# imaginateit/csm-train-pytorch

Hardware: AMD Instinct MI355X
Metric: train tokens/sec (text+audio) CSM-1B bf16 seq2048 (higher is better)
Workload: dtype bf16

## Files before the change

csm-train-pytorch_amd/csm/engine.py:

```python
from __future__ import annotations

import math
import numbers
from contextlib import contextmanager
from typing import Dict, List, Optional

import torch

from .hip import ops

BF16 = torch.bfloat16
F32 = torch.float32
import os as _os
FUSE_SWIGLU = _os.environ.get("CSM_FUSE_SWIGLU", "1") == "1"
FUSE_ROPE_BWD = _os.environ.get("CSM_FUSE_ROPE_BWD", "1") == "1"
FUSE_ROPE_FWD = _os.environ.get("CSM_FUSE_ROPE_FWD", "1") == "1"
PAIR_DX_DW = int(_os.environ.get("CSM_PAIR_DX_DW", "0"))
GROUP_ATTN_DW = _os.environ.get("CSM_GROUP_ATTN_DW", "1") == "1"
DEFER_ATTN_DW = int(_os.environ.get("CSM_DEFER_ATTN_DW", "3"))
DEFER_NORM_DW = _os.environ.get("CSM_DEFER_NORM_DW", "1") == "1"
ROWS_ON_HOST = _os.environ.get("CSM_ROWS_ON_HOST", "1") == "1"
EMB_KEYSORT = _os.environ.get("CSM_EMB_KEYSORT", "1") == "1"
DECODE_POS_HOST = _os.environ.get("CSM_DECODE_POS_HOST", "1") == "1"
LORA_FUSE = _os.environ.get("CSM_LORA_FUSE", "1") != "0"
# ... 562 lines not shown

    def _decoder_forward(self, hidden, rows, tg, B, S, save, sel=None):
        m, a = self.m, self.m.args
        dev = m.device
        K, V, Vp = a.audio_num_codebooks, a.audio_vocab_size, m.vocab_pad
        N = rows.numel()
        d, dd = m.bb.embed_dim, m.dc.embed_dim
        codes = tg[:, :S, :].reshape(-1, K) if tg.shape[1] >= S else None
        if codes is None:
            b, p = rows.long() // S, rows.long() % S
            codes = tg[b, p]
        else:
            codes = codes[rows.long()]
        codes = codes.contiguous()
        seq = torch.empty(N * K, d, dtype=BF16, device=dev)
        ops.decoder_input_fwd(hidden, rows, codes, m.block("audio_embeddings.weight"), seq, V)
        x0 = torch.empty(N * K, dd, dtype=BF16, device=dev)
        ops.linear_fwd(seq, m.block("projection.weight"), x0)
        dsel = sel[rows.long()].repeat_interleave(K).contiguous() if sel is not None else None
        xf = self.decoder.forward(x0, N, K, save, on_layer_start=self.param_hook, sel=dsel)
        logits = torch.empty(K - 1, N, Vp, dtype=F32, device=dev)
        ah = m.block("audio_head.padded")
        xf2 = xf.view(N, K * dd)
        ops.gemm(xf2[:, dd:2 * dd], ah[0], logits[0], None, False, True, batch=K - 1, sA=dd, sB=dd * Vp, sC=N * Vp)
        tgt = codes[:, 1:].t().contiguous().reshape(-1)
        rows_loss = torch.empty((K - 1) * N, dtype=F32, device=dev)
        ops.ce_fwd_bwd(logits.view(-1, Vp), tgt, rows_loss, None, V, 0.0)
        out = dict(rows_loss=rows_loss, n_rows=(K - 1) * N)
        if save:
            out.update(rows=rows, codes=codes, seq=seq, xf=xf, logits=logits, tgt=tgt, N=N, sel=dsel)
        return out

    def backward(self, gscale: float = 1.0):
        if self.saved is None:
            raise RuntimeError("backward() without a saved forward (was the forward run under no_grad?)")
        s, m, a = self.saved, self.m, self.m.args
        self.saved = None
        dev = m.device
        B, S = s["B"], s["S"]
        K, V, Vp = a.audio_num_codebooks, a.audio_vocab_size, m.vocab_pad
        M, d, dd = B * S, m.bb.embed_dim, m.dc.embed_dim
        tr = m.trainable
        train_embeddings, train_other = tr["embeddings"], tr["other"]
        m.ensure_grads()
        gst = m.grad_state
        dec_runs = s["dec"] is not None and s["aw"] != 0.0
        writes = {"backbone": tr["backbone"], "decoder": dec_runs and tr["decoder"], "other": train_other,
                  "embeddings": train_embeddings}
        acc = {}
        for g_, w_ in writes.items():
            acc[g_] = gst[g_] == "live"
            if gst[g_] == "stale" and (not w_ or g_ == "embeddings"):
                o_, n_ = m.group_range(g_)
                m.grad_arena[o_:o_ + n_].zero_()
                gst[g_] = "zero"
            if w_:
                gst[g_] = "live"
        if train_other and not acc["other"] and not dec_runs:
            m.block("projection.weight", True).zero_()
            m.block("audio_head.padded", True).zero_()
        hidden = s["hidden"]
        dseq = None
        dec_pos0 = None
        dec = s["dec"]
        if dec is not None and s["aw"] != 0.0:
            N = dec["N"]
            dl = torch.empty(K - 1, N, Vp, dtype=BF16, device=dev)
            ops.ce_fwd_bwd(dec["logits"].view(-1, Vp), dec["tgt"], dec["rows_loss"], dl.view(-1, Vp), V,
                           gscale * s["aw"] / dec["n_rows"])
            ah = m.block("audio_head.padded")
            dxf = torch.zeros(N, K * dd, dtype=BF16, device=dev)
            ops.gemm(dl[0], ah[0], dxf[:, dd:2 * dd], None, False, False, batch=K - 1, sA=N * Vp, sB=dd * Vp, sC=dd)
            xf2 = dec["xf"].view(N, K * dd)
            if train_other:
                gah = m.block("audio_head.padded", True)
                ops.gemm(xf2[:, dd:2 * dd], dl[0], gah[0], gah[0] if acc["other"] else None, True, True, batch=K - 1, sA=dd,
                         sB=N * Vp, sC=dd * Vp, sR=dd * Vp)
            del dl
            dx0 = self.decoder.backward(dxf.view(N * K, dd), N, K, tr["decoder"], 1.0, on_layer_done=self.grad_hook,
                                        acc=acc["decoder"], sel=dec.get("sel"))
            dseq = torch.empty(N * K, d, dtype=BF16, device=dev)
            ops.linear_dx(dx0, m.block("projection.weight"), dseq)
            if train_other:
                ops.linear_dw(dx0, dec["seq"], m.block("projection.weight", True), accumulate=acc["other"])
            dec_pos0 = (dseq, dec["rows"], K)
            if self.grad_hook is not None:
                self.grad_hook("decoder", -1)

        dlog = torch.empty(M, Vp, dtype=BF16, device=dev)
        rows_loss = torch.empty(M, dtype=F32, device=dev)
        ops.ce_fwd_bwd(s["logits"], s["t0"], rows_loss, dlog, V, gscale * s["sw"] / s["n_sem"])
        dhid = torch.empty(M, d, dtype=BF16, device=dev)
        ops.linear_dx(dlog, m.block("codebook0_head.padded"), dhid)
        if train_other:
            ops.linear_dw(dlog, hidden, m.block("codebook0_head.padded", True), accumulate=acc["other"])
        del dlog
        if dec_pos0 is not None:
            ops.rows_add_bf16(dhid, dec_pos0[1], dec_pos0[0], dec_pos0[2])
        if self.grad_hook is not None:
            self.grad_hook("other", -1)

        dh0 = self.backbone.backward(dhid, B, S, tr["backbone"], 1.0, on_layer_done=self.grad_hook, acc=acc["backbone"], seg=s.get("seg"),
                                    sel=s.get("sel"))
        if train_embeddings:
            self._embedding_backward(s, dh0, dseq if (dec is not None and s["aw"] != 0.0) else None)
        if self.grad_hook is not None:
            self.grad_hook("embeddings", -1)

    def _embedding_backward(self, s, dh0, dseq):
        m, a = self.m, self.m.args
        dev = m.device
        K, V = a.audio_num_codebooks, a.audio_vocab_size
        TV = a.text_vocab_size
        n_rows = TV + K * V
        tk, mk = s["tk"], s["mk"]
        M = tk.shape[0]
        ck = ("embbwd", M, K, V, TV)
        c = self._consts.get(ck)
        if c is None:
            slot = torch.arange(K + 1, device=dev)
            c = self._consts[ck] = dict(off=torch.where(slot < K, TV + slot * V, torch.zeros_like(slot)),
                                        src=torch.arange(M, device=dev).unsqueeze(1).expand(M, K + 1).reshape(-1).contiguous())
        rows = torch.where(mk.bool(), tk + c["off"], torch.full_like(tk, n_rows)).reshape(-1)
        src = c["src"]
        n_src = M
        if dseq is not None:
            codes, N = s["dec"]["codes"], s["dec"]["N"]
            dk = ("embbwd_dec", M, N, K, V, TV)
            d = self._consts.get(dk)
            if d is None:
                d = self._consts[dk] = dict(off=TV + torch.arange(K - 1, device=dev) * V,
                                            src=(M + torch.arange(N, device=dev).unsqueeze(1) * K + torch.arange(1, K, device=dev)).reshape(-1))
            rows = torch.cat([rows, (codes[:, :K - 1] + d["off"]).reshape(-1)])
            src = torch.cat([src, d["src"]])
            n_src = M + N * K
        if n_src <= (1 << 20) and EMB_KEYSORT:
            key = torch.sort((rows << 20) | src).values
            rows_s, src_s = key >> 20, key & ((1 << 20) - 1)
        else:
            order = torch.argsort(rows, stable=True)
            rows_s, src_s = rows[order].contiguous(), src[order].contiguous()
        ops.embed_bwd_sorted(rows_s, src_s, dh0, dseq,
                             m.block("text_embeddings.weight", True), m.block("audio_embeddings.weight", True))

    @torch.no_grad()
    def hidden_states(self, tokens: torch.Tensor, masks: torch.Tensor) -> torch.Tensor:
        m, a = self.m, self.m.args
        B, S, K1 = tokens.shape
        M = B * S
        tk = tokens.reshape(M, K1).to(device=m.device, dtype=torch.int64).contiguous()
        mk = masks.reshape(M, K1).to(device=m.device, dtype=torch.uint8).contiguous()
        h0 = torch.empty(M, m.bb.embed_dim, dtype=BF16, device=m.device)
        self._need()
        ops.embed_fwd(tk, mk, m.block("text_embeddings.weight"), m.block("audio_embeddings.weight"), h0, a.audio_vocab_size)
        return self.backbone.forward(h0, B, S, False).view(B, S, -1)

    @torch.no_grad()
    def generate_frame(self, tokens, tokens_mask, input_pos, temperature, topk, noise=None, adapters=None, top_p=None,
                       min_p=None):
        m, a = self.m, self.m.args
        self._need()
        if int(input_pos[0, 0]) == 0:
            m._gen_adapters = list(adapters) if adapters is not None and any(x is not None for x in adapters) else None
        if not getattr(m, "use_kv_cache", True):
            if top_p is not None or min_p is not None:
                raise ValueError("the recompute path (use_kv_cache = False) has no top_p / min_p: the filters need the KV-cache path")
            return self._generate_frame_recompute(tokens, tokens_mask, input_pos, temperature, topk, noise)
        dev = m.device
        K, V, Vp = a.audio_num_codebooks, a.audio_vocab_size, m.vocab_pad
        d, dd = m.bb.embed_dim, m.dc.embed_dim
        tokens, tokens_mask = tokens.to(dev), tokens_mask.to(dev)
        Bn, Sn, K1 = tokens.shape
        first = int(input_pos[0, 0]) == 0
        st = getattr(m, "_decode_state", None)
        if not first and (st is None or st.B != Bn or st.cur < 0):
            raise RuntimeError("generate_frame: a non-first call (input_pos > 0) needs the state of a prompt prefilled with the "
                               "same batch size (call it with input_pos starting at 0 first)")
        if first:
            st = m._decode_state = DecodeState(self, Bn, adapters)
        temperature, topk = st.sampling_args(temperature, topk, top_p, min_p)
        if first:
            last_h = st.prefill(tokens, tokens_mask)
            return self._frame_tail(st, last_h, temperature, topk, noise)
        if Sn != 1:
            raise ValueError("generate_frame with caches: after the prompt, feed one position per call")
        if getattr(m, "use_hip_graph", True):
            return st.graph_frame(tokens, tokens_mask, temperature, topk, noise)
        st._advance()
        return self._decode_frame(st, tokens, tokens_mask, temperature, topk, noise)

    @torch.no_grad()
    def generate_first_frames(self, tokens_list, masks_list, temperature, topk, noise=None, adapters=None, top_p=None,
                              min_p=None):
        m = self.m
        self._need()
        st = m._decode_state = DecodeState(self, len(tokens_list), adapters)
# ... 753 lines not shown
```

csm-train-pytorch_amd/csm/hip/__init__.py:

```python
import ctypes as C
import os

_HERE = os.path.dirname(os.path.abspath(__file__))
LIB_PATH = os.environ.get("CSM_HIP_LIB") or os.path.join(_HERE, "libcsm_hip.so")


class CsmHipError(RuntimeError):
    pass


if not os.path.exists(LIB_PATH):
    raise ImportError(
        f"{LIB_PATH} is missing: build it with `python __graft_entry__.py build` (or `make -C csm-train-pytorch_amd/csrc`). "
        "The CSM MI355X path has no fallback implementation."
    )

lib = C.CDLL(LIB_PATH)

_p, _i, _f, _ll = C.c_void_p, C.c_int, C.c_float, C.c_longlong

_SIGS = {
    "csm_abi_version": ([], _i),
    "csm_last_error": ([], C.c_char_p),
    "csm_device_check": ([_i], _i),
    "csm_gemm_bf16": ([_p, _p, _p, _p, _i, _i, _i, _i, _i, _i, _i, _i, _i, _i, _f, _i, _ll, _ll, _ll, _ll, _p], _i),
    "csm_gemm_bf16_ex": ([_p, _p, _p, _p, _i, _i, _i, _i, _i, _i, _i, _i, _i, _i, _f, _i, _ll, _ll, _ll, _ll, _i, _p, _p, _i, _p], _i),
    "csm_gemm_bf16_rope": ([_p, _p, _p, _i, _i, _i, _i, _i, _i, _p, _i, _i, _i, _p], _i),
    "csm_gemm_bf16_kext": ([_p, _p, _p, _p, _i, _i, _i, _i, _i, _i, _i, _i, _i, _p, _p, _i, _i, _p, _p, _i, _i, _i, _p], _i),
    "csm_gemm_bf16_pinned": ([_p, _p, _p, _p, _i, _i, _i, _i, _i, _i, _i, _i, _i, _f, _p, _p, _i, _i, _p, _p, _i, _i, _i, _p], _i),
    "csm_skinny_nt_bf16": ([_p, _p, _p, _i, _i, _i, _i, _i, _i, _f, _p], _i),
    "csm_skinny_nt_sel_bf16": ([_p, _p, _p, _p, _i, _i, _i, _i, _i, _i, _i, _f, _p], _i),
    "csm_gemm_bf16_dgrad_wgrad": ([_p, _p, _p, _p, _p, _i, _i, _i, _i, _i, _i, _i, _i, _i, _p, _i, _i, _f, _p], _i),
    "csm_gemm_bf16_two_wgrad": ([_p, _p, _p, _i, _i, _i, _i, _i, _p, _p, _p, _i, _i, _i, _i, _i, _i, _i, _f, _p], _i),
    "csm_gemm_bf16_multi_wgrad": ([_i, _p, _p, _p, _p, _p, _p, _p, _p, _i, _i, _f, _p], _i),
    "csm_set_gemm_variant": ([_i], _i),
    "csm_set_gemm256_persistent": ([_i], _i),
    "csm_get_gemm256_persistent": ([], _i),
    "csm_set_gemm_tuning": ([_i, _i], _i),
    "csm_gemm_last_kernel": ([], C.c_char_p),
    "csm_attn_bwd_workspace_bytes": ([_i, _i, _i], _ll),
    "csm_rmsnorm_fwd": ([_p, _p, _p, _p, _i, _i, _f, _p], _i),
    "csm_rmsnorm_bwd_blocks": ([], _i),
    "csm_rmsnorm_bwd": ([_p, _p, _p, _p, _p, _p, _p, _i, _i, _p], _i),
    "csm_colsum_bf16": ([_p, _i, _i, _p, _i, _p], _i),
    "csm_colsum_bf16_multi": ([_i, _p, _p, _i, _i, _i, _p], _i),
    "csm_dropout_bf16": ([_p, _i, _p, _i, _ll, _i, _f, C.c_ulonglong, _i, _p], _i),
    "csm_bias_add_bf16": ([_p, _i, _p, _ll, _i, _p], _i),
    "csm_colsum_rows_bf16": ([_p, _i, _ll, _i, _p, _i, _p], _i),
    "csm_rope": ([_p, _p, _p, _ll, _i, _i, _i, _i, _i, _p], _i),
    "csm_set_attn_variant": ([_i], _i),
    "csm_attn_last_dkv_kernel": ([], _i),
    "csm_attn64_set_debug": ([_p], _i),
    "csm_set_decode_tuning": ([_i, _i], _i),
    "csm_attn_fwd": ([_p, _p, _p, _i, _i, _i, _i, _i, _p], _i),
    "csm_attn_bwd": ([_p, _p, _p, _p, _p, _p, _i, _i, _i, _i, _i, _p], _i),
    "csm_attn_bwd_rope": ([_p, _p, _p, _p, _p, _p, _p, _i, _i, _i, _i, _i, _p], _i),
    "csm_attn_fwd_seg": ([_p, _p, _p, _p, _i, _i, _i, _i, _i, _p], _i),
    "csm_attn_bwd_seg": ([_p, _p, _p, _p, _p, _p, _p, _p, _i, _i, _i, _i, _i, _p], _i),
    "csm_swiglu_fwd": ([_p, _p, _ll, _i, _p], _i),
    "csm_swiglu_bwd": ([_p, _p, _p, _ll, _i, _p], _i),
    "csm_embed_fwd": ([_p, _p, _p, _p, _p, _ll, _i, _i, _i, _p], _i),
    "csm_embed_bwd_sorted": ([_p, _p, _ll, _p, _p, _ll, _p, _p, _ll, _ll, _i, _p], _i),
    "csm_rows_add_bf16": ([_p, _p, _p, _ll, _i, _i, _p], _i),
    "csm_rows_take_bf16": ([_p, _p, _p, _ll, _i, _p], _i),
    "csm_decoder_input_fwd": ([_p, _p, _p, _p, _p, _ll, _i, _i, _i, _p], _i),
    "csm_ce_fwd_bwd": ([_p, _p, _p, _p, _ll, _i, _i, _i, _f, _p], _i),
    "csm_reduce_sum_f32": ([_p, _ll, _f, _p, _p], _i),
    "csm_sumsq_blocks": ([], _i),
    "csm_sumsq_bf16": ([_p, _ll, _p, _p], _i),
    "csm_clip_coef": ([_p, _i, _f, _p, _p], _i),
    "csm_adamw_step": ([_p, _p, _p, _p, _p, _ll, _f, _f, _f, _f, _f, _i, _p, _f, _i, _p], _i),
    "csm_adamw_step_split": ([_p, _p, _p, _p, _p, _ll, _f, _f, _f, _f, _f, _i, _p, _f, _i, _p], _i),
    "csm_adamw_step_live": ([_p, _p, _p, _p, _p, _ll, _f, _f, _f, _f, _f, _i, _p, _f, _i, _p, _p], _i),
    "csm_adamw_step_split_live": ([_p, _p, _p, _p, _p, _ll, _f, _f, _f, _f, _f, _i, _p, _f, _i, _p, _p], _i),
    "csm_set_adamw_blocks": ([_i], _i),
    "csm_gemv_bf16": ([_p, _p, _p, _p, _i, _i, _i, _i, _i, _i, _i, _p], _i),
    "csm_gemv_bf16_kext": ([_p, _p, _p, _p, _i, _i, _i, _i, _i, _i, _i, _p, _f, _i, _p, _i, _p, _p, _i, _i, _i, _p, _p], _i),
    "csm_lora_project_bf16": ([_p, _p, _p, _i, _i, _i, _i, _i, _i, _f, _p, _f, _p], _i),
    "csm_lora_project_rows_bf16": ([_p, _p, _p, _p, _p, _i, _i, _i, _i, _i, _i, _i, _p, _f, _p], _i),
    "csm_gemv_bf16_kext_rows": ([_p, _p, _p, _p, _i, _i, _i, _i, _i, _i, _i, _p, _f, _i, _p, _i, _p, _p, _p, _p, _i, _i, _i, _i, _p], _i),
    "csm_gemv_t_bf16": ([_p, _p, _p, _i, _i, _i, _i, _i, _i, _i, _p], _i),
    "csm_gemv_bf16_ex": ([_p, _p, _p, _p, _i, _i, _i, _i, _i, _i, _i, _p, _f, _i, _p, _i, _p], _i),
    "csm_quantize_rows_fp8": ([_p, _p, _p, _i, _i, _i, _i, _p], _i),
    "csm_gemv_fp8w": ([_p, _p, _p, _p, _p, _i, _i, _i, _i, _i, _i, _i, _p, _f, _i, _p, _i, _p], _i),
    "csm_attn_decode_rope": ([_p, _p, _p, _p, _p, _p, _i, _i, _i, _i, _i, _i, _p], _i),
    "csm_gemv_attn_bf16": ([_p, _p, _p, _p, _p, _p, _p, _p, _i, _i, _i, _i, _i, _i, _i, _i, _i, _p], _i),
    "csm_gemv_attn_at_bf16": ([_p, _p, _p, _i, _p, _p, _p, _p, _i, _i, _i, _i, _i, _i, _p], _i),
    "csm_attn_decode_rope_at": ([_p, _p, _p, _p, _i, _p, _i, _i, _i, _i, _i, _i, _p], _i),
    "csm_attn_append": ([_p, _p, _p, _p, _i, _i, _i, _i, _i, _i, _i, _f, _p], _i),
    "csm_attn_append_rows": ([_p, _p, _p, _p, _p, _p, _p, _i, _i, _i, _i, _i, _f, _p], _i),
    "csm_kv_append": ([_p, _p, _p, _p, _i, _i, _i, _i, _i, _i, _p], _i),
    "csm_kv_shift": ([_p, _p, _p, _i, _i, _i, _i, _i, _i, _i, _p], _i),
    "csm_attn_decode": ([_p, _p, _p, _p, _p, _i, _i, _i, _i, _i, _i, _p], _i),
    "csm_sample_topk": ([_p, _p, _p, _i, _i, _i, _i, _f, _p], _i),
    "csm_sample_topk_rows": ([_p, _p, _p, _i, _i, _i, _p, _p, _p], _i),
    "csm_sample_filtered_rows": ([_p, _p, _p, _i, _i, _i, _p, _p, _p, _p, _p], _i),
    "csm_rvq_encode": ([_p, _p, _p, _i, _i, _i, _i, _i, _p], _i),
    "csm_conv1d_f32": ([_p, _p, _p, _p, _p, _i, _i, _i, _i, _i, _i, _i, _i, _i, _i, _i, _p], _i),
    "csm_conv_transpose1d_f32": ([_p, _p, _p, _p, _i, _i, _i, _i, _i, _i, _i, _i, _i, _p], _i),
    "csm_layernorm_f32": ([_p, _p, _p, _p, _i, _i, _f, _p], _i),
    "csm_linear_f32": ([_p, _p, _p, _p, _p, _i, _i, _i, _i, _i, _p], _i),
    "csm_rope_half_f32": ([_p, _i, _i, _i, _f, _i, _p], _i),
    "csm_attn_window_f32": ([_p, _p, _i, _i, _i, _i, _p], _i),
    "csm_transpose_f32": ([_p, _p, _i, _i, _p], _i),
    "csm_conv1d_stream_f32": ([_p, _p, _p, _p, _p, _p, _p, _i, _i, _i, _i, _i, _i, _i, _p], _i),
    "csm_conv1d_stream_strided_f32": ([_p, _p, _p, _p, _p, _p, _p, _i, _i, _i, _i, _i, _i, _i, _i, _i, _p], _i),
    "csm_conv_transpose1d_stream_f32": ([_p, _p, _p, _p, _p, _p, _i, _i, _i, _i, _i, _i, _i, _i, _p], _i),
    "csm_attn_window_stream_f32": ([_p, _p, _p, _p, _i, _i, _i, _i, _i, _i, _p], _i),
    "csm_rvq_decode": ([_p, _p, _p, _i, _i, _i, _i, _p], _i),
    "csm_conv1d_stream_rows_f32": ([_p, _p, _p, _p, _p, _p, _i, _p, _p, _i, _i, _i, _i, _i, _i, _i, _i, _p], _i),
    "csm_conv1d_stream_strided_rows_f32": ([_p, _p, _p, _p, _p, _p, _i, _p, _p, C.c_uint, _i, _i, _i, _i, _i, _i, _i, _i, _i, _p], _i),
    "csm_conv_transpose1d_stream_rows_f32": ([_p, _p, _p, _p, _p, _i, _p, _p, _p, _i, _i, _i, _i, _i, _i, _i, _i, _p], _i),
    "csm_rope_half_rows_f32": ([_p, _i, _p, _i, _i, _i, _f, _p], _i),
    "csm_attn_window_stream_rows_f32": ([_p, _p, _p, _p, _i, _p, _p, _i, _i, _i, _i, _i, _i, _p], _i),
    "csm_transpose_rows_f32": ([_p, _p, _i, _i, _i, _p], _i),
    "csm_resample_f32": ([_p, _p, _p, _i, _ll, _i, _i, _i, _p], _i),
    "csm_resample_stream_rows_f32": ([_p, _p, _p, _p, _ll, _i, _p, _p, _p, _p, C.c_uint, _i, _i, _i, _i, _i, _p], _i),
    "csm_resample_stream_f32": ([_p, _i, _p, _i, _ll, _i, _p, _p, _ll, _i, _i, _i, _i, _p], _i),
}

for _name, (_args, _res) in _SIGS.items():
    _fn = getattr(lib, _name)
    _fn.argtypes = _args
# ... 34 lines not shown
```

csm-train-pytorch_amd/csm/hip/ops.py:

```python
import ctypes
import math
from typing import Optional

import torch

from . import CsmHipError, check, lib

BF16 = torch.bfloat16


def _stream() -> int:
    return torch.cuda.current_stream().cuda_stream


def _ptr(t: Optional[torch.Tensor]) -> Optional[int]:
    return None if t is None else t.data_ptr()


def _mat(t: torch.Tensor, dtype=BF16):
    assert t.is_cuda and t.dtype == dtype and t.dim() == 2 and t.stride(1) == 1, (t.dtype, t.shape, t.stride())
    return t.data_ptr(), t.shape[0], t.shape[1], t.stride(0)


def _pin(pin):
# ... 256 lines not shown
    need = lib.csm_attn_bwd_workspace_bytes(B, S, H)
    assert delta_ws.dtype == torch.float32 and delta_ws.is_contiguous() and delta_ws.numel() * 4 >= need, f"delta_ws: {need} bytes of scratch"
    if rope_table is None:
        check(lib.csm_attn_bwd(qkv.data_ptr(), out.data_ptr(), dout.data_ptr(), lse.data_ptr(), dqkv.data_ptr(),
                               delta_ws.data_ptr(), B, S, H, KV, HD, _stream()), "csm_attn_bwd")
    else:
        assert rope_table.dtype == torch.float32 and rope_table.is_contiguous() and rope_table.shape[0] >= S
        check(lib.csm_attn_bwd_rope(qkv.data_ptr(), out.data_ptr(), dout.data_ptr(), lse.data_ptr(), dqkv.data_ptr(),
                                    delta_ws.data_ptr(), rope_table.data_ptr(), B, S, H, KV, HD, _stream()), "csm_attn_bwd_rope")
    return dqkv


def _seg_array(t, B, S):
    assert t.dtype == torch.int32 and t.is_cuda and t.is_contiguous() and t.numel() == B * S, "segment array: int32 [B*S] on the device"
    return t.data_ptr()


def attn_fwd_seg(qkv, out, lse, seg_start, B, S, H, KV, HD):
    assert qkv.is_contiguous() and out.is_contiguous() and qkv.shape == (B * S, (H + 2 * KV) * HD)
    check(lib.csm_attn_fwd_seg(qkv.data_ptr(), out.data_ptr(), lse.data_ptr(), _seg_array(seg_start, B, S), B, S, H, KV, HD, _stream()),
          "csm_attn_fwd_seg")
    return out


def attn_bwd_seg(qkv, out, dout, lse, dqkv, delta_ws, seg_start, seg_end, B, S, H, KV, HD):
    assert qkv.is_contiguous() and out.is_contiguous() and dout.is_contiguous() and dqkv.is_contiguous()
    need = lib.csm_attn_bwd_workspace_bytes(B, S, H)
    assert delta_ws.dtype == torch.float32 and delta_ws.is_contiguous() and delta_ws.numel() * 4 >= need, f"delta_ws: {need} bytes of scratch"
    check(lib.csm_attn_bwd_seg(qkv.data_ptr(), out.data_ptr(), dout.data_ptr(), lse.data_ptr(), dqkv.data_ptr(), delta_ws.data_ptr(),
                               _seg_array(seg_start, B, S), _seg_array(seg_end, B, S), B, S, H, KV, HD, _stream()), "csm_attn_bwd_seg")
    return dqkv


def swiglu_fwd(gu, out):
    M, F2 = gu.shape
    check(lib.csm_swiglu_fwd(gu.data_ptr(), out.data_ptr(), M, F2 // 2, _stream()), "csm_swiglu_fwd")
    return out


def swiglu_bwd(gu, dout, dgu):
    M, F2 = gu.shape
    check(lib.csm_swiglu_bwd(gu.data_ptr(), dout.data_ptr(), dgu.data_ptr(), M, F2 // 2, _stream()), "csm_swiglu_bwd")
    return dgu


def embed_fwd(tokens, mask_u8, text_emb, audio_emb, out, audio_vocab):
    M, K1 = tokens.shape
    assert tokens.dtype == torch.int64 and mask_u8.dtype == torch.uint8 and tokens.is_contiguous() and mask_u8.is_contiguous()
    check(lib.csm_embed_fwd(tokens.data_ptr(), mask_u8.data_ptr(), text_emb.data_ptr(), audio_emb.data_ptr(), out.data_ptr(),
                            M, K1 - 1, out.shape[1], audio_vocab, _stream()), "csm_embed_fwd")
    return out


def embed_bwd_sorted(sorted_rows, src_index, dh, dseq, g_text, g_audio):
    assert sorted_rows.dtype == torch.int64 and src_index.dtype == torch.int64 and sorted_rows.is_contiguous() and src_index.is_contiguous()
    check(lib.csm_embed_bwd_sorted(sorted_rows.data_ptr(), src_index.data_ptr(), sorted_rows.numel(), dh.data_ptr(), _ptr(dseq),
                                   dh.shape[0], g_text.data_ptr(), g_audio.data_ptr(), g_text.shape[0],
                                   g_text.shape[0] + g_audio.shape[0], dh.shape[1], _stream()), "csm_embed_bwd_sorted")


def rows_add_bf16(dst, rows_i32, src, src_stride_rows):
    check(lib.csm_rows_add_bf16(dst.data_ptr(), rows_i32.data_ptr(), src.data_ptr(), rows_i32.numel(), int(src_stride_rows),
                                dst.shape[1], _stream()), "csm_rows_add_bf16")


def rows_take_bf16(table, rows_i32, out):
    assert rows_i32.dtype == torch.int32 and rows_i32.is_contiguous() and out.is_contiguous() and out.shape == (rows_i32.numel(), table.shape[1])
    check(lib.csm_rows_take_bf16(table.data_ptr(), rows_i32.data_ptr(), out.data_ptr(), rows_i32.numel(), table.shape[1], _stream()),
          "csm_rows_take_bf16")
    return out


def decoder_input_fwd(hidden, rows_i32, codes, audio_emb, out, audio_vocab):
    N, K = codes.shape
    assert rows_i32.dtype == torch.int32 and codes.dtype == torch.int64 and codes.is_contiguous()
    check(lib.csm_decoder_input_fwd(hidden.data_ptr(), rows_i32.data_ptr(), codes.data_ptr(), audio_emb.data_ptr(),
                                    out.data_ptr(), N, K, hidden.shape[1], audio_vocab, _stream()), "csm_decoder_input_fwd")
    return out


def ce_fwd_bwd(logits_f32, targets, loss_rows, dlogits, V, grad_scale):
    R, ldl = logits_f32.shape[0], logits_f32.stride(0)
    assert logits_f32.dtype == torch.float32 and targets.dtype == torch.int64 and targets.is_contiguous()
    ldd = dlogits.stride(0) if dlogits is not None else 0
    check(lib.csm_ce_fwd_bwd(logits_f32.data_ptr(), targets.data_ptr(), loss_rows.data_ptr(), _ptr(dlogits), R, V, ldl, ldd,
                             float(grad_scale), _stream()), "csm_ce_fwd_bwd")


def reduce_sum(x_f32, out_f32, scale=1.0):
    check(lib.csm_reduce_sum_f32(x_f32.data_ptr(), x_f32.numel(), float(scale), out_f32.data_ptr(), _stream()), "csm_reduce_sum_f32")


def sumsq_blocks() -> int:
    return lib.csm_sumsq_blocks()


def sumsq_bf16(g, partials):
    check(lib.csm_sumsq_bf16(g.data_ptr(), g.numel(), partials.data_ptr(), _stream()), "csm_sumsq_bf16")


def clip_coef(partials, max_norm, norm_and_coef):
    check(lib.csm_clip_coef(partials.data_ptr(), partials.numel(), float(max_norm), norm_and_coef.data_ptr(), _stream()), "csm_clip_coef")


ADAMW_BLOCK = 2048


def _live_ptr(block_live, n):
    assert block_live.dtype == torch.uint8 and block_live.is_contiguous() and block_live.numel() == -(-n // ADAMW_BLOCK)
    return block_live.data_ptr()


def adamw_step(master, m, v, param, grad, lr, beta1, beta2, eps, wd, step, norm_and_coef=None, grad_mul=1.0, zero_grad=False, *,
               block_live=None):
    n = master.numel()
    assert master.dtype == torch.float32 and param.dtype == BF16 and grad.dtype == BF16 and param.numel() == n == grad.numel()
    args = (master.data_ptr(), m.data_ptr(), v.data_ptr(), param.data_ptr(), grad.data_ptr(), n, lr, beta1, beta2, eps, wd, int(step),
            _ptr(norm_and_coef), float(grad_mul), int(zero_grad))
    if block_live is None:
        check(lib.csm_adamw_step(*args, _stream()), "csm_adamw_step")
    else:
        check(lib.csm_adamw_step_live(*args, _live_ptr(block_live, n), _stream()), "csm_adamw_step_live")


def adamw_step_split(master_lo, m, v, param, grad, lr, beta1, beta2, eps, wd, step, norm_and_coef=None, grad_mul=1.0, zero_grad=False, *,
                     block_live=None):
    n = master_lo.numel()
    assert master_lo.dtype == torch.int16 and param.dtype == BF16 and grad.dtype == BF16 and param.numel() == n == grad.numel()
    args = (master_lo.data_ptr(), m.data_ptr(), v.data_ptr(), param.data_ptr(), grad.data_ptr(), n, lr, beta1, beta2, eps, wd, int(step),
            _ptr(norm_and_coef), float(grad_mul), int(zero_grad))
    if block_live is None:
        check(lib.csm_adamw_step_split(*args, _stream()), "csm_adamw_step_split")
    else:
        check(lib.csm_adamw_step_split_live(*args, _live_ptr(block_live, n), _stream()), "csm_adamw_step_split_live")


def gemv(x, W, y, residual=None):
    B, K = x.shape
    N = W.shape[0]
    assert W.shape[1] == K and y.shape == (B, N) and x.stride(1) == 1 and W.stride(1) == 1 and y.stride(1) == 1
    check(lib.csm_gemv_bf16(x.data_ptr(), W.data_ptr(), y.data_ptr(), _ptr(residual), B, N, K, W.stride(0), x.stride(0),
                            y.stride(0), int(y.dtype == torch.float32), _stream()), "csm_gemv_bf16")
    return y


def gemv_ex(x, W, y, residual=None, norm_scale=None, eps=1e-5, swiglu=False, row_index=None, row_offset=0):
    B = y.shape[0]
    K = x.shape[1]
    N = W.shape[0]
    assert W.shape[1] == K and y.shape == (B, N // 2 if swiglu else N) and x.stride(1) == 1 and W.stride(1) == 1 and y.stride(1) == 1
    assert row_index is not None or x.shape[0] == B
    assert row_index is None or (row_index.dtype == torch.int32 and row_index.numel() == B and row_index.is_contiguous())
    check(lib.csm_gemv_bf16_ex(x.data_ptr(), W.data_ptr(), y.data_ptr(), _ptr(residual), B, N, K, W.stride(0), x.stride(0),
                               y.stride(0), int(y.dtype == torch.float32), _ptr(norm_scale), float(eps), int(swiglu),
                               _ptr(row_index), int(row_offset), _stream()), "csm_gemv_bf16_ex")
# ... 411 lines not shown
```

csm-train-pytorch_amd/csm/training/optim.py:

```python
import os
from typing import Dict, List, Optional

import torch

from ..hip import ops

F32 = torch.float32
SPLIT_MASTER = os.environ.get("CSM_ADAMW_SPLIT", "1") == "1"
FLAGGED_GROUPS = ("embeddings",)


def split_master(master: torch.Tensor, param_out: torch.Tensor) -> torch.Tensor:
    bits = master.contiguous().view(torch.int32)
    param_out.view(torch.int16).copy_(((bits + 0x8000) >> 16).to(torch.int16))
    return (bits & 0xFFFF).to(torch.int16)


def join_master(param: torch.Tensor, lo: torch.Tensor) -> torch.Tensor:
    hi = param.view(torch.int16).to(torch.int32) & 0xFFFF
    l = lo.to(torch.int32) & 0xFFFF
    return (((hi - (l >> 15)) << 16) | l).view(torch.float32)


def seed_master(model, offset: int, numel: int, param: torch.Tensor, from_fp32_source: bool = False) -> torch.Tensor:
    master = param.float()
    src = getattr(model, "_fp32_source", None) if from_fp32_source else None
    if src:
        views, base = model._views(model.arena), model.arena.storage_offset()
        for k, t in src.items():
            v = views.get(k)
            if v is None:
                continue
            so = v.storage_offset() - base
            end = _span_end(v, so)
            if so >= offset and end <= offset + numel:
                torch.as_strided(master, v.size(), v.stride(), so - offset).copy_(t.to(master.device))
            elif so < offset + numel and end > offset:
                a_, b_ = max(so, offset), min(end, offset + numel)
                scratch = torch.zeros(end - so, dtype=master.dtype, device=master.device)
                scratch[a_ - so:b_ - so] = master[a_ - offset:b_ - offset]
                torch.as_strided(scratch, v.size(), v.stride(), 0).copy_(t.to(master.device))
                master[a_ - offset:b_ - offset] = scratch[a_ - so:b_ - so]
    return master


def _span_end(v: torch.Tensor, so: int) -> int:
    return so + sum((sz - 1) * st for sz, st in zip(v.size(), v.stride())) + 1


def live_blocks(m: torch.Tensor, v: torch.Tensor) -> torch.Tensor:
    bits, B = m.view(torch.int32) | v.view(torch.int32), ops.ADAMW_BLOCK
    full = bits.numel() // B * B
    live = [bits[:full].view(-1, B).any(dim=1)]
    if full < bits.numel():
        live.append(bits[full:].any().reshape(1))
    return torch.cat(live).to(torch.uint8)


class FusedAdamW:
    sharded = False
    dead_blocks = True

    def __init__(self, model, group_lrs: Dict[str, float], weight_decay: float = 0.01, betas=(0.9, 0.999),
                 eps: float = 1e-8, lora_lr: Optional[float] = None, lora_weight_decay: float = 0.0):
        self.model = model
        self.betas, self.eps = betas, eps
        self.param_groups: List[dict] = []
        self.state: Dict[str, Dict[str, torch.Tensor]] = {}
        self.step_count = 0
        self._coef: Optional[torch.Tensor] = None
        self.dead_blocks = os.environ.get("CSM_ADAMW_DEAD_BLOCKS", "1") == "1"
        model.ensure_grads()
        for name, lr in group_lrs.items():
            if lr is None or not model.trainable.get(name, False):
                continue
            off, n = model.group_range(name)
            self.param_groups.append(dict(name=name, lr=float(lr), weight_decay=weight_decay, offset=off, numel=n,
                                          param=model.arena[off:off + n], grad=model.grad_arena[off:off + n]))
        if model.lora is not None and lora_lr is not None:
            lo = model.lora
            self.param_groups.append(dict(name="lora", lr=float(lora_lr), weight_decay=lora_weight_decay, offset=0,
                                          numel=lo.arena.numel(), param=lo.arena, grad=lo.grad_arena))
        for g in self.param_groups:
            master = self._seed_master(g, from_fp32_source=True)
            if SPLIT_MASTER:
                lo = split_master(master, g["param"])
                self.state[g["name"]] = dict(lo=lo, m=torch.zeros_like(master), v=torch.zeros_like(master))
                del master
            else:
                self.state[g["name"]] = dict(master=master, m=torch.zeros_like(master), v=torch.zeros_like(master))
            if self.dead_blocks and g["name"] in FLAGGED_GROUPS:
                self.state[g["name"]]["live"] = torch.zeros(-(-g["numel"] // ops.ADAMW_BLOCK), dtype=torch.uint8, device=g["param"].device)
        self._partials = torch.empty(max(1, len(self.param_groups)) * ops.sumsq_blocks(), dtype=F32, device=model.device)
        self._norm_coef = torch.ones(2, dtype=F32, device=model.device)
        import weakref
        if not hasattr(model, "_optimizers"):
            model._optimizers = []
        model._optimizers.append(weakref.ref(self))

    def _seed_master(self, g, from_fp32_source: bool = False) -> torch.Tensor:
        return seed_master(self.model, g["offset"], g["numel"], g["param"], from_fp32_source and g["name"] != "lora")

    def moments_rewritten(self):
        for name in FLAGGED_GROUPS:
            if self.dead_blocks and name in self.state:
                st = self.state[name]
                st["live"] = live_blocks(st["m"], st["v"])

    def named_master(self):
        m = self.model
        views, base = m._views(m.arena), m.arena.storage_offset()
        for g in self.param_groups:
            if g["name"] == "lora":
                continue
            master = self.master(g["name"])
            for k, v in views.items():
                so = v.storage_offset() - base
                if g["offset"] <= so < g["offset"] + g["numel"]:
                    yield k, torch.as_strided(master, v.size(), v.stride(), so - g["offset"])

    def _group(self, name):
        return next(g for g in self.param_groups if g["name"] == name)

    def master(self, name: str) -> torch.Tensor:
        st = self.state[name]
        return st["master"] if "master" in st else join_master(self._group(name)["param"], st["lo"])

    def set_master(self, name: str, master: torch.Tensor):
        st, g = self.state[name], self._group(name)
        if "master" in st:
            st["master"].copy_(master)
            g["param"].copy_(st["master"])
        else:
            st["lo"].copy_(split_master(master.to(device=g["param"].device, dtype=F32), g["param"]))

    def num_trainable(self) -> int:
        return sum(g["numel"] for g in self.param_groups)

    def zero_grad(self, set_to_none: bool = False):
        for g in self.param_groups:
            g["grad"].zero_()
            if g["name"] in self.model.grad_state:
                self.model.grad_state[g["name"]] = "zero"
        self._coef = None

    def _settle(self):
        gs = self.model.grad_state
        for g in self.param_groups:
            if gs.get(g["name"]) == "stale":
                g["grad"].zero_()
                gs[g["name"]] = "zero"

    def clip_grad_norm(self, max_norm: float) -> torch.Tensor:
        self._settle()
        nb = ops.sumsq_blocks()
        for i, g in enumerate(self.param_groups):
            ops.sumsq_bf16(g["grad"], self._partials[i * nb:(i + 1) * nb])
        ops.clip_coef(self._partials[:len(self.param_groups) * nb], max_norm, self._norm_coef)
        self._coef = self._norm_coef
        return self._norm_coef[0]

    def step(self, zero_grad=False, skip: Optional[torch.Tensor] = None):
        self._settle()
        self.step_count += 1
        self.model._fp32_source = None
        if skip is not None:
            coef = self._coef[1] if self._coef is not None else torch.ones((), dtype=F32, device=skip.device)
            self._norm_coef[1] = torch.where(skip.reshape(()) != 0, torch.full_like(coef, -1.0), coef)
            self._coef = self._norm_coef
        b1, b2 = self.betas
        gs = self.model.grad_state
        for g in self.param_groups:
            st = self.state[g["name"]]
            name = g["name"]
            zero = bool(zero_grad) if zero_grad != "lazy" else (name == "embeddings" or name not in gs)
            if "lo" in st:
                ops.adamw_step_split(st["lo"], st["m"], st["v"], g["param"], g["grad"], g["lr"], b1, b2, self.eps,
                                     g["weight_decay"], self.step_count, self._coef, zero_grad=zero, block_live=st.get("live"))
            else:
                ops.adamw_step(st["master"], st["m"], st["v"], g["param"], g["grad"], g["lr"], b1, b2, self.eps,
                               g["weight_decay"], self.step_count, self._coef, zero_grad=zero, block_live=st.get("live"))
            if name in gs:
                if zero:
                    gs[name] = "zero"
                elif zero_grad == "lazy" and gs[name] == "live":
                    gs[name] = "stale"
        self._coef = None

    def uncount_step(self):
        self.step_count = max(0, self.step_count - 1)

    def params_rewritten(self, base: bool = True, lora: bool = True, from_fp32_source: bool = False):
        for g in self.param_groups:
            if lora if g["name"] == "lora" else base:
                self.set_master(g["name"], self._seed_master(g, from_fp32_source))

    def state_dict(self):
        return {"step": self.step_count,
                "groups": [{k: g[k] for k in ("name", "lr", "weight_decay", "offset", "numel")} for g in self.param_groups],
                "state": {n: {"master": self.master(n).cpu(), "m": st["m"].cpu(), "v": st["v"].cpu()} for n, st in self.state.items()}}

    def load_state_dict(self, sd):
        saved_by_name = {g["name"]: g for g in sd["groups"]}
        mine = [g["name"] for g in self.param_groups]
        if sorted(saved_by_name) != sorted(mine) or sorted(sd["state"]) != sorted(mine):
            raise ValueError(f"optimizer state was saved for parameter groups {sorted(saved_by_name)} but this optimizer has "
                             f"{sorted(mine)} (different freeze flags / LoRA setting?)")
        for g in self.param_groups:
            saved = saved_by_name[g["name"]]
            if (saved["offset"], saved["numel"]) != (g["offset"], g["numel"]):
                raise ValueError(f"optimizer group {g['name']!r}: saved range {saved['offset']}+{saved['numel']} != {g['offset']}+{g['numel']}")
        self.step_count = sd["step"]
        for n, st in sd["state"].items():
            for k, v in st.items():
                if k == "master":
                    self.set_master(n, v)
# ... 7 lines not shown
```

csm-train-pytorch_amd/csrc/common.h:

```cpp
#pragma once
#include <hip/hip_runtime.h>
#include <stdint.h>

typedef uint16_t bf16_t;
typedef __attribute__((ext_vector_type(8))) short bf16x8;
typedef __attribute__((ext_vector_type(4))) short bf16x4;
typedef __attribute__((ext_vector_type(4))) float f32x4;

#define CSM_WAVE 64

__device__ __forceinline__ float bf2f(bf16_t v) { return __uint_as_float(((uint32_t)v) << 16); }

__device__ __forceinline__ bf16_t f2bf(float f) {
    __bf16 b = (__bf16)f;
    return *reinterpret_cast<bf16_t*>(&b);
}

__device__ __forceinline__ uint32_t pack2bf(float lo, float hi) {
    return (uint32_t)f2bf(lo) | ((uint32_t)f2bf(hi) << 16);
}

typedef __attribute__((ext_vector_type(2))) float csm_f32x2;
typedef __attribute__((ext_vector_type(2))) __bf16 csm_bf16x2;
__device__ __forceinline__ uint32_t pack2bf_pk(float lo, float hi) {
// ... 33 lines not shown
    v += lane_xor<32>(v); v += lane_xor<16>(v); v += lane_xor<8>(v); v += lane_xor<4>(v); v += lane_xor<2>(v); v += lane_xor<1>(v);
    return v;
}

__device__ __forceinline__ float wave_max(float v) {
    v = fmaxf(v, lane_xor<32>(v)); v = fmaxf(v, lane_xor<16>(v)); v = fmaxf(v, lane_xor<8>(v));
    v = fmaxf(v, lane_xor<4>(v)); v = fmaxf(v, lane_xor<2>(v)); v = fmaxf(v, lane_xor<1>(v));
    return v;
}

__device__ __forceinline__ void lds_barrier() { asm volatile("s_waitcnt lgkmcnt(0)\n\ts_barrier" ::: "memory"); }

__device__ __forceinline__ float block_sum(float v, float* red) {
    const int lane = threadIdx.x & 63, w = threadIdx.x >> 6, nw = (blockDim.x + 63) >> 6;
    v = wave_sum(v);
    __syncthreads();
    if (lane == 0) red[w] = v;
    __syncthreads();
    float t = 0.f;
    for (int i = 0; i < nw; ++i) t += red[i];
    return t;
}

__device__ __forceinline__ float block_max(float v, float* red) {
    const int lane = threadIdx.x & 63, w = threadIdx.x >> 6, nw = (blockDim.x + 63) >> 6;
    v = wave_max(v);
    __syncthreads();
    if (lane == 0) red[w] = v;
    __syncthreads();
    float t = red[0];
    for (int i = 1; i < nw; ++i) t = fmaxf(t, red[i]);
    return t;
}

typedef __attribute__((ext_vector_type(4))) uint32_t U4;

__device__ __forceinline__ void unpack8(const U4& u, float* f) {
    f[0] = __uint_as_float(u.x << 16); f[1] = __uint_as_float(u.x & 0xffff0000u);
    f[2] = __uint_as_float(u.y << 16); f[3] = __uint_as_float(u.y & 0xffff0000u);
    f[4] = __uint_as_float(u.z << 16); f[5] = __uint_as_float(u.z & 0xffff0000u);
    f[6] = __uint_as_float(u.w << 16); f[7] = __uint_as_float(u.w & 0xffff0000u);
}

__device__ __forceinline__ U4 pack8(const float* f) {
    U4 u = {pack2bf(f[0], f[1]), pack2bf(f[2], f[3]), pack2bf(f[4], f[5]), pack2bf(f[6], f[7])};
    return u;
}

__device__ __forceinline__ U4 pack8_pk(const float* f) {
    U4 u = {pack2bf_pk(f[0], f[1]), pack2bf_pk(f[2], f[3]), pack2bf_pk(f[4], f[5]), pack2bf_pk(f[6], f[7])};
    return u;
}

__device__ __forceinline__ bf16x4 lds_read_tr16(const void* lds_addr) {
    return __builtin_amdgcn_ds_read_tr16_b64_v4i16((__attribute__((address_space(3))) bf16x4*)(lds_addr));
}

__device__ __forceinline__ bf16x8 cat4(bf16x4 a, bf16x4 b) {
    bf16x8 r;
    r[0] = a[0]; r[1] = a[1]; r[2] = a[2]; r[3] = a[3];
    r[4] = b[0]; r[5] = b[1]; r[6] = b[2]; r[7] = b[3];
    return r;
}

extern "C" void csm_set_error(const char* fmt, ...);
#define CSM_CHECK_LAUNCH(name)                                                        \
    do {                                                                              \
        hipError_t e__ = hipGetLastError();                                           \
        if (e__ != hipSuccess) {                                                      \
            csm_set_error("%s: launch failed: %s", name, hipGetErrorString(e__));     \
            return 2;                                                                 \
        }                                                                             \
    } while (0)
#define CSM_REQUIRE(cond, ...)                                                        \
    do {                                                                              \
        if (!(cond)) {                                                                \
            csm_set_error(__VA_ARGS__);                                               \
            return 1;                                                                 \
        }                                                                             \
    } while (0)
```

csm-train-pytorch_amd/csrc/gemm.hip:

```cpp
#include "gemm_common.h"

const char* g_last_gemm_kernel = "";

namespace {

template <int TA, int TB, typename OutT, bool GLDS>
__global__ __launch_bounds__(256, 2) void gemm_kernel(GemmArgs g) {
    extern __shared__ __attribute__((aligned(16))) char smem[];
    const int nwg = g.tiles_m * g.tiles_n;
    int id = blockIdx.x;
    {
        const int q = nwg >> 3, r = nwg & 7, xcd = id & 7, within = id >> 3;
        id = (xcd < r ? xcd * (q + 1) : r * (q + 1) + (xcd - r) * q) + within;
    }
    constexpr int GROUP_M = 8;
    const int per_group = GROUP_M * g.tiles_n;
    const int grp = id / per_group;
    const int first_m = grp * GROUP_M;
    const int gsz = min(g.tiles_m - first_m, GROUP_M);
    const int tm = first_m + (id % per_group) % gsz;
    const int tn = (id % per_group) / gsz;
    const int m0 = tm * BM, n0 = tn * BN;

    const int bz = blockIdx.z;
// ... 254 lines not shown
}

}

int csm_gemm256_launch(const void* A, const void* B, void* C, const void* R, int M, int N, int K, int lda, int ldb, int ldc,
                       int ldr, int transA, int transB, int out_f32, float alpha, int batch, long long sA, long long sB,
                       long long sC, long long sR, int epi_mode, const void* aux_in, void* aux_out, int ld_aux,
                       hipStream_t stream, int epi_p0 = 0, int epi_p1 = 0, const void* xA = nullptr, const void* xB = nullptr, int kx = 0);

int csm_gemm256w4_launch(const void* A, const void* B, void* C, const void* R, int M, int N, int K, int lda, int ldb, int ldc, int ldr,
                         int transA, int transB, int out_f32, float alpha, int batch, long long sA, long long sB, long long sC,
                         long long sR, int epi_mode, const void* aux_in, void* aux_out, int ld_aux,
                         hipStream_t stream, int epi_p0, int epi_p1, const void* xA = nullptr, const void* xB = nullptr, int kx = 0);

int g_gemm_w4 = 1;
int g_w4_kext = 1;
static bool prefer_256(int M, int N, int K, int batch, double need = 0.80) {
    if (K % 64 != 0 || M < 8 || N < 8) return false;
    const long long tiles = (long long)((M + 255) / 256) * ((N + 255) / 256) * batch;
    const long long rounds = (tiles + 255) / 256;
    const double fill = (double)tiles / (double)(rounds * 256);
    const double area = ((double)M * N * batch) / ((double)tiles * 65536.0);
    return fill * area >= need;
}

extern int g_persistent;
extern "C" int csm_set_gemm256_persistent(int v) { g_persistent = v ? 1 : 0; return 0; }
extern "C" int csm_get_gemm256_persistent(void) { return g_persistent; }
extern "C" const char* csm_gemm_last_kernel(void) { return g_last_gemm_kernel; }

extern int g_gemm_touch;
extern int g_w4_stagger[4];
extern int g_w4_fast_epi, g_w4_n6;
extern "C" int csm_set_gemm_tuning(int key, int value) {
    CSM_REQUIRE(key >= 0 && key <= 8, "csm_set_gemm_tuning: unknown key %d", key);
    if (key == 0) g_gemm_touch = value ? 1 : 0;
    else if (key == 1) g_gemm_w4 = value ? 1 : 0;
    else if (key == 6) g_w4_fast_epi = value ? 1 : 0;
    else if (key == 7) g_w4_kext = value ? 1 : 0;
    else if (key == 8) g_w4_n6 = value ? 1 : 0;
    else {
        CSM_REQUIRE(value >= 0 && value <= (key == 2 ? 32 : 20000), "csm_set_gemm_tuning: key %d value %d out of range", key, value);
        g_w4_stagger[key - 2] = key == 2 ? (value < 1 ? 1 : value) : value;
    }
    return 0;
}

extern "C" int csm_set_gemm_variant(int v) {
    CSM_REQUIRE(v >= 0 && v <= 4, "csm_set_gemm_variant: %d is not one of 0..4", v);
    g_gemm_variant = v;
    return 0;
}

static int gemm_dispatch(const void* A, const void* B, void* C, const void* R, int M, int N, int K, int lda,
                         int ldb, int ldc, int ldr, int transA, int transB, int out_f32, float alpha, int batch,
                         long long strideA, long long strideB, long long strideC, long long strideR, int epilogue,
                         const void* aux_in, void* aux_out, int ld_aux, hipStream_t stream, int epi_p0, int epi_p1,
                         const void* xA = nullptr, const void* xB = nullptr, int kx = 0, int pin = 0) {
    const int variant = pin ? 1 : g_gemm_variant;
    CSM_REQUIRE(A && B && C, "csm_gemm_bf16: null operand");
    CSM_REQUIRE(M > 0 && N > 0 && K > 0 && batch > 0, "csm_gemm_bf16: bad shape M=%d N=%d K=%d batch=%d", M, N, K, batch);
    CSM_REQUIRE((lda & 7) == 0 && (ldb & 7) == 0, "csm_gemm_bf16: lda/ldb must be multiples of 8 (lda=%d ldb=%d)", lda, ldb);
    CSM_REQUIRE(((uintptr_t)A & 15) == 0 && ((uintptr_t)B & 15) == 0, "csm_gemm_bf16: A/B must be 16-byte aligned");
    CSM_REQUIRE((strideA & 7) == 0 && (strideB & 7) == 0, "csm_gemm_bf16: batch strides of A/B must be multiples of 8");
    if (!transA) CSM_REQUIRE((K & 7) == 0, "csm_gemm_bf16: K must be a multiple of 8 when A is [M][K] (K=%d)", K);
    else CSM_REQUIRE((M & 7) == 0, "csm_gemm_bf16: M must be a multiple of 8 when A is [K][M] (M=%d)", M);
    if (!transB) CSM_REQUIRE((K & 7) == 0, "csm_gemm_bf16: K must be a multiple of 8 when B is [N][K] (K=%d)", K);
    else CSM_REQUIRE((N & 7) == 0, "csm_gemm_bf16: N must be a multiple of 8 when B is [K][N] (N=%d)", N);
    CSM_REQUIRE(lda >= (transA ? M : K) && ldb >= (transB ? N : K) && ldc >= (epilogue == 2 ? 2 * N : N), "csm_gemm_bf16: leading dimension too small");
    if (epilogue == 1) CSM_REQUIRE(!out_f32 && aux_out && (N & 3) == 0 && (ldc & 3) == 0 && ld_aux >= N / 2 && (ld_aux & 1) == 0, "csm_gemm_bf16_ex: bad SwiGLU-forward epilogue arguments");
    if (epilogue == 2) CSM_REQUIRE(!out_f32 && aux_in && (N & 3) == 0 && (ldc & 7) == 0 && (ld_aux & 7) == 0 && ld_aux >= 2 * N && !R && ((uintptr_t)aux_in & 15) == 0 && ((uintptr_t)C & 15) == 0, "csm_gemm_bf16_ex: bad SwiGLU-backward epilogue arguments");
    CSM_REQUIRE(epilogue >= 0 && epilogue <= 3, "csm_gemm_bf16_ex: unknown epilogue %d", epilogue);
    if (epilogue == 1 || epilogue == 3) CSM_REQUIRE(!R || (ldr & 3) == 0, "csm_gemm_bf16: a residual under the SwiGLU-forward / RoPE epilogue needs ldr %% 4 == 0 (ldr=%d)", ldr);
    if (((variant == 2 && g_gemm_w4 && prefer_256(M, N, K, batch, 0.70)) || (variant == 4 && K % 64 == 0 && M >= 8 && N >= 8)) && (kx == 0 || g_w4_kext))
        return csm_gemm256w4_launch(A, B, C, R, M, N, K, lda, ldb, ldc, ldr, transA, transB, out_f32, alpha, batch, strideA, strideB,
                                    strideC, strideR, epilogue, aux_in, aux_out, ld_aux, stream, epi_p0, epi_p1, xA, xB, kx);
    if ((variant == 2 && prefer_256(M, N, K, batch)) || (variant >= 3 && K % 64 == 0 && M >= 8 && N >= 8))
        return csm_gemm256_launch(A, B, C, R, M, N, K, lda, ldb, ldc, ldr, transA, transB, out_f32, alpha, batch, strideA,
                                  strideB, strideC, strideR, epilogue, aux_in, aux_out, ld_aux, stream, epi_p0, epi_p1, xA, xB, kx);
    GemmArgs g;
    g.epi_p0 = epi_p0; g.epi_p1 = epi_p1;
    g.xA = (const bf16_t*)xA; g.xB = (const bf16_t*)xB; g.kx = kx;
    g.A = (const bf16_t*)A; g.B = (const bf16_t*)B; g.C = C; g.R = (const bf16_t*)R;
    g.M = M; g.N = N; g.K = K; g.lda = lda; g.ldb = ldb; g.ldc = ldc; g.ldr = ldr;
    g.sA = strideA; g.sB = strideB; g.sC = strideC; g.sR = strideR;
    g.alpha = alpha;
    g.epi_mode = epilogue; g.aux_in = (const bf16_t*)aux_in; g.aux_out = (bf16_t*)aux_out; g.ld_aux = ld_aux;
    g.tiles_m = (M + BM - 1) / BM; g.tiles_n = (N + BN - 1) / BN;
    if (!transA && !transB) return launch<0, 0>(g, out_f32, batch, stream, pin);
    if (!transA && transB) return launch<0, 1>(g, out_f32, batch, stream, pin);
    if (transA && transB) return launch<1, 1>(g, out_f32, batch, stream, pin);
    return launch<1, 0>(g, out_f32, batch, stream, pin);
}

extern "C" int csm_gemm_bf16_ex(const void* A, const void* B, void* C, const void* R, int M, int N, int K, int lda,
                                int ldb, int ldc, int ldr, int transA, int transB, int out_f32, float alpha, int batch,
                                long long strideA, long long strideB, long long strideC, long long strideR, int epilogue,
                                const void* aux_in, void* aux_out, int ld_aux, hipStream_t stream) {
    CSM_REQUIRE(epilogue >= 0 && epilogue <= 2, "csm_gemm_bf16_ex: unknown epilogue %d", epilogue);
    return gemm_dispatch(A, B, C, R, M, N, K, lda, ldb, ldc, ldr, transA, transB, out_f32, alpha, batch, strideA, strideB, strideC,
                         strideR, epilogue, aux_in, aux_out, ld_aux, stream, 0, 0);
}

extern "C" int csm_gemm_bf16_rope(const void* A, const void* W, void* C, int M, int N, int K, int lda, int ldw, int ldc,
                                  const float* rope_table, int rows_per_seq, int n_rope_cols, int head_dim, hipStream_t stream) {
    CSM_REQUIRE(rope_table && rows_per_seq > 0 && head_dim >= 8 && (head_dim & 7) == 0 && n_rope_cols >= 0 && n_rope_cols <= N &&
                n_rope_cols % head_dim == 0 && (N & 7) == 0 && (ldc & 7) == 0 && ((uintptr_t)C & 15) == 0,
                "csm_gemm_bf16_rope: bad arguments");
    return gemm_dispatch(A, W, C, nullptr, M, N, K, lda, ldw, ldc, 0, 0, 0, 0, 1.f, 1, 0, 0, 0, 0, EPI_ROPE, rope_table, nullptr,
                         rows_per_seq, stream, n_rope_cols, head_dim);
}

extern "C" int csm_gemm_bf16_kext(const void* A, const void* B, void* C, const void* R, int M, int N, int K, int lda, int ldb, int ldc,
// ... 34 lines not shown
    CSM_CHECK_LAUNCH("csm_skinny_nt_bf16");
    return 0;
}

extern "C" int csm_skinny_nt_sel_bf16(const void* X, const void* Wt, void* out, const int* sel, int M, int N, int K, int blk, int ldx,
                                      int ldw, int ldo, float alpha, hipStream_t stream) {
    CSM_REQUIRE(X && Wt && out && sel && M > 0, "csm_skinny_nt_sel_bf16: null operand");
    CSM_REQUIRE(N >= 32 && N <= 256 && N % 32 == 0 && K >= 128 && K % 128 == 0,
                "csm_skinny_nt_sel_bf16: N must be a multiple of 32 in [32, 256] and K a multiple of 128 (N=%d K=%d)", N, K);
    CSM_REQUIRE(blk >= 8 && blk % 8 == 0, "csm_skinny_nt_sel_bf16: blk must be a positive multiple of 8 (blk=%d)", blk);
    CSM_REQUIRE((ldx & 7) == 0 && (ldw & 7) == 0 && (ldo & 3) == 0 && ldx >= K && ldw >= K && ldo >= N, "csm_skinny_nt_sel_bf16: bad leading dimensions");
    CSM_REQUIRE(((uintptr_t)X & 15) == 0 && ((uintptr_t)Wt & 15) == 0 && ((uintptr_t)out & 7) == 0 && ((uintptr_t)sel & 3) == 0,
                "csm_skinny_nt_sel_bf16: operands must be 16-byte aligned (sel: 4-byte)");
    const dim3 grid((M + 15) / 16), block(256);
#define CSM_SEL_CASE(NT) \
    case NT: hipLaunchKernelGGL((skinny_nt_sel_kernel<NT>), grid, block, 0, stream, (const bf16_t*)X, (const bf16_t*)Wt, (bf16_t*)out, sel, M, K, blk, \
                                ldx, ldw, ldo, alpha); break;
    switch (N / 16) {
        CSM_SEL_CASE(2) CSM_SEL_CASE(4) CSM_SEL_CASE(6) CSM_SEL_CASE(8) CSM_SEL_CASE(10) CSM_SEL_CASE(12) CSM_SEL_CASE(14) CSM_SEL_CASE(16)
    }
#undef CSM_SEL_CASE
    CSM_CHECK_LAUNCH("csm_skinny_nt_sel_bf16");
    return 0;
}

extern "C" int csm_gemm_bf16(const void* A, const void* B, void* C, const void* R, int M, int N, int K, int lda,
                             int ldb, int ldc, int ldr, int transA, int transB, int out_f32, float alpha, int batch,
                             long long strideA, long long strideB, long long strideC, long long strideR,
                             hipStream_t stream) {
    return csm_gemm_bf16_ex(A, B, C, R, M, N, K, lda, ldb, ldc, ldr, transA, transB, out_f32, alpha, batch, strideA, strideB,
                            strideC, strideR, 0, nullptr, nullptr, 0, stream);
}

int csm_gemm256_pair_launch(const void* dY, const void* W, void* dX, int M, int Nout, int Kin, int ld_dy, int ldw, int ld_dx,
                            int dx_epi, const void* aux_in, int ld_aux,
                            const void* X, int ldx, void* dW, int ld_dw, int accumulate, float alpha_w, hipStream_t stream);

extern "C" int csm_gemm_bf16_dgrad_wgrad(const void* dY, const void* W, void* dX, const void* X, void* dW, int M, int Nout, int Kin,
                                         int ld_dy, int ldw, int ld_dx, int ldx, int ld_dw, int dx_epilogue, const void* aux_in,
                                         int ld_aux, int accumulate, float alpha_w, hipStream_t stream) {
    CSM_REQUIRE(dY && W && dX && X && dW, "csm_gemm_bf16_dgrad_wgrad: null operand");
    CSM_REQUIRE(M > 0 && Nout > 0 && Kin > 0 && M % 64 == 0 && Nout % 64 == 0 && (Kin & 7) == 0,
                "csm_gemm_bf16_dgrad_wgrad: M and Nout must be multiples of 64, Kin of 8 (M=%d Nout=%d Kin=%d)", M, Nout, Kin);
    CSM_REQUIRE((ld_dy & 7) == 0 && (ldw & 7) == 0 && (ldx & 7) == 0 && (ld_dw & 7) == 0 && (ld_dx & 7) == 0 && ld_dy >= Nout && ldw >= Kin &&
                ldx >= Kin && ld_dw >= Kin, "csm_gemm_bf16_dgrad_wgrad: bad leading dimensions");
    CSM_REQUIRE(((uintptr_t)dY & 15) == 0 && ((uintptr_t)W & 15) == 0 && ((uintptr_t)X & 15) == 0 && ((uintptr_t)dX & 15) == 0 &&
                ((uintptr_t)dW & 15) == 0, "csm_gemm_bf16_dgrad_wgrad: operands must be 16-byte aligned");
    CSM_REQUIRE(dx_epilogue == 0 || dx_epilogue == 2, "csm_gemm_bf16_dgrad_wgrad: dx_epilogue must be 0 or 2");
    if (dx_epilogue == 2)
        CSM_REQUIRE(aux_in && (Kin & 3) == 0 && ld_dx >= 2 * Kin && (ld_aux & 7) == 0 && ld_aux >= 2 * Kin && ((uintptr_t)aux_in & 15) == 0,
                    "csm_gemm_bf16_dgrad_wgrad: bad SwiGLU-backward epilogue arguments");
    else
        CSM_REQUIRE(ld_dx >= Kin, "csm_gemm_bf16_dgrad_wgrad: ld_dx too small");
    return csm_gemm256_pair_launch(dY, W, dX, M, Nout, Kin, ld_dy, ldw, ld_dx, dx_epilogue, aux_in, ld_aux, X, ldx, dW, ld_dw, accumulate,
                                   alpha_w, stream);
}

int csm_gemm256_two_wgrad_launch(const void* dY1, const void* X1, void* dW1, int N1, int K1, int ld_dy1, int ldx1, int ld_dw1,
                                 const void* dY2, const void* X2, void* dW2, int N2, int K2, int ld_dy2, int ldx2, int ld_dw2,
                                 int M, int accumulate, float alpha, hipStream_t stream);

int csm_gemm256w4_two_wgrad_launch(const void* dY1, const void* X1, void* dW1, int N1, int K1, int ld_dy1, int ldx1, int ld_dw1,
                                   const void* dY2, const void* X2, void* dW2, int N2, int K2, int ld_dy2, int ldx2, int ld_dw2,
                                   int M, int accumulate, float alpha, hipStream_t stream);
extern "C" int csm_gemm_bf16_two_wgrad(const void* dY1, const void* X1, void* dW1, int N1, int K1, int ld_dy1, int ldx1, int ld_dw1,
                                       const void* dY2, const void* X2, void* dW2, int N2, int K2, int ld_dy2, int ldx2, int ld_dw2,
                                       int M, int accumulate, float alpha, hipStream_t stream) {
    CSM_REQUIRE(dY1 && X1 && dW1 && dY2 && X2 && dW2, "csm_gemm_bf16_two_wgrad: null operand");
    CSM_REQUIRE(M > 0 && M % 64 == 0 && N1 > 0 && N2 > 0 && K1 > 0 && K2 > 0 && ((N1 | N2 | K1 | K2) & 7) == 0,
                "csm_gemm_bf16_two_wgrad: M must be a multiple of 64, the other dimensions of 8");
    CSM_REQUIRE(((ld_dy1 | ldx1 | ld_dw1 | ld_dy2 | ldx2 | ld_dw2) & 7) == 0 && ld_dy1 >= N1 && ldx1 >= K1 && ld_dw1 >= K1 && ld_dy2 >= N2 &&
                ldx2 >= K2 && ld_dw2 >= K2, "csm_gemm_bf16_two_wgrad: bad leading dimensions");
    CSM_REQUIRE((((uintptr_t)dY1 | (uintptr_t)X1 | (uintptr_t)dW1 | (uintptr_t)dY2 | (uintptr_t)X2 | (uintptr_t)dW2) & 15) == 0,
                "csm_gemm_bf16_two_wgrad: operands must be 16-byte aligned");
    if (g_gemm_w4 && g_gemm_variant != 3)
        return csm_gemm256w4_two_wgrad_launch(dY1, X1, dW1, N1, K1, ld_dy1, ldx1, ld_dw1, dY2, X2, dW2, N2, K2, ld_dy2, ldx2, ld_dw2, M,
                                              accumulate, alpha, stream);
    return csm_gemm256_two_wgrad_launch(dY1, X1, dW1, N1, K1, ld_dy1, ldx1, ld_dw1, dY2, X2, dW2, N2, K2, ld_dy2, ldx2, ld_dw2, M,
                                        accumulate, alpha, stream);
}

int csm_gemm256w4_multi_wgrad_launch(int n, const void* const* dY, const void* const* X, void* const* dW, const int* N, const int* K,
                                     const int* ld_dy, const int* ldx, const int* ld_dw, int M, int accumulate, float alpha,
                                     hipStream_t stream);
extern "C" int csm_gemm_bf16_multi_wgrad(int n, const void* const* dY, const void* const* X, void* const* dW, const int* N, const int* K,
                                         const int* ld_dy, const int* ldx, const int* ld_dw, int M, int accumulate, float alpha,
                                         hipStream_t stream) {
    CSM_REQUIRE(n >= 1 && n <= 12 && dY && X && dW && N && K && ld_dy && ldx && ld_dw, "csm_gemm_bf16_multi_wgrad: 1..12 products, no null array");
    CSM_REQUIRE(M > 0 && M % 64 == 0, "csm_gemm_bf16_multi_wgrad: M must be a positive multiple of 64");
    for (int i = 0; i < n; ++i) {
        CSM_REQUIRE(dY[i] && X[i] && dW[i], "csm_gemm_bf16_multi_wgrad: null operand in product %d", i);
        CSM_REQUIRE(N[i] > 0 && K[i] > 0 && ((N[i] | K[i] | ld_dy[i] | ldx[i] | ld_dw[i]) & 7) == 0 && ld_dy[i] >= N[i] && ldx[i] >= K[i] &&
                    ld_dw[i] >= K[i], "csm_gemm_bf16_multi_wgrad: product %d: dimensions must be multiples of 8, leading dimensions >= the row length", i);
        CSM_REQUIRE((((uintptr_t)dY[i] | (uintptr_t)X[i] | (uintptr_t)dW[i]) & 15) == 0, "csm_gemm_bf16_multi_wgrad: product %d: operands must be 16-byte aligned", i);
    }
    if (!(g_gemm_w4 && g_gemm_variant != 3)) {
        for (int i = 0; i < n; ++i) {
            const int rc = csm_gemm_bf16(dY[i], X[i], dW[i], accumulate ? dW[i] : nullptr, N[i], K[i], M, ld_dy[i], ldx[i], ld_dw[i], ld_dw[i], 1, 1,
                                         0, alpha, 1, 0, 0, 0, 0, stream);
            if (rc) return rc;
        }
        return 0;
    }
    return csm_gemm256w4_multi_wgrad_launch(n, dY, X, dW, N, K, ld_dy, ldx, ld_dw, M, accumulate, alpha, stream);
}
```

csm-train-pytorch_amd/csrc/gemm256w4.hip:

```cpp
#include "gemm_common.h"
#include "gemm256w4_loop.inc"

extern const char* g_last_gemm_kernel;
extern int g_persistent;
extern int g_gemm_touch;
int g_w4_fast_epi = 1;
int g_w4_n6 = 1;
int g_w4_stagger[4] = {1, 0, 0, 0};
#ifndef CSM_W4_TOUCH
#define CSM_W4_TOUCH 0
#endif
namespace { constexpr int g_w4_touch_dev = CSM_W4_TOUCH; }

namespace {

struct W4Args {
    const bf16_t* A; const bf16_t* B; void* C; const bf16_t* R;
    int M, N, K, lda, ldb, ldc, ldr;
    long long sA, sB, sC, sR;
    float alpha;
    int tiles_m, tiles_n;
    int epi_mode; const bf16_t* aux_in; bf16_t* aux_out; int ld_aux;
    int epi_p0, epi_p1;
    int touch;
    int fast_epi;
    const bf16_t* xA; const bf16_t* xB; int kx;
    int stagger_groups, stagger_ticks;
    int n6;
};

template <int N>
__device__ __forceinline__ f32x4 acc_read() {
    f32x4 v;
    asm volatile("v_accvgpr_read_b32 %0, a[%4]\n\tv_accvgpr_read_b32 %1, a[%5]\n\tv_accvgpr_read_b32 %2, a[%6]\n\tv_accvgpr_read_b32 %3, a[%7]"
                 : "=v"(v[0]), "=v"(v[1]), "=v"(v[2]), "=v"(v[3]) : "i"(N), "i"(N + 1), "i"(N + 2), "i"(N + 3));
    return v;
}
template <int I, int N, class F>
__device__ __forceinline__ void static_for(F&& f) {
    if constexpr (I < N) { f(std::integral_constant<int, I>{}); static_for<I + 1, N>(f); }
}

#ifndef CSM_ABLATE_W4EPI
#define CSM_ABLATE_W4EPI 0
#endif
#ifndef CSM_W4_STORE_POLICY
#define CSM_W4_STORE_POLICY ""
#endif
template <int IMM>
__device__ __forceinline__ void st16_s(const void* sbase, unsigned voff, const U4& v) {
    if (CSM_ABLATE_W4EPI & 2) { asm volatile("" ::"v"(v)); return; }
    asm volatile("global_store_dwordx4 %0, %1, %2 offset:%3" CSM_W4_STORE_POLICY "\n\ts_nop 1" ::"v"(voff), "v"(v), "s"(sbase), "n"(IMM) : "memory");
}
template <int IMM>
__device__ __forceinline__ void st8_s(const void* sbase, unsigned voff, const uint2& v) {
    if (CSM_ABLATE_W4EPI & 2) { asm volatile("" ::"v"(v)); return; }
    asm volatile("global_store_dwordx2 %0, %1, %2 offset:%3" CSM_W4_STORE_POLICY ::"v"(voff), "v"(v), "s"(sbase), "n"(IMM) : "memory");
}
template <int IMM>
__device__ __forceinline__ void ld16_s(U4& d, const void* sbase, unsigned voff) {
    if (CSM_ABLATE_W4EPI & 1) { d = (U4){0x3f803f80u + voff, 0x3f803f80u, 0x3f803f80u, 0x3f803f80u}; return; }
    asm volatile("global_load_dwordx4 %0, %1, %2 offset:%3" : "=v"(d) : "v"(voff), "s"(sbase), "n"(IMM) : "memory");
}
template <int N>
__device__ __forceinline__ void wait_loaded(U4 (&d)[2][4]) {
    asm volatile("s_waitcnt vmcnt(%8)"
                 : "+v"(d[0][0]), "+v"(d[0][1]), "+v"(d[0][2]), "+v"(d[0][3]), "+v"(d[1][0]), "+v"(d[1][1]), "+v"(d[1][2]), "+v"(d[1][3])
                 : "n"(N) : "memory");
}
template <int NA, int NB>
__device__ __forceinline__ void w4_gather(float (&v)[8]) {
    asm volatile("v_accvgpr_read_b32 %0, a[%8]\n\tv_accvgpr_read_b32 %1, a[%9]\n\tv_accvgpr_read_b32 %2, a[%10]\n\tv_accvgpr_read_b32 %3, a[%11]\n\t"
                 "v_accvgpr_read_b32 %4, a[%12]\n\tv_accvgpr_read_b32 %5, a[%13]\n\tv_accvgpr_read_b32 %6, a[%14]\n\tv_accvgpr_read_b32 %7, a[%15]\n\t"
                 "s_nop 1\n\t"
                 "v_permlane16_swap_b32 %0, %4\n\tv_permlane16_swap_b32 %1, %5\n\tv_permlane16_swap_b32 %2, %6\n\tv_permlane16_swap_b32 %3, %7\n\t"
                 "s_nop 1"
                 : "=v"(v[0]), "=v"(v[1]), "=v"(v[2]), "=v"(v[3]), "=v"(v[4]), "=v"(v[5]), "=v"(v[6]), "=v"(v[7])
                 : "n"(NA), "n"(NA + 1), "n"(NA + 2), "n"(NA + 3), "n"(NB), "n"(NB + 1), "n"(NB + 2), "n"(NB + 3));
}

template <int JH, bool SWIGLU>
__device__ __forceinline__ void w4_epi_plain(const Epi& e, int mb, int nb, int lane) {
    asm volatile("" : "+v"(lane));
    const int g = lane >> 4, r = lane & 15;
    const int nl = (g & 1) ? 16 + 4 * (g - 1) : 4 * g;
    const char* baseC = reinterpret_cast<const char*>(e.C) + ((size_t)mb * e.ldc + nb) * 2;
    const char* baseX = reinterpret_cast<const char*>(e.aux_out) + ((size_t)mb * e.ld_aux + (nb >> 1)) * 2;
    const unsigned voffC = (unsigned)(r * e.ldc + nl) * 2u, stepC = (unsigned)e.ldc * 32u;
    const unsigned voffX = (unsigned)(r * e.ld_aux + (nl >> 1)) * 2u, stepX = (unsigned)e.ld_aux * 32u;
    static_for<0, 8>([&](auto i_) {
        constexpr int i = decltype(i_)::value;
        static_for<0, 2>([&](auto jp_) {
            constexpr int jp = decltype(jp_)::value;
            float v[8];
            w4_gather<(8 * i + 4 * JH + 2 * jp) * 4, (8 * i + 4 * JH + 2 * jp + 1) * 4>(v);
#pragma unroll
            for (int k = 0; k < 8; ++k) v[k] *= e.alpha;
            st16_s<64 * jp>(baseC, voffC + i * stepC, pack8_pk(v));
            if constexpr (SWIGLU) {
                float a[4];
#pragma unroll
                for (int k = 0; k < 4; ++k) a[k] = silu(v[2 * k]) * v[2 * k + 1];
                uint2 w; w.x = pack2bf_pk(a[0], a[1]); w.y = pack2bf_pk(a[2], a[3]);
                st8_s<32 * jp>(baseX, voffX + i * stepX, w);
            }
        });
    });
}

__device__ __forceinline__ void w4_epi_swiglu_bwd(const Epi& e, int mb, int nb, int lane) {
    asm volatile("" : "+v"(lane));
    const int g = lane >> 4, r = lane & 15;
    const char* baseG = reinterpret_cast<const char*>(e.aux_in) + ((size_t)mb * e.ld_aux + 2 * nb) * 2;
    const char* baseC = reinterpret_cast<const char*>(e.C) + ((size_t)mb * e.ldc + 2 * nb) * 2;
    const unsigned voffG = (unsigned)(r * e.ld_aux + 8 * g) * 2u, stepG = (unsigned)e.ld_aux * 32u;
    const unsigned voffC = (unsigned)(r * e.ldc + 8 * g) * 2u, stepC = (unsigned)e.ldc * 32u;
    U4 gu[2][2][4];
    auto fetch = [&](auto p_, U4 (&dst)[2][4]) {
        constexpr int P = decltype(p_)::value, JH = P / 4, I0 = 2 * (P % 4);
#pragma unroll
        for (int ii = 0; ii < 2; ++ii) {
            const unsigned vo = voffG + (unsigned)(I0 + ii) * stepG;
            ld16_s<256 * JH>(dst[ii][0], baseG, vo); ld16_s<256 * JH + 64>(dst[ii][1], baseG, vo);
            ld16_s<256 * JH + 128>(dst[ii][2], baseG, vo); ld16_s<256 * JH + 192>(dst[ii][3], baseG, vo);
        }
    };
    fetch(std::integral_constant<int, 0>{}, gu[0]);
    static_for<0, 8>([&](auto p_) {
        constexpr int P = decltype(p_)::value, JH = P / 4, I0 = 2 * (P % 4);
        if constexpr (P < 7) fetch(std::integral_constant<int, P + 1>{}, gu[(P + 1) & 1]);
        U4 (&cur)[2][4] = gu[P & 1];
        wait_loaded<(P == 0 || P == 7) ? 8 : 16>(cur);
        static_for<0, 2>([&](auto ii_) {
            constexpr int ii = decltype(ii_)::value;
            constexpr int i = I0 + ii;
            const unsigned vo = voffC + (unsigned)i * stepC;
            static_for<0, 4>([&](auto j_) {
                constexpr int j = decltype(j_)::value;
                const f32x4 a = acc_read<(8 * i + 4 * JH + j) * 4>();
                float gv[8], o[8];
                unpack8(cur[ii][j], gv);
#pragma unroll
                for (int k = 0; k < 4; ++k) {
                    const float v = a[k] * e.alpha, gt = gv[2 * k], up = gv[2 * k + 1];
                    const float sg = (CSM_ABLATE_W4EPI & 4) ? gt : fast_sigmoid(gt);
                    o[2 * k] = v * up * sg * (1.f + gt * (1.f - sg));
                    o[2 * k + 1] = v * gt * sg;
                }
                st16_s<256 * JH + 64 * j>(baseC, vo, pack8_pk(o));
            });
        });
    });
}

template <int T, int PPW = 4>
__device__ __forceinline__ const char* w4_dma_offsets(const bf16_t* __restrict__ P, int ld, int rows, int row0, int wave, int lane,
                                                      unsigned (&off)[8], long long& step) {
    static_assert(PPW == 4 || T == 0, "the 96-row half-tile exists for K-contiguous operands only");
    step = T == 0 ? 128 : (long long)ld * 128;
    const int ub = T == 0 ? min(row0, rows - 1) : min(row0, rows - 8);
#pragma unroll
    for (int h = 0; h < 2; ++h)
#pragma unroll
        for (int i = 0; i < 4; ++i) {
            const int j = wave * PPW + (i < PPW ? i : PPW - 1);
            if (T == 0) {
                const int r = 8 * j + (lane >> 3);
                const int c = (lane & 7) ^ (r & 7);
                const int row = min(row0 + 32 * PPW * h + r, rows - 1);
                off[4 * h + i] = (unsigned)((row - ub) * ld + c * 8) * 2u;
            } else {
                const int kr = 4 * j + (lane >> 4);
                const int u = lane & 15;
                const int sl = (u >> 1) ^ ks_swz(kr);
                const int gc = min(row0 + 128 * h + sl * 16 + (u & 1) * 8, rows - 8);
                off[4 * h + i] = (unsigned)(kr * ld + (gc - ub)) * 2u;
            }
        }
    return reinterpret_cast<const char*>(T == 0 ? P + (size_t)ub * ld : P + ub);
}

#define WAIT_VM(n) asm volatile("s_waitcnt vmcnt(" #n ")" ::: "memory")
#define WAIT_VM_DYN(n) do { switch ((n) >> 2) { case 15: WAIT_VM(60); break; case 14: WAIT_VM(56); break; case 13: WAIT_VM(52); break; \
    case 12: WAIT_VM(48); break; case 11: WAIT_VM(44); break; case 10: WAIT_VM(40); break; case 9: WAIT_VM(36); break;                  \
    case 8: WAIT_VM(32); break; case 7: WAIT_VM(28); break; case 6: WAIT_VM(24); break; case 5: WAIT_VM(20); break;                     \
    case 4: WAIT_VM(16); break; case 3: WAIT_VM(12); break; case 2: WAIT_VM(8); break; case 1: WAIT_VM(4); break;                       \
    default: WAIT_VM(0); break; } } while (0)

template <int TA, int TB, typename OutT, int NJ = 8>
__device__ __forceinline__ void w4_tiles(const W4Args& g, int tile, const int stride, const int bz, char* smem) {
    constexpr int TN = 32 * NJ;
    const int nwg = g.tiles_m * g.tiles_n;
    const bf16_t* Ap = g.A + (size_t)bz * g.sA;
    const bf16_t* Bp = g.B + (size_t)bz * g.sB;
    const int lane = threadIdx.x & 63;
    const int wave = __builtin_amdgcn_readfirstlane(threadIdx.x >> 6);
    const int wr = wave >> 1, wc = wave & 1;
    const unsigned sbase = (unsigned)(uintptr_t)smem;
    unsigned la, lb;
    {
        const int r = lane & 15;
        const unsigned row_img = (unsigned)(r * 128 + (((lane >> 4) ^ (r & 7)) << 4));
        la = sbase + wr * 16384 + (TA == 0 ? row_img : (unsigned)tr_lane_off(lane));
        lb = sbase + wc * 16384 + (TB == 0 ? row_img : (unsigned)tr_lane_off(lane));
    }
    const unsigned key = (unsigned)tr_lane_key(lane);
    const int nt = __builtin_amdgcn_readfirstlane(g.K / 64);
    const unsigned woff = __builtin_amdgcn_readfirstlane(sbase + wave * 4096);
    auto coords = [&](int t_id, int& m0_, int& n0_) {
        const int q = nwg >> 3, r = nwg & 7, xcd = t_id & 7, within = t_id >> 3;
        t_id = (xcd < r ? xcd * (q + 1) : r * (q + 1) + (xcd - r) * q) + within;
        constexpr int GROUP_M = 4;
        const int per_group = GROUP_M * g.tiles_n;
        const int grp = t_id / per_group;
        const int first_m = grp * GROUP_M;
        const int gsz = min(g.tiles_m - first_m, GROUP_M);
        m0_ = (first_m + (t_id % per_group) % gsz) * 256;
        n0_ = ((t_id % per_group) / gsz) * TN;
    };
    unsigned offA[8], offB[8];
    long long stepA, stepB;
    const char *baseA, *baseB;
    int m0, n0;
    auto prep = [&]() {
        baseA = w4_dma_offsets<TA>(Ap, g.lda, g.M, m0, wave, lane, offA, stepA);
        baseB = w4_dma_offsets<TB, NJ / 2>(Bp, g.ldb, g.N, n0, wave, lane, offB, stepB);
    };
#define CSM_W4_OFFS "v"(offA[0]), "v"(offA[1]), "v"(offA[2]), "v"(offA[3]), "v"(offA[4]), "v"(offA[5]), "v"(offA[6]), "v"(offA[7]),      \
        "v"(offB[0]), "v"(offB[1]), "v"(offB[2]), "v"(offB[3]), "v"(offB[4]), "v"(offB[5]), "v"(offB[6]), "v"(offB[7])
    auto prologue = [&]() {
        prep();
        if constexpr (NJ == 8) asm volatile(CSM_W4_PRO ::CSM_W4_OFFS, "s"(baseA), "s"(baseB), "s"(stepA), "s"(stepB), "s"(nt), "s"(woff) : CSM_W4_PRO_CLOBBERS);
        else asm volatile(CSM_W4N6_PRO ::CSM_W4_OFFS, "s"(baseA), "s"(baseB), "s"(stepA), "s"(stepB), "s"(nt), "s"(woff) : CSM_W4_PRO_CLOBBERS);
    };
    coords(tile, m0, n0);
    prologue();
    int pend = 0;
    for (;;) {
        prep();
        const char* tptr = baseA;
        long long tstride = 0;
        int tcount = 0, tper = 0;
        if constexpr (sizeof(OutT) == 2) {
            if (NJ == 8 && g.epi_mode == EPI_SWIGLU_BWD && nt >= 16 && m0 + 256 <= g.M && n0 + 256 <= g.N) {
                tptr = reinterpret_cast<const char*>(g.aux_in) + (long long)(m0 + (int)(threadIdx.x >> 4)) * g.ld_aux * 2 +
                       (long long)n0 * 4 + (threadIdx.x & 15) * 64;
                tstride = (long long)16 * g.ld_aux * 2;
                tcount = (g_w4_touch_dev && g.touch) ? 16 : 0;
                tper = (nt - 4) / 16 - 1;
            }
        }
        tcount = __builtin_amdgcn_readfirstlane(tcount); tper = __builtin_amdgcn_readfirstlane(tper);
        { const int w = min(63, 8 + NJ + pend); WAIT_VM_DYN(w); }
#define CSM_W4_OPERANDS                                                                                                  \
    ::"v"(la), "v"(lb), "v"(key), CSM_W4_OFFS, "s"(baseA), "s"(baseB), "s"(stepA), "s"(stepB), "s"(nt), "s"(woff), "v"(tptr),            \
        "s"(tstride), "s"(tcount), "s"(tper)                                                                             \
        : CSM_W4_CLOBBERS
        if constexpr (NJ == 6) {
            static_assert(NJ == 8 || TB == 0, "256 x 192 tiles: K-contiguous B only");
            if constexpr (TA == 0) { asm volatile(CSM_W4N6_LOOP_00 CSM_W4_OPERANDS); } else { asm volatile(CSM_W4N6_LOOP_10 CSM_W4_OPERANDS); }
        }
        else if constexpr (TA == 0 && TB == 0) { asm volatile(CSM_W4_LOOP_00 CSM_W4_OPERANDS); }
        else if constexpr (TA == 0 && TB == 1) { asm volatile(CSM_W4_LOOP_01 CSM_W4_OPERANDS); }
        else if constexpr (TA == 1 && TB == 1) { asm volatile(CSM_W4_LOOP_11 CSM_W4_OPERANDS); }
        else { asm volatile(CSM_W4_LOOP_10 CSM_W4_OPERANDS); }
#undef CSM_W4_OPERANDS
        if (NJ == 8 && g.kx) {
            const int c8 = (lane >> 4) * 8, r16 = lane & 15;
            const int mb_ = m0 + wr * 128, nb_ = n0 + wc * 128;
            for (int k0 = 0; k0 < g.kx; k0 += 32) {
                bf16x8 fa[8], fb[8];
#pragma unroll
                for (int j = 0; j < 8; ++j)
                    fb[j] = *reinterpret_cast<const bf16x8*>(g.xB + (size_t)min(nb_ + 16 * j + r16, g.N - 1) * g.kx + k0 + c8);
#pragma unroll
                for (int i = 0; i < 8; ++i)
                    fa[i] = *reinterpret_cast<const bf16x8*>(g.xA + (size_t)min(mb_ + 16 * i + r16, g.M - 1) * g.kx + k0 + c8);
                asm volatile(CSM_W4_KEXT ::"v"(fa[0]), "v"(fa[1]), "v"(fa[2]), "v"(fa[3]), "v"(fa[4]), "v"(fa[5]), "v"(fa[6]), "v"(fa[7]),
                             "v"(fb[0]), "v"(fb[1]), "v"(fb[2]), "v"(fb[3]), "v"(fb[4]), "v"(fb[5]), "v"(fb[6]), "v"(fb[7])
                             : CSM_W4_KEXT_CLOBBERS);
            }
        }
        const int em0 = m0, en0 = n0;
        tile += stride;
        const bool more = tile < nwg;
        if (more) {
            coords(tile, m0, n0);
            prologue();
            asm volatile("" ::: "memory");
            __builtin_amdgcn_sched_barrier(0);
        }
        Epi e;
        e.C = reinterpret_cast<OutT*>(g.C) + (size_t)bz * g.sC;
        e.R = g.R ? g.R + (size_t)bz * g.sR : nullptr;
        e.ldc = g.ldc; e.ldr = g.ldr; e.alpha = g.alpha; e.mode = g.epi_mode; e.aux_in = g.aux_in; e.aux_out = g.aux_out;
        e.ld_aux = g.ld_aux; e.M = g.M; e.N = g.N; e.p0 = g.epi_p0; e.p1 = g.epi_p1;
        const bool vec_ok = ((g.ldc & 3) == 0) && (!e.R || (g.ldr & 3) == 0);
        const bool full = em0 + 256 <= g.M && en0 + TN <= g.N;
        pend = 0;
        int fastm = 0;
        if constexpr (sizeof(OutT) == 2) {
            const bool al = NJ == 8 && full && !e.R && (g.ldc & 7) == 0 && (reinterpret_cast<uintptr_t>(e.C) & 15) == 0 && g.fast_epi;
            if (al && e.mode == EPI_NONE) fastm = 1;
            else if (al && e.mode == EPI_SWIGLU_FWD && (e.ld_aux & 3) == 0 && (reinterpret_cast<uintptr_t>(e.aux_out) & 7) == 0) fastm = 2;
            else if (al && e.mode == EPI_SWIGLU_BWD && (e.ld_aux & 7) == 0 && (reinterpret_cast<uintptr_t>(e.aux_in) & 15) == 0) fastm = 3;
        }
        fastm = __builtin_amdgcn_readfirstlane(fastm);
        static_for<0, 2>([&](auto jh_) {
            constexpr int jh = decltype(jh_)::value;
            if constexpr (sizeof(OutT) == 2) {
                if (fastm) {
                    if (CSM_ABLATE_W4EPI & 8) return;
                    const int mb = __builtin_amdgcn_readfirstlane(em0 + wr * 128), nb = __builtin_amdgcn_readfirstlane(en0 + wc * (16 * NJ) + jh * 64);
                    if (fastm == 1) { w4_epi_plain<jh, false>(e, mb, nb, lane); pend += 16; }
                    else if (fastm == 2) { w4_epi_plain<jh, true>(e, mb, nb, lane); pend += 32; }
                    else if (jh == 0) { w4_epi_swiglu_bwd(e, mb, nb, lane); pend += 128; }
                    return;
                }
            }
            f32x4 acc[8][4];
            static_for<0, 8>([&](auto i_) {
                constexpr int i = decltype(i_)::value;
                static_for<0, 4>([&](auto j_) {
                    constexpr int j = decltype(j_)::value;
                    if constexpr (4 * jh + j < NJ) acc[i][j] = acc_read<(8 * i + 4 * jh + j) * 4>();
                });
            });
            const int mb = em0 + wr * 128, nb = en0 + wc * (16 * NJ) + jh * 64;
            bool swb = false;
            if constexpr (sizeof(OutT) == 2) swb = e.mode == EPI_SWIGLU_BWD;
            if constexpr (NJ == 6 && jh == 1) {
                pend += epi_block<OutT, 8, 1>(e, vec_ok, mb, nb, lane, acc);
            } else if (swb) {
                if constexpr (sizeof(OutT) == 2) epi_swiglu_bwd_block<8, 4>(e, mb, nb, lane, acc);
                pend += 32;
            } else {
                pend += epi_block<OutT, 8>(e, vec_ok, mb, nb, lane, acc);
            }
        });
        if (!full) pend = 0;
        if (!more) break;
    }
#undef CSM_W4_OFFS
}

template <int TA, int TB, typename OutT>
__global__ __launch_bounds__(256, 1) void gemm256w4_kernel(W4Args g) {
    extern __shared__ __attribute__((aligned(16))) char smem[];
    if (g.stagger_ticks > 0) {
        const unsigned grp = (blockIdx.x >> 3) % (unsigned)g.stagger_groups;
        if (grp) {
            const unsigned long long t0 = wall_clock64(), d = (unsigned long long)grp * (unsigned)g.stagger_ticks;
            while (wall_clock64() - t0 < d) __builtin_amdgcn_s_sleep(8);
        }
    }
    w4_tiles<TA, TB, OutT>(g, blockIdx.x, gridDim.x, blockIdx.z, smem);
}

template <int TA>
__global__ __launch_bounds__(256, 1) void gemm256w4n6_kernel(W4Args g) {
    extern __shared__ __attribute__((aligned(16))) char smem[];
    w4_tiles<TA, 0, bf16_t, 6>(g, blockIdx.x, gridDim.x, blockIdx.z, smem);
}

struct W4Two { W4Args a, b; int na; };
__global__ __launch_bounds__(256, 1) void gemm256w4_two_tn_kernel(W4Two p) {
    extern __shared__ __attribute__((aligned(16))) char smem[];
    if ((int)blockIdx.x < p.na) w4_tiles<1, 1, bf16_t>(p.a, blockIdx.x, 1 << 30, 0, smem);
    else w4_tiles<1, 1, bf16_t>(p.b, blockIdx.x - p.na, 1 << 30, 0, smem);
}

constexpr int W4_MULTI_MAX = 12;
struct W4Multi { W4Args p[W4_MULTI_MAX]; int start[W4_MULTI_MAX + 1]; int n; };
__global__ __launch_bounds__(256, 1) void gemm256w4_multi_tn_kernel(W4Multi m) {
    extern __shared__ __attribute__((aligned(16))) char smem[];
    int i = 0;
    while (i + 1 < m.n && (int)blockIdx.x >= m.start[i + 1]) ++i;
    i = __builtin_amdgcn_readfirstlane(i);
    w4_tiles<1, 1, bf16_t>(m.p[i], blockIdx.x - m.start[i], 1 << 30, 0, smem);
}

#define CSM_KNAMEW4(TA, TB, f32) \
    ((f32) ? (TA ? (TB ? "gemm256w4_kernel<1, 1, float>" : "gemm256w4_kernel<1, 0, float>") : (TB ? "gemm256w4_kernel<0, 1, float>" : "gemm256w4_kernel<0, 0, float>")) \
           : (TA ? (TB ? "gemm256w4_kernel<1, 1, unsigned short>" : "gemm256w4_kernel<1, 0, unsigned short>") : (TB ? "gemm256w4_kernel<0, 1, unsigned short>" : "gemm256w4_kernel<0, 0, unsigned short>")))

template <int TA, int TB>
int launch_w4(const W4Args& g, int out_f32, int batch, hipStream_t stream) {
    const int tiles = g.tiles_m * g.tiles_n;
    dim3 grid(g_persistent && tiles > 256 ? 256 : tiles, 1, batch), block(256);
    const size_t lds = 160 * 1024;
    if constexpr (TB == 0) {
        if (g.n6) {
            static bool done6 = false;
            auto k = gemm256w4n6_kernel<TA>;
            if (!done6) { (void)hipFuncSetAttribute((const void*)k, hipFuncAttributeMaxDynamicSharedMemorySize, (int)lds); done6 = true; }
            hipLaunchKernelGGL(k, grid, block, lds, stream, g);
            g_last_gemm_kernel = TA ? "gemm256w4n6_kernel<1>" : "gemm256w4n6_kernel<0>";
            CSM_CHECK_LAUNCH("csm_gemm_bf16(256 x 192 w4)");
            return 0;
        }
    }
    static bool done[2] = {false, false};
    if (out_f32) {
        auto k = gemm256w4_kernel<TA, TB, float>;
        if (!done[1]) { (void)hipFuncSetAttribute((const void*)k, hipFuncAttributeMaxDynamicSharedMemorySize, (int)lds); done[1] = true; }
        hipLaunchKernelGGL(k, grid, block, lds, stream, g);
    } else {
        auto k = gemm256w4_kernel<TA, TB, bf16_t>;
        if (!done[0]) { (void)hipFuncSetAttribute((const void*)k, hipFuncAttributeMaxDynamicSharedMemorySize, (int)lds); done[0] = true; }
        hipLaunchKernelGGL(k, grid, block, lds, stream, g);
    }
    g_last_gemm_kernel = CSM_KNAMEW4(TA, TB, out_f32);
    CSM_CHECK_LAUNCH("csm_gemm_bf16(256 w4)");
    return 0;
}

}

int csm_gemm256w4_launch(const void* A, const void* B, void* C, const void* R, int M, int N, int K, int lda, int ldb, int ldc, int ldr,
                         int transA, int transB, int out_f32, float alpha, int batch, long long sA, long long sB, long long sC,
                         long long sR, int epi_mode, const void* aux_in, void* aux_out, int ld_aux,
                         hipStream_t stream, int epi_p0, int epi_p1, const void* xA, const void* xB, int kx) {
    W4Args g;
    g.xA = (const bf16_t*)xA; g.xB = (const bf16_t*)xB; g.kx = kx;
    g.sA = sA; g.sB = sB; g.sC = sC; g.sR = sR;
    g.A = (const bf16_t*)A; g.B = (const bf16_t*)B; g.C = C; g.R = (const bf16_t*)R;
    g.M = M; g.N = N; g.K = K; g.lda = lda; g.ldb = ldb; g.ldc = ldc; g.ldr = ldr; g.alpha = alpha;
    g.tiles_m = (M + 255) / 256; g.tiles_n = (N + 255) / 256;
    g.n6 = 0;
    {
        const long long t8 = (long long)g.tiles_m * g.tiles_n, t6 = (long long)g.tiles_m * (N / 192);
        const bool ok = g_w4_n6 && !transB && !out_f32 && kx == 0 && N % 192 == 0 && (epi_mode == EPI_NONE || epi_mode == EPI_ROPE) && M % 256 == 0 && g_persistent;
        if (ok && 3 * ((t6 + 255) / 256) < 4 * ((t8 + 255) / 256)) { g.n6 = 1; g.tiles_n = N / 192; }
    }
    g.epi_mode = epi_mode; g.aux_in = (const bf16_t*)aux_in; g.aux_out = (bf16_t*)aux_out; g.ld_aux = ld_aux;
    g.epi_p0 = epi_p0; g.epi_p1 = epi_p1; g.touch = g_gemm_touch; g.fast_epi = g_w4_fast_epi;
    {
        const long long tiles = (long long)g.tiles_m * g.tiles_n;
        const int ticks = g_w4_stagger[epi_mode == EPI_SWIGLU_FWD ? 1 : epi_mode == EPI_SWIGLU_BWD ? 2 : 3];
        const bool on = g_persistent && g_w4_stagger[0] > 1 && ticks > 0 && tiles >= 768;
        g.stagger_groups = on ? g_w4_stagger[0] : 1; g.stagger_ticks = on ? ticks : 0;
    }
    if (!transA && !transB) return launch_w4<0, 0>(g, out_f32, batch, stream);
    if (!transA && transB) return launch_w4<0, 1>(g, out_f32, batch, stream);
    if (transA && transB) return launch_w4<1, 1>(g, out_f32, batch, stream);
    return launch_w4<1, 0>(g, out_f32, batch, stream);
}

static void fill_w4(W4Args& g, const void* A, const void* B, void* C, const void* R, int M, int N, int K, int lda, int ldb, int ldc, int ldr,
                    float alpha) {
    g.A = (const bf16_t*)A; g.B = (const bf16_t*)B; g.C = C; g.R = (const bf16_t*)R;
    g.M = M; g.N = N; g.K = K; g.lda = lda; g.ldb = ldb; g.ldc = ldc; g.ldr = ldr; g.alpha = alpha;
    g.sA = g.sB = g.sC = g.sR = 0;
    g.tiles_m = (M + 255) / 256; g.tiles_n = (N + 255) / 256;
    g.epi_mode = EPI_NONE; g.aux_in = nullptr; g.aux_out = nullptr; g.ld_aux = 0; g.epi_p0 = g.epi_p1 = 0; g.touch = 0;
    g.stagger_groups = 1; g.stagger_ticks = 0; g.fast_epi = g_w4_fast_epi;
    g.xA = g.xB = nullptr; g.kx = 0; g.n6 = 0;
}

int csm_gemm256w4_two_wgrad_launch(const void* dY1, const void* X1, void* dW1, int N1, int K1, int ld_dy1, int ldx1, int ld_dw1,
                                   const void* dY2, const void* X2, void* dW2, int N2, int K2, int ld_dy2, int ldx2, int ld_dw2,
                                   int M, int accumulate, float alpha, hipStream_t stream) {
    W4Two p;
    fill_w4(p.a, dY1, X1, dW1, accumulate ? dW1 : nullptr, N1, K1, M, ld_dy1, ldx1, ld_dw1, ld_dw1, alpha);
    fill_w4(p.b, dY2, X2, dW2, accumulate ? dW2 : nullptr, N2, K2, M, ld_dy2, ldx2, ld_dw2, ld_dw2, alpha);
    p.na = p.a.tiles_m * p.a.tiles_n;
    const int nb = p.b.tiles_m * p.b.tiles_n;
    static bool done = false;
    const size_t lds = 160 * 1024;
    if (!done) { (void)hipFuncSetAttribute((const void*)gemm256w4_two_tn_kernel, hipFuncAttributeMaxDynamicSharedMemorySize, (int)lds); done = true; }
    g_last_gemm_kernel = "gemm256w4_two_tn_kernel";
    hipLaunchKernelGGL(gemm256w4_two_tn_kernel, dim3(p.na + nb), dim3(256), lds, stream, p);
    CSM_CHECK_LAUNCH("csm_gemm_bf16_two_wgrad(w4)");
    return 0;
}

int csm_gemm256w4_multi_wgrad_launch(int n, const void* const* dY, const void* const* X, void* const* dW, const int* N, const int* K,
                                     const int* ld_dy, const int* ldx, const int* ld_dw, int M, int accumulate, float alpha,
                                     hipStream_t stream) {
    if (n < 1 || n > W4_MULTI_MAX) return -1;
    W4Multi p;
    p.n = n; p.start[0] = 0;
    for (int i = 0; i < n; ++i) {
        fill_w4(p.p[i], dY[i], X[i], dW[i], accumulate ? dW[i] : nullptr, N[i], K[i], M, ld_dy[i], ldx[i], ld_dw[i], ld_dw[i], alpha);
        p.start[i + 1] = p.start[i] + p.p[i].tiles_m * p.p[i].tiles_n;
    }
    for (int i = n; i < W4_MULTI_MAX; ++i) { p.p[i] = p.p[0]; p.start[i + 1] = p.start[n]; }
    static bool done = false;
    const size_t lds = 160 * 1024;
    if (!done) { (void)hipFuncSetAttribute((const void*)gemm256w4_multi_tn_kernel, hipFuncAttributeMaxDynamicSharedMemorySize, (int)lds); done = true; }
    g_last_gemm_kernel = "gemm256w4_multi_tn_kernel";
    hipLaunchKernelGGL(gemm256w4_multi_tn_kernel, dim3(p.start[n]), dim3(256), lds, stream, p);
    CSM_CHECK_LAUNCH("csm_gemm_bf16_multi_wgrad");
    return 0;
}
```

csm-train-pytorch_amd/csrc/gemm_common.h:

```cpp
#pragma once
#include "common.h"

namespace {

__device__ __forceinline__ int ks_swz(int kr) { return (kr & 3) | (((kr >> 3) & 1) << 2); }

constexpr int BM = 128, BN = 128, BK = 64;
constexpr int TILE_BYTES = 128 * 64 * 2;

struct GemmArgs {
    const bf16_t* A; const bf16_t* B; void* C; const bf16_t* R;
    int M, N, K, lda, ldb, ldc, ldr;
    long long sA, sB, sC, sR;
    float alpha;
    int tiles_m, tiles_n;
    int epi_mode; const bf16_t* aux_in; bf16_t* aux_out; int ld_aux;
    int epi_p0, epi_p1;
    const bf16_t* xA; const bf16_t* xB; int kx;
};

template <int T>
__device__ __forceinline__ void stage_load(const bf16_t* __restrict__ P, int ld, int rows , int K,
                                           int row0, int k0, U4 (&reg)[4]) {
    const int t = threadIdx.x;
// ... 143 lines not shown
                for (int ks = 0; ks < 2; ++ks) row[i][ks] = load_frag_row(img, r0 + 16 * i, ks, lane);
        } else {
            const unsigned base = (unsigned)(uintptr_t)img + tr_lane_off(lane);
            const int key = tr_lane_key(lane);
#pragma unroll
            for (int i = 0; i < NT; ++i) {
                const unsigned a = base + ((((r0 >> 4) + i) ^ key) << 5);
                tr[i][0] = load_frag_tr<0>(a);
                tr[i][1] = load_frag_tr<1>(a);
            }
        }
    }
    __device__ __forceinline__ bf16x8 get(int i, int ks) const {
        if constexpr (T == 0) return row[i][ks];
        else return cat4(tr[i][ks].lo, tr[i][ks].hi);
    }
};

__device__ __forceinline__ void store16_asm(void* p, const U4& v) {
    asm volatile("global_store_dwordx4 %0, %1, off\n\ts_nop 1" ::"v"(p), "v"(v) : "memory");
}
__device__ __forceinline__ void store8_asm(void* p, const uint2& v) {
    asm volatile("global_store_dwordx2 %0, %1, off" ::"v"(p), "v"(v) : "memory");
}
__device__ __forceinline__ void store4_asm(void* p, uint32_t v) {
    asm volatile("global_store_dword %0, %1, off" ::"v"(p), "v"(v) : "memory");
}
__device__ __forceinline__ void store2_asm(void* p, uint32_t v ) {
    asm volatile("global_store_short %0, %1, off" ::"v"(p), "v"(v) : "memory");
}

struct Epi {
    void* C; const bf16_t* R; int ldc, ldr; float alpha;
    int mode; const bf16_t* aux_in; bf16_t* aux_out; int ld_aux;
    int M, N;
    int p0, p1;
};
enum { EPI_NONE = 0, EPI_SWIGLU_FWD = 1, EPI_SWIGLU_BWD = 2, EPI_ROPE = 3 };

template <int NP>
__device__ __forceinline__ void epi_rope(const Epi& e, int m, int n, float* v) {
    if (n >= e.p0) return;
    const float* table = reinterpret_cast<const float*>(e.aux_in);
    const int pos = m % e.ld_aux, hd = e.p1;
    const float* t = table + ((size_t)pos * (hd >> 1) + ((n % hd) >> 1)) * 2;
#pragma unroll
    for (int i = 0; i < NP; i += 2) {
        const float4 cs = *reinterpret_cast<const float4*>(t + 2 * i);
        rope_rot(v[2 * i], v[2 * i + 1], cs.x, cs.y);
        rope_rot(v[2 * i + 2], v[2 * i + 3], cs.z, cs.w);
    }
}

template <typename OutT>
__device__ __forceinline__ void epi_store(const Epi& e, bool vec_ok, int m, int n, const f32x4& a) {
    float v[4] = {a[0] * e.alpha, a[1] * e.alpha, a[2] * e.alpha, a[3] * e.alpha};
    if (e.mode == EPI_SWIGLU_BWD) {
        if constexpr (sizeof(OutT) == 2) {
            float g[8], o[8];
            unpack8(*reinterpret_cast<const U4*>(e.aux_in + (size_t)m * e.ld_aux + 2 * n), g);
#pragma unroll
            for (int i = 0; i < 4; ++i) {
                const float gt = g[2 * i], up = g[2 * i + 1];
                const float sg = fast_sigmoid(gt);
                o[2 * i] = v[i] * up * sg * (1.f + gt * (1.f - sg));
                o[2 * i + 1] = v[i] * gt * sg;
            }
            store16_asm(reinterpret_cast<bf16_t*>(e.C) + (size_t)m * e.ldc + 2 * n, pack8(o));
        }
        return;
    }
    if (vec_ok && n + 3 < e.N) {
        if (e.R) {
            const uint2 r2 = *reinterpret_cast<const uint2*>(e.R + (size_t)m * e.ldr + n);
            v[0] += __uint_as_float(r2.x << 16); v[1] += __uint_as_float(r2.x & 0xffff0000u);
            v[2] += __uint_as_float(r2.y << 16); v[3] += __uint_as_float(r2.y & 0xffff0000u);
        }
        if (e.mode == EPI_ROPE) epi_rope<2>(e, m, n, v);
        if constexpr (sizeof(OutT) == 2) {
            uint2 o; o.x = pack2bf(v[0], v[1]); o.y = pack2bf(v[2], v[3]);
            store8_asm(reinterpret_cast<bf16_t*>(e.C) + (size_t)m * e.ldc + n, o);
            if (e.mode == EPI_SWIGLU_FWD) {
                const float a0 = silu(v[0]) * v[1];
                const float a1 = silu(v[2]) * v[3];
                store4_asm(e.aux_out + (size_t)m * e.ld_aux + (n >> 1), pack2bf(a0, a1));
            }
        } else {
            store16_asm(reinterpret_cast<float*>(e.C) + (size_t)m * e.ldc + n,
                        (U4){__float_as_uint(v[0]), __float_as_uint(v[1]), __float_as_uint(v[2]), __float_as_uint(v[3])});
        }
    } else {
        for (int k = 0; k < 4 && n + k < e.N; ++k) {
            float x = v[k];
            if (e.R) x += bf2f(e.R[(size_t)m * e.ldr + n + k]);
            if constexpr (sizeof(OutT) == 2) store2_asm(reinterpret_cast<bf16_t*>(e.C) + (size_t)m * e.ldc + n + k, f2bf(x));
            else store4_asm(reinterpret_cast<float*>(e.C) + (size_t)m * e.ldc + n + k, __float_as_uint(x));
        }
    }
}

#ifndef CSM_ABLATE_EPI
#define CSM_ABLATE_EPI 0
#endif
template <int NI, int NJ>
__device__ __forceinline__ void epi_swiglu_bwd_block(const Epi& e, int mb, int nb, int lane, const f32x4 (&acc)[NI][NJ]) {
    const int g = lane >> 4;
    bf16_t* C = reinterpret_cast<bf16_t*>(e.C);
    U4 gu[2][2][NJ];
    auto fetch = [&](int i, U4 (&dst)[2][NJ]) {
#pragma unroll
        for (int ii = 0; ii < 2; ++ii)
#pragma unroll
            for (int j = 0; j < NJ; ++j) {
                const int m = min(mb + 16 * (i + ii) + (lane & 15), e.M - 1), n = min(nb + 16 * j + 4 * g, e.N - 4);
                if (CSM_ABLATE_EPI & 1) dst[ii][j] = (U4){0x3f803f80u + (unsigned)m, 0x3f803f80u, 0x3f803f80u, 0x3f803f80u + (unsigned)n};
                else dst[ii][j] = *reinterpret_cast<const U4*>(e.aux_in + (size_t)m * e.ld_aux + 2 * n);
            }
    };
    fetch(0, gu[0]);
#pragma unroll
    for (int i = 0; i < NI; i += 2) {
        if (i + 2 < NI) fetch(i + 2, gu[((i >> 1) + 1) & 1]);
        const U4 (&cur)[2][NJ] = gu[(i >> 1) & 1];
#pragma unroll
        for (int ii = 0; ii < 2; ++ii)
#pragma unroll
            for (int j = 0; j < NJ; ++j) {
                const int m = mb + 16 * (i + ii) + (lane & 15), n = nb + 16 * j + 4 * g;
                float gv[8], o[8];
                unpack8(cur[ii][j], gv);
#pragma unroll
                for (int k = 0; k < 4; ++k) {
                    const float v = acc[i + ii][j][k] * e.alpha, gt = gv[2 * k], up = gv[2 * k + 1];
                    const float sg = (CSM_ABLATE_EPI & 4) ? gt : fast_sigmoid(gt);
                    o[2 * k] = v * up * sg * (1.f + gt * (1.f - sg));
                    o[2 * k + 1] = v * gt * sg;
                }
                if ((CSM_ABLATE_EPI & 2) ? (m < 0 && o[0] == 12345.f) : (m < e.M && n < e.N)) store16_asm(C + (size_t)m * e.ldc + 2 * n, pack8(o));
            }
    }
}

template <typename OutT>
__device__ __forceinline__ void epi_store_pair(const Epi& e, bool vec_ok, int m, int nb, int lane, const f32x4& a, const f32x4& b) {
    const int g = lane >> 4;
    bool wide = false;
    if constexpr (sizeof(OutT) == 2)
        wide = vec_ok && (e.mode == EPI_NONE || e.mode == EPI_ROPE || (e.mode == EPI_SWIGLU_FWD && (e.ld_aux & 3) == 0)) && (e.ldc & 7) == 0 &&
               (!e.R || (e.ldr & 7) == 0) && nb + 31 < e.N && ((reinterpret_cast<uintptr_t>(e.C) & 15) == 0) &&
               (!e.R || (reinterpret_cast<uintptr_t>(e.R) & 15) == 0);
    if (!wide) {
        const int n = nb + 4 * g;
        if (m < e.M && n < e.N) epi_store<OutT>(e, vec_ok, m, n, a);
        if (m < e.M && n + 16 < e.N) epi_store<OutT>(e, vec_ok, m, n + 16, b);
        return;
    }
    float v[8];
#pragma unroll
    for (int k = 0; k < 4; ++k) {
        auto r = __builtin_amdgcn_permlane16_swap(__float_as_uint(a[k]), __float_as_uint(b[k]), false, false);
        v[k] = __uint_as_float(r[0]) * e.alpha;
        v[4 + k] = __uint_as_float(r[1]) * e.alpha;
    }
    if (m >= e.M) return;
    const int n = nb + ((g & 1) ? 16 + 4 * (g - 1) : 4 * g);
    if (e.R) {
        float rr[8];
        unpack8(*reinterpret_cast<const U4*>(e.R + (size_t)m * e.ldr + n), rr);
#pragma unroll
        for (int k = 0; k < 8; ++k) v[k] += rr[k];
    }
    if (e.mode == EPI_ROPE) epi_rope<4>(e, m, n, v);
    store16_asm(reinterpret_cast<bf16_t*>(e.C) + (size_t)m * e.ldc + n, pack8(v));
    if (e.mode == EPI_SWIGLU_FWD) {
        float a[4];
#pragma unroll
        for (int k = 0; k < 4; ++k) a[k] = silu(v[2 * k]) * v[2 * k + 1];
        uint2 w; w.x = pack2bf(a[0], a[1]); w.y = pack2bf(a[2], a[3]);
        store8_asm(e.aux_out + (size_t)m * e.ld_aux + (n >> 1), w);
    }
}

template <typename OutT, int NI, int NJP = 2>
__device__ __forceinline__ int epi_block(const Epi& e, bool vec_ok, int mb, int nb, int lane, const f32x4 (&acc)[NI][4]) {
    bool fast = false;
    if constexpr (sizeof(OutT) == 2)
        fast = vec_ok && (e.mode == EPI_NONE || (e.mode == EPI_ROPE && (e.p0 & 63) == 0 && (e.p1 & 7) == 0) ||
                          (e.mode == EPI_SWIGLU_FWD && (e.ld_aux & 3) == 0)) &&
               (e.ldc & 7) == 0 && (!e.R || (e.ldr & 7) == 0) && nb + 32 * NJP - 1 < e.N && ((reinterpret_cast<uintptr_t>(e.C) & 15) == 0) &&
               (!e.R || (reinterpret_cast<uintptr_t>(e.R) & 15) == 0);
    if (!fast) {
#pragma unroll
        for (int i = 0; i < NI; ++i) {
            const int m = mb + 16 * i + (lane & 15);
#pragma unroll
            for (int jp = 0; jp < NJP; ++jp) epi_store_pair<OutT>(e, vec_ok, m, nb + 32 * jp, lane, acc[i][2 * jp], acc[i][2 * jp + 1]);
        }
        return 0;
    }
    if constexpr (sizeof(OutT) == 2) {
        const int g = lane >> 4;
        const int nl = nb + ((g & 1) ? 16 + 4 * (g - 1) : 4 * g);
        const int ml = mb + (lane & 15);
        bf16_t* C = reinterpret_cast<bf16_t*>(e.C);
        auto gather = [&](int i, int jp, float (&v)[8]) {
#pragma unroll
            for (int k = 0; k < 4; ++k) {
                auto r = __builtin_amdgcn_permlane16_swap(__float_as_uint(acc[i][2 * jp][k]), __float_as_uint(acc[i][2 * jp + 1][k]), false, false);
                v[k] = __uint_as_float(r[0]) * e.alpha;
                v[4 + k] = __uint_as_float(r[1]) * e.alpha;
            }
        };
        if (e.mode == EPI_ROPE && nb < e.p0) {
            float4 cs[2][2][2][2];
            auto rope_fetch = [&](int i, float4 (&dst)[2][2][2]) {
                const float* table = reinterpret_cast<const float*>(e.aux_in);
#pragma unroll
                for (int ii = 0; ii < 2; ++ii)
#pragma unroll
                    for (int jp = 0; jp < NJP; ++jp) {
                        const int pos = (ml + 16 * (i + ii)) % e.ld_aux, n = nl + 32 * jp;
                        const float* t = table + ((size_t)pos * (e.p1 >> 1) + ((n % e.p1) >> 1)) * 2;
                        dst[ii][jp][0] = *reinterpret_cast<const float4*>(t);
                        dst[ii][jp][1] = *reinterpret_cast<const float4*>(t + 4);
                    }
            };
            rope_fetch(0, cs[0]);
#pragma unroll
            for (int i = 0; i < NI; ++i) {
                if ((i & 1) == 0 && i + 2 < NI) rope_fetch(i + 2, cs[((i >> 1) + 1) & 1]);
                const int m = ml + 16 * i;
#pragma unroll
                for (int jp = 0; jp < NJP; ++jp) {
                    float v[8];
                    gather(i, jp, v);
                    const int n = nl + 32 * jp;
                    if (e.R && m < e.M) {
                        float f[8];
                        unpack8(*reinterpret_cast<const U4*>(e.R + (size_t)m * e.ldr + n), f);
#pragma unroll
                        for (int k = 0; k < 8; ++k) v[k] += f[k];
                    }
                    const float4 (&q)[2] = cs[(i >> 1) & 1][i & 1][jp];
                    if (nb + 32 * jp < e.p0)
#pragma unroll
                    for (int h = 0; h < 2; ++h) {
                        rope_rot(v[4 * h], v[4 * h + 1], q[h].x, q[h].y);
                        rope_rot(v[4 * h + 2], v[4 * h + 3], q[h].z, q[h].w);
                    }
                    if (m < e.M) store16_asm(C + (size_t)m * e.ldc + n, pack8(v));
                }
            }
            return NJP * NI;
        }
        U4 rr[NI][2];
        if (e.R) {
#pragma unroll
            for (int i = 0; i < NI; ++i)
#pragma unroll
                for (int jp = 0; jp < NJP; ++jp)
                    rr[i][jp] = *reinterpret_cast<const U4*>(e.R + (size_t)min(ml + 16 * i, e.M - 1) * e.ldr + nl + 32 * jp);
        }
#pragma unroll
        for (int i = 0; i < NI; ++i) {
            const int m = ml + 16 * i;
#pragma unroll
            for (int jp = 0; jp < NJP; ++jp) {
                float v[8];
                gather(i, jp, v);
                if (e.R) {
                    float f[8];
                    unpack8(rr[i][jp], f);
#pragma unroll
                    for (int k = 0; k < 8; ++k) v[k] += f[k];
                }
                const int n = nl + 32 * jp;
                if (m < e.M) {
                    store16_asm(C + (size_t)m * e.ldc + n, pack8(v));
                    if (e.mode == EPI_SWIGLU_FWD) {
                        float a[4];
#pragma unroll
                        for (int k = 0; k < 4; ++k) a[k] = silu(v[2 * k]) * v[2 * k + 1];
                        uint2 w; w.x = pack2bf(a[0], a[1]); w.y = pack2bf(a[2], a[3]);
                        store8_asm(e.aux_out + (size_t)m * e.ld_aux + (n >> 1), w);
                    }
                }
            }
        }
        return NJP * NI * (1 + (e.mode == EPI_SWIGLU_FWD ? 1 : 0));
    }
    return 0;
}

template <int NI>
__device__ __forceinline__ void k_extend(const bf16_t* __restrict__ xA, const bf16_t* __restrict__ xB, int kx, int M, int N, int mb,
                                         int nb, int lane, f32x4 (&acc)[NI][4]) {
    const int c = (lane >> 4) * 8;
    for (int k0 = 0; k0 < kx; k0 += 32) {
        bf16x8 fa[NI], fb[4];
#pragma unroll
        for (int j = 0; j < 4; ++j)
            fb[j] = *reinterpret_cast<const bf16x8*>(xB + (size_t)min(nb + 16 * j + (lane & 15), N - 1) * kx + k0 + c);
#pragma unroll
        for (int i = 0; i < NI; ++i)
            fa[i] = *reinterpret_cast<const bf16x8*>(xA + (size_t)min(mb + 16 * i + (lane & 15), M - 1) * kx + k0 + c);
#pragma unroll
        for (int i = 0; i < NI; ++i)
#pragma unroll
            for (int j = 0; j < 4; ++j) acc[i][j] = __builtin_amdgcn_mfma_f32_16x16x32_bf16(fb[j], fa[i], acc[i][j], 0, 0, 0);
    }
}

}
```

csm-train-pytorch_amd/csrc/ops.hip:

```cpp
#include "common.h"
#include <math.h>

namespace {

template <int NC>
__global__ __launch_bounds__(256) void rmsnorm_fwd_kernel(const bf16_t* __restrict__ x, const bf16_t* __restrict__ w,
                                                          bf16_t* __restrict__ y, float* __restrict__ rstd, int M, int D,
                                                          float eps) {
    const int lane = threadIdx.x & 63;
    const int wpb = blockDim.x >> 6;
    const int nchunk = D >> 3;
    for (long long row = (long long)blockIdx.x * wpb + (threadIdx.x >> 6); row < M; row += (long long)gridDim.x * wpb) {
        U4 v[NC];
        float ss = 0.f;
#pragma unroll
        for (int i = 0; i < NC; ++i) {
            const int c = lane + 64 * i;
            v[i] = (U4){0u, 0u, 0u, 0u};
            if (c < nchunk) v[i] = *reinterpret_cast<const U4*>(x + (size_t)row * D + c * 8);
            float f[8];
            unpack8(v[i], f);
#pragma unroll
            for (int j = 0; j < 8; ++j) ss += f[j] * f[j];
        }
        ss = wave_sum(ss);
        const float r = rsqrtf(ss / (float)D + eps);
        if (lane == 0 && rstd) rstd[row] = r;
#pragma unroll
        for (int i = 0; i < NC; ++i) {
            const int c = lane + 64 * i;
            if (c < nchunk) {
                float f[8], s[8];
                unpack8(v[i], f);
                unpack8(*reinterpret_cast<const U4*>(w + c * 8), s);
#pragma unroll
                for (int j = 0; j < 8; ++j) f[j] = f[j] * r * s[j];
                *reinterpret_cast<U4*>(y + (size_t)row * D + c * 8) = pack8(f);
            }
        }
    }
}

template <int NC>
__global__ __launch_bounds__(512) void rmsnorm_bwd_kernel(const bf16_t* __restrict__ x, const bf16_t* __restrict__ w,
                                                          const float* __restrict__ rstd, const bf16_t* __restrict__ dy,
                                                          const bf16_t* __restrict__ dres, bf16_t* __restrict__ dx,
                                                          float* __restrict__ dw_acc, int M, int D) {
    extern __shared__ __attribute__((aligned(16))) char smem_dw[];
    const int lane = threadIdx.x & 63;
    const int wpb = blockDim.x >> 6;
    const int nchunk = D >> 3;
    float dwl[NC][8];
#pragma unroll
    for (int i = 0; i < NC; ++i)
// ... 217 lines not shown
        float g[8];
        unpack8(*reinterpret_cast<const U4*>(gu + (size_t)row * 2 * F + c * 8), g);
        uint2 o;
        o.x = pack2bf(silu(g[0]) * g[1], silu(g[2]) * g[3]);
        o.y = pack2bf(silu(g[4]) * g[5], silu(g[6]) * g[7]);
        *reinterpret_cast<uint2*>(out + (size_t)row * F + c * 4) = o;
    }
}

__global__ __launch_bounds__(256) void swiglu_bwd_kernel(const bf16_t* __restrict__ gu, const bf16_t* __restrict__ dout,
                                                         bf16_t* __restrict__ dgu, long long M, int F) {
    const int cpr = F >> 2;
    const long long total = M * cpr;
    for (long long idx = (long long)blockIdx.x * blockDim.x + threadIdx.x; idx < total;
         idx += (long long)gridDim.x * blockDim.x) {
        const long long row = idx / cpr;
        const int c = (int)(idx % cpr);
        float g[8], o[8];
        unpack8(*reinterpret_cast<const U4*>(gu + (size_t)row * 2 * F + c * 8), g);
        const uint2 d2 = *reinterpret_cast<const uint2*>(dout + (size_t)row * F + c * 4);
        const float d[4] = {__uint_as_float(d2.x << 16), __uint_as_float(d2.x & 0xffff0000u), __uint_as_float(d2.y << 16),
                            __uint_as_float(d2.y & 0xffff0000u)};
#pragma unroll
        for (int i = 0; i < 4; ++i) {
            const float gt = g[2 * i], up = g[2 * i + 1];
            const float sg = fast_sigmoid(gt);
            o[2 * i] = d[i] * up * sg * (1.f + gt * (1.f - sg));
            o[2 * i + 1] = d[i] * gt * sg;
        }
        *reinterpret_cast<U4*>(dgu + (size_t)row * 2 * F + c * 8) = pack8(o);
    }
}

__global__ __launch_bounds__(256) void embed_fwd_kernel(const long long* __restrict__ tokens, const uint8_t* __restrict__ mask,
                                                        const bf16_t* __restrict__ text_emb, const bf16_t* __restrict__ audio_emb,
                                                        bf16_t* __restrict__ out, int K, int D, int audio_vocab) {
    const long long row = blockIdx.x;
    const long long* tok = tokens + row * (K + 1);
    const uint8_t* mk = mask + row * (K + 1);
    for (int c0 = threadIdx.x * 8; c0 < D; c0 += blockDim.x * 8) {
        float acc[8] = {0.f, 0.f, 0.f, 0.f, 0.f, 0.f, 0.f, 0.f};
        for (int s = 0; s <= K; ++s) {
            if (!mk[s]) continue;
            const bf16_t* src = (s < K) ? audio_emb + ((size_t)tok[s] + (size_t)s * audio_vocab) * D : text_emb + (size_t)tok[s] * D;
            float f[8];
            unpack8(*reinterpret_cast<const U4*>(src + c0), f);
#pragma unroll
            for (int j = 0; j < 8; ++j) acc[j] += f[j];
        }
        *reinterpret_cast<U4*>(out + (size_t)row * D + c0) = pack8(acc);
    }
}

template <int NC>
__global__ __launch_bounds__(256) void embed_bwd_sorted_kernel(const long long* __restrict__ rows, const long long* __restrict__ src,
                                                               long long n_occ, const bf16_t* __restrict__ dh,
                                                               const bf16_t* __restrict__ dseq, long long M,
                                                               bf16_t* __restrict__ g_text, bf16_t* __restrict__ g_audio,
                                                               long long text_rows, long long n_rows, int D) {
    const int lane = threadIdx.x & 63;
    const long long i = (long long)blockIdx.x * (blockDim.x >> 6) + (threadIdx.x >> 6);
    if (i >= n_occ) return;
    const long long r = rows[i];
    if (r >= n_rows || (i > 0 && rows[i - 1] == r)) return;
    float acc[NC][8];
#pragma unroll
    for (int c = 0; c < NC; ++c)
#pragma unroll
        for (int j = 0; j < 8; ++j) acc[c][j] = 0.f;
    const int nchunk = D >> 3;
    for (long long k = i; k < n_occ && rows[k] == r; ++k) {
        const long long sidx = src[k];
        const bf16_t* p = sidx < M ? dh + (size_t)sidx * D : dseq + (size_t)(sidx - M) * D;
#pragma unroll
        for (int c = 0; c < NC; ++c) {
            const int ch = lane + 64 * c;
            if (ch < nchunk) {
                float f[8];
                unpack8(*reinterpret_cast<const U4*>(p + ch * 8), f);
#pragma unroll
                for (int j = 0; j < 8; ++j) acc[c][j] += f[j];
            }
        }
    }
    bf16_t* dst = r < text_rows ? g_text + (size_t)r * D : g_audio + (size_t)(r - text_rows) * D;
#pragma unroll
    for (int c = 0; c < NC; ++c) {
        const int ch = lane + 64 * c;
        if (ch < nchunk) {
            float f[8];
            unpack8(*reinterpret_cast<const U4*>(dst + ch * 8), f);
#pragma unroll
            for (int j = 0; j < 8; ++j) f[j] += acc[c][j];
            *reinterpret_cast<U4*>(dst + ch * 8) = pack8(f);
        }
    }
}

__global__ __launch_bounds__(256) void rows_add_kernel(bf16_t* __restrict__ dst, const int* __restrict__ rows,
                                                       const bf16_t* __restrict__ src, long long N, int src_stride_rows, int D) {
    const int lane = threadIdx.x & 63;
    const long long n = (long long)blockIdx.x * (blockDim.x >> 6) + (threadIdx.x >> 6);
    if (n >= N) return;
    if (rows[n] < 0) return;
    bf16_t* d = dst + (size_t)rows[n] * D;
    const bf16_t* s = src + (size_t)n * src_stride_rows * D;
    for (int c0 = lane * 8; c0 < D; c0 += 512) {
        float a[8], b[8];
        unpack8(*reinterpret_cast<const U4*>(d + c0), a);
        unpack8(*reinterpret_cast<const U4*>(s + c0), b);
#pragma unroll
        for (int j = 0; j < 8; ++j) a[j] += b[j];
        *reinterpret_cast<U4*>(d + c0) = pack8(a);
    }
}

__global__ __launch_bounds__(256) void rows_take_kernel(bf16_t* __restrict__ table, const int* __restrict__ rows,
                                                        bf16_t* __restrict__ out, long long N, int D) {
    const int lane = threadIdx.x & 63;
    const long long n = (long long)blockIdx.x * (blockDim.x >> 6) + (threadIdx.x >> 6);
    if (n >= N) return;
    const int r = rows[n];
    bf16_t* o = out + (size_t)n * D;
    const U4 z = {0u, 0u, 0u, 0u};
    for (int c0 = lane * 8; c0 < D; c0 += 512) {
        if (r < 0) { *reinterpret_cast<U4*>(o + c0) = z; continue; }
        bf16_t* t = table + (size_t)r * D + c0;
        *reinterpret_cast<U4*>(o + c0) = *reinterpret_cast<const U4*>(t);
        *reinterpret_cast<U4*>(t) = z;
    }
}

__global__ __launch_bounds__(256) void decoder_input_kernel(const bf16_t* __restrict__ hidden, const int* __restrict__ rows,
                                                            const long long* __restrict__ codes ,
                                                            const bf16_t* __restrict__ audio_emb, bf16_t* __restrict__ out,
                                                            int K, int D, int audio_vocab) {
    const long long n = blockIdx.x / K;
    const int i = blockIdx.x % K;
    const bf16_t* src = (i == 0) ? hidden + (size_t)rows[n] * D
                                 : audio_emb + ((size_t)codes[n * K + i - 1] + (size_t)(i - 1) * audio_vocab) * D;
    for (int c0 = threadIdx.x * 8; c0 < D; c0 += blockDim.x * 8)
        *reinterpret_cast<U4*>(out + ((size_t)n * K + i) * D + c0) = *reinterpret_cast<const U4*>(src + c0);
}

__global__ __launch_bounds__(256) void ce_kernel(const float* __restrict__ logits, const long long* __restrict__ targets,
                                                 float* __restrict__ loss_rows, bf16_t* __restrict__ dlogits, int V, int ldl,
                                                 int ldd, float gscale) {
    __shared__ float red[16];
// ... 62 lines not shown
#pragma unroll
        for (int i = 0; i < NC; ++i) {
            const int c = (lane + 64 * i) * 4;
            if (c < ldd) {
                float g[4];
#pragma unroll
                for (int j = 0; j < 4; ++j) g[j] = c + j < V ? (__expf(v[i][j] - lse) - (c + j == t ? 1.f : 0.f)) * gscale : 0.f;
                uint2 o; o.x = pack2bf(g[0], g[1]); o.y = pack2bf(g[2], g[3]);
                *reinterpret_cast<uint2*>(dlogits + (size_t)row * ldd + c) = o;
            }
        }
    }
}

__global__ __launch_bounds__(1024) void reduce_sum_kernel(const float* __restrict__ x, long long n, float scale,
                                                          float* __restrict__ out) {
    __shared__ float red[16];
    float acc = 0.f;
    for (long long i = threadIdx.x; i < n; i += blockDim.x) acc += x[i];
    acc = block_sum(acc, red);
    if (threadIdx.x == 0) out[0] = acc * scale;
}

__global__ __launch_bounds__(256) void sumsq_kernel(const bf16_t* __restrict__ g, long long n, float* __restrict__ partials) {
    __shared__ float red[16];
    float acc = 0.f;
    const long long nvec = n >> 3;
    const long long stride = (long long)gridDim.x * blockDim.x;
    long long i = (long long)blockIdx.x * blockDim.x + threadIdx.x;
    for (; i + 3 * stride < nvec; i += 4 * stride) {
        const U4 q0 = *reinterpret_cast<const U4*>(g + i * 8), q1 = *reinterpret_cast<const U4*>(g + (i + stride) * 8);
        const U4 q2 = *reinterpret_cast<const U4*>(g + (i + 2 * stride) * 8), q3 = *reinterpret_cast<const U4*>(g + (i + 3 * stride) * 8);
        float f0[8], f1[8], f2[8], f3[8];
        unpack8(q0, f0); unpack8(q1, f1); unpack8(q2, f2); unpack8(q3, f3);
#pragma unroll
        for (int j = 0; j < 8; ++j) acc += f0[j] * f0[j];
#pragma unroll
        for (int j = 0; j < 8; ++j) acc += f1[j] * f1[j];
#pragma unroll
        for (int j = 0; j < 8; ++j) acc += f2[j] * f2[j];
#pragma unroll
        for (int j = 0; j < 8; ++j) acc += f3[j] * f3[j];
    }
    for (; i < nvec; i += stride) {
        float f[8];
        unpack8(*reinterpret_cast<const U4*>(g + i * 8), f);
#pragma unroll
        for (int j = 0; j < 8; ++j) acc += f[j] * f[j];
    }
    if (blockIdx.x == 0)
        for (long long i = (nvec << 3) + threadIdx.x; i < n; i += blockDim.x) { const float f = bf2f(g[i]); acc += f * f; }
    acc = block_sum(acc, red);
    if (threadIdx.x == 0) partials[blockIdx.x] = acc;
}

__global__ __launch_bounds__(1024) void clip_coef_kernel(const float* __restrict__ partials, int n, float max_norm,
                                                         float* __restrict__ out) {
    __shared__ float red[16];
    float acc = 0.f;
    for (int i = threadIdx.x; i < n; i += blockDim.x) acc += partials[i];
    acc = block_sum(acc, red);
    if (threadIdx.x == 0) {
        const float norm = sqrtf(acc);
        out[0] = norm;
        out[1] = (max_norm > 0.f) ? fminf(1.f, max_norm / (norm + 1e-6f)) : 1.f;
    }
}

__device__ __forceinline__ float adam_decay(float p, float lr, float wd) {
#pragma clang fp contract(off)
    return p * (1.f - lr * wd);
}

__device__ __forceinline__ float adam_moments(float& m, float& v, float g, float lr, float beta1, float beta2, float eps, float bc1,
                                              float bc2_sqrt) {
#pragma clang fp contract(off)
    m = beta1 * m + (1.f - beta1) * g;
    v = beta2 * v + ((1.f - beta2) * g) * g;
    const float denom = sqrtf(v) / bc2_sqrt + eps;
    return (lr / bc1) * (m / denom);
}

__device__ __forceinline__ void adam_update(float& p, float& m, float& v, float g, float lr, float beta1, float beta2, float eps,
                                            float wd, float bc1, float bc2_sqrt) {
#pragma clang fp contract(off)
    p = adam_decay(p, lr, wd);
    p = p - adam_moments(m, v, g, lr, beta1, beta2, eps, bc1, bc2_sqrt);
}

__device__ __forceinline__ void adamw_skipped(bf16_t* __restrict__ grad, long long nvec, int zero_grad) {
    if (!zero_grad) return;
    for (long long i = (long long)blockIdx.x * blockDim.x + threadIdx.x; i < nvec; i += (long long)gridDim.x * blockDim.x)
        *reinterpret_cast<U4*>(grad + i * 8) = (U4){0u, 0u, 0u, 0u};
}

struct AdamArgs {
    float lr, beta1, beta2, eps, wd, bc1, bc2_sqrt, coef;
    int zero_grad;
};

__device__ __forceinline__ void adamw_vec(float* __restrict__ master, float* __restrict__ m, float* __restrict__ v,
                                          bf16_t* __restrict__ param, bf16_t* __restrict__ grad, long long i, const AdamArgs& a) {
    float g[8];
    unpack8(*reinterpret_cast<const U4*>(grad + i * 8), g);
    float4 p0 = *reinterpret_cast<const float4*>(master + i * 8), p1 = *reinterpret_cast<const float4*>(master + i * 8 + 4);
    float4 m0 = *reinterpret_cast<const float4*>(m + i * 8), m1 = *reinterpret_cast<const float4*>(m + i * 8 + 4);
// ... 157 lines not shown
                continue;
            }
            if (threadIdx.x == 0) block_live[b] = 1;
        }
        if (in) adamw_split_vec(lo, m, v, param, grad, i, a);
    }
}

inline int grid_for(long long work_items, int block, int cap = 256 * 8) {
    long long b = (work_items + block - 1) / block;
    if (b < 1) b = 1;
    return (int)(b > cap ? cap : b);
}

}

extern "C" int csm_rmsnorm_fwd(const void* x, const void* scale, void* y, float* rstd, int M, int D, float eps,
                               hipStream_t stream) {
    CSM_REQUIRE(x && scale && y, "csm_rmsnorm_fwd: null pointer");
    CSM_REQUIRE(M > 0 && D > 0 && (D & 7) == 0 && D <= 4096, "csm_rmsnorm_fwd: D=%d must be a multiple of 8 and <= 4096", D);
    const int grid = grid_for(M, 4, 4096);
    const int nc = (D + 511) / 512;
#define L(NC) hipLaunchKernelGGL((rmsnorm_fwd_kernel<NC>), dim3(grid), dim3(256), 0, stream, (const bf16_t*)x, (const bf16_t*)scale, (bf16_t*)y, rstd, M, D, eps)
    if (nc <= 1) L(1); else if (nc <= 2) L(2); else if (nc <= 4) L(4); else L(8);
#undef L
    CSM_CHECK_LAUNCH("csm_rmsnorm_fwd");
    return 0;
}

#define CSM_RMSNORM_BWD_BLOCKS 256
extern "C" int csm_rmsnorm_bwd_blocks(void) { return CSM_RMSNORM_BWD_BLOCKS; }

extern "C" int csm_rmsnorm_bwd(const void* x, const void* scale, const float* rstd, const void* dy, const void* dres,
                               void* dx, float* dscale_partials, int M, int D, hipStream_t stream) {
    CSM_REQUIRE(x && scale && rstd && dy && dx, "csm_rmsnorm_bwd: null pointer");
    CSM_REQUIRE(M > 0 && D > 0 && (D & 7) == 0 && D <= 4096, "csm_rmsnorm_bwd: D=%d must be a multiple of 8 and <= 4096", D);
    const int grid = CSM_RMSNORM_BWD_BLOCKS;
    const int nc = (D + 511) / 512;
    const size_t lds = dscale_partials ? (size_t)8 * D * sizeof(float) : 0;
    if (lds > 65536) {
        static bool done = false;
        if (!done) (void)hipFuncSetAttribute((const void*)rmsnorm_bwd_kernel<8>, hipFuncAttributeMaxDynamicSharedMemorySize, (int)(8 * 4096 * sizeof(float)));
        done = true;
    }
#define L(NC) hipLaunchKernelGGL((rmsnorm_bwd_kernel<NC>), dim3(grid), dim3(512), lds, stream, (const bf16_t*)x, (const bf16_t*)scale, rstd, (const bf16_t*)dy, (const bf16_t*)dres, (bf16_t*)dx, dscale_partials, M, D)
    if (nc <= 1) L(1); else if (nc <= 2) L(2); else if (nc <= 4) L(4); else L(8);
#undef L
    CSM_CHECK_LAUNCH("csm_rmsnorm_bwd");
    return 0;
}

extern "C" int csm_colsum_bf16(const float* partials, int rows, int D, void* dst, int accumulate, hipStream_t stream) {
    CSM_REQUIRE(partials && dst && rows > 0 && D > 0, "csm_colsum_bf16: bad arguments");
    hipLaunchKernelGGL(colsum_kernel, dim3((D + 63) / 64), dim3(rows >= 64 ? 1024 : 256), 0, stream, partials, rows, D, (bf16_t*)dst,
                       accumulate);
    CSM_CHECK_LAUNCH("csm_colsum_bf16");
    return 0;
}

extern "C" int csm_colsum_bf16_multi(int n, const float* const* partials, void* const* dst, int rows, int D, int accumulate,
                                     hipStream_t stream) {
    CSM_REQUIRE(n >= 1 && n <= 8 && partials && dst && rows > 0 && D > 0, "csm_colsum_bf16_multi: 1..8 pairs, rows, D > 0");
    ColsumMulti p;
    for (int i = 0; i < 8; ++i) {
        CSM_REQUIRE(i >= n || (partials[i] && dst[i]), "csm_colsum_bf16_multi: null pointer in pair %d", i);
        p.partials[i] = partials[i < n ? i : 0]; p.dst[i] = (bf16_t*)dst[i < n ? i : 0];
    }
    hipLaunchKernelGGL(colsum_multi_kernel, dim3((D + 63) / 64, n), dim3(rows >= 64 ? 1024 : 256), 0, stream, p, rows, D, accumulate);
    CSM_CHECK_LAUNCH("csm_colsum_bf16_multi");
    return 0;
}

extern "C" int csm_dropout_bf16(const void* in, int ld_in, void* out, int ld_out, long long M, int D, float p,
                                unsigned long long seed, int accumulate, hipStream_t stream) {
    CSM_REQUIRE(in && out && M > 0 && D > 0 && D % 8 == 0 && ld_in % 8 == 0 && ld_out % 8 == 0 && ld_in >= D && ld_out >= D,
                "csm_dropout_bf16: bad arguments (D and strides must be multiples of 8)");
    CSM_REQUIRE(p >= 0.f && p < 1.f, "csm_dropout_bf16: p must be in [0, 1)");
    const uint32_t thresh = (uint32_t)(p * 65536.0f + 0.5f);
    const long long total = M * (D / 8);
    const int blocks = (int)std::min<long long>((total + 255) / 256, 8192);
    hipLaunchKernelGGL(dropout_kernel, dim3(blocks), dim3(256), 0, stream, (const bf16_t*)in, ld_in, (bf16_t*)out, ld_out, M, D,
                       thresh, 1.0f / (1.0f - thresh / 65536.0f), (uint64_t)seed, accumulate);
    CSM_CHECK_LAUNCH("csm_dropout_bf16");
    return 0;
}

extern "C" int csm_bias_add_bf16(void* y, int ld, const void* bias, long long M, int D, hipStream_t stream) {
    CSM_REQUIRE(y && bias && M > 0 && D > 0 && D % 8 == 0 && ld % 8 == 0 && ld >= D, "csm_bias_add_bf16: bad arguments");
    const long long total = M * (D / 8);
    const int blocks = (int)std::min<long long>((total + 255) / 256, 8192);
    hipLaunchKernelGGL(bias_add_kernel, dim3(blocks), dim3(256), 0, stream, (bf16_t*)y, ld, (const bf16_t*)bias, M, D);
    CSM_CHECK_LAUNCH("csm_bias_add_bf16");
    return 0;
}

extern "C" int csm_colsum_rows_bf16(const void* x, int ld, long long M, int D, float* partials, int slices, hipStream_t stream) {
    CSM_REQUIRE(x && partials && M > 0 && D > 0 && ld >= D && slices > 0 && slices <= 65535, "csm_colsum_rows_bf16: bad arguments");
    hipLaunchKernelGGL(colsum_rows_kernel, dim3((D + 63) / 64, slices), dim3(256), 0, stream, (const bf16_t*)x, ld, M, D, partials);
    CSM_CHECK_LAUNCH("csm_colsum_rows_bf16");
    return 0;
}

extern "C" int csm_rope(void* qkv, const float* table, const int* pos, long long M, int S, int n_heads_qk, int head_dim,
                        int ld, int inverse, hipStream_t stream) {
    CSM_REQUIRE(qkv && table, "csm_rope: null pointer");
    CSM_REQUIRE(M > 0 && S > 0 && n_heads_qk > 0 && (head_dim & 7) == 0 && (ld & 7) == 0, "csm_rope: bad shape");
    const long long total = M * n_heads_qk * (head_dim >> 3);
    hipLaunchKernelGGL(rope_kernel, dim3(grid_for(total, 256, 8192)), dim3(256), 0, stream, (bf16_t*)qkv, table, pos, M, S,
                       n_heads_qk, head_dim, ld, inverse);
    CSM_CHECK_LAUNCH("csm_rope");
    return 0;
}

extern "C" int csm_swiglu_fwd(const void* gu, void* out, long long M, int F, hipStream_t stream) {
    CSM_REQUIRE(gu && out && M > 0 && F > 0 && (F & 7) == 0, "csm_swiglu_fwd: bad arguments");
    hipLaunchKernelGGL(swiglu_fwd_kernel, dim3(grid_for(M * (F >> 2), 256, 8192)), dim3(256), 0, stream, (const bf16_t*)gu,
                       (bf16_t*)out, M, F);
    CSM_CHECK_LAUNCH("csm_swiglu_fwd");
    return 0;
}

extern "C" int csm_swiglu_bwd(const void* gu, const void* dout, void* dgu, long long M, int F, hipStream_t stream) {
    CSM_REQUIRE(gu && dout && dgu && M > 0 && F > 0 && (F & 7) == 0, "csm_swiglu_bwd: bad arguments");
    hipLaunchKernelGGL(swiglu_bwd_kernel, dim3(grid_for(M * (F >> 2), 256, 8192)), dim3(256), 0, stream, (const bf16_t*)gu,
                       (const bf16_t*)dout, (bf16_t*)dgu, M, F);
    CSM_CHECK_LAUNCH("csm_swiglu_bwd");
    return 0;
}

extern "C" int csm_embed_fwd(const long long* tokens, const uint8_t* mask, const void* text_emb, const void* audio_emb,
                             void* out, long long M, int K, int D, int audio_vocab, hipStream_t stream) {
    CSM_REQUIRE(tokens && mask && text_emb && audio_emb && out, "csm_embed_fwd: null pointer");
    CSM_REQUIRE(M > 0 && M < (1ll << 31) && K > 0 && (D & 7) == 0, "csm_embed_fwd: bad shape");
    hipLaunchKernelGGL(embed_fwd_kernel, dim3((unsigned)M), dim3(256), 0, stream, tokens, mask, (const bf16_t*)text_emb,
                       (const bf16_t*)audio_emb, (bf16_t*)out, K, D, audio_vocab);
    CSM_CHECK_LAUNCH("csm_embed_fwd");
    return 0;
}

extern "C" int csm_embed_bwd_sorted(const long long* sorted_rows, const long long* src_index, long long n_occ, const void* dh,
                                    const void* dseq, long long M, void* g_text, void* g_audio, long long text_rows,
                                    long long n_rows, int D, hipStream_t stream) {
    CSM_REQUIRE(sorted_rows && src_index && dh && g_text && g_audio && n_occ > 0, "csm_embed_bwd_sorted: bad arguments");
    CSM_REQUIRE((D & 7) == 0 && D <= 4096, "csm_embed_bwd_sorted: D=%d must be a multiple of 8 and <= 4096", D);
    const long long blocks = (n_occ + 3) / 4;
    CSM_REQUIRE(blocks < (1ll << 31), "csm_embed_bwd_sorted: too many occurrences");
    const int nc = (D + 511) / 512;
#define L(NC) hipLaunchKernelGGL((embed_bwd_sorted_kernel<NC>), dim3((unsigned)blocks), dim3(256), 0, stream, sorted_rows, src_index, n_occ, (const bf16_t*)dh, (const bf16_t*)dseq, M, (bf16_t*)g_text, (bf16_t*)g_audio, text_rows, n_rows, D)
    if (nc <= 1) L(1); else if (nc <= 2) L(2); else if (nc <= 4) L(4); else L(8);
#undef L
    CSM_CHECK_LAUNCH("csm_embed_bwd_sorted");
    return 0;
}

extern "C" int csm_rows_add_bf16(void* dst, const int* rows, const void* src, long long N, int src_stride_rows, int D,
                                 hipStream_t stream) {
    CSM_REQUIRE(dst && rows && src && N > 0 && (D & 7) == 0 && src_stride_rows > 0, "csm_rows_add_bf16: bad arguments");
    hipLaunchKernelGGL(rows_add_kernel, dim3((unsigned)((N + 3) / 4)), dim3(256), 0, stream, (bf16_t*)dst, rows, (const bf16_t*)src,
                       N, src_stride_rows, D);
    CSM_CHECK_LAUNCH("csm_rows_add_bf16");
    return 0;
}

extern "C" int csm_rows_take_bf16(void* table, const int* rows, void* out, long long N, int D, hipStream_t stream) {
    CSM_REQUIRE(table && rows && out && N > 0 && (D & 7) == 0, "csm_rows_take_bf16: bad arguments");
    hipLaunchKernelGGL(rows_take_kernel, dim3((unsigned)((N + 3) / 4)), dim3(256), 0, stream, (bf16_t*)table, rows, (bf16_t*)out, N, D);
    CSM_CHECK_LAUNCH("csm_rows_take_bf16");
    return 0;
}

extern "C" int csm_decoder_input_fwd(const void* hidden, const int* rows, const long long* codes, const void* audio_emb,
                                     void* out, long long N, int K, int D, int audio_vocab, hipStream_t stream) {
    CSM_REQUIRE(hidden && rows && codes && audio_emb && out && N > 0 && N * K < (1ll << 31) && (D & 7) == 0,
                "csm_decoder_input_fwd: bad arguments");
    hipLaunchKernelGGL(decoder_input_kernel, dim3((unsigned)(N * K)), dim3(256), 0, stream, (const bf16_t*)hidden, rows, codes,
                       (const bf16_t*)audio_emb, (bf16_t*)out, K, D, audio_vocab);
    CSM_CHECK_LAUNCH("csm_decoder_input_fwd");
    return 0;
}

extern "C" int csm_ce_fwd_bwd(const float* logits, const long long* targets, float* loss_rows, void* dlogits, long long R,
                              int V, int ldl, int ldd, float grad_scale, hipStream_t stream) {
    CSM_REQUIRE(logits && targets && loss_rows && R > 0 && R < (1ll << 31) && V > 0 && ldl >= V, "csm_ce_fwd_bwd: bad arguments");
    CSM_REQUIRE(!dlogits || ldd >= V, "csm_ce_fwd_bwd: ldd < V");
    const int width = ldl > ldd && dlogits ? ldl : (dlogits ? ldd : ldl);
    const bool vec = (ldl & 3) == 0 && ((uintptr_t)logits & 15) == 0 && (!dlogits || ((ldd & 3) == 0 && ((uintptr_t)dlogits & 7) == 0 && ldd <= ldl + 0));
    if (vec && width <= 256 * 12) {
        const dim3 grid((unsigned)((R + 3) / 4)), block(256);
#define L(NC) hipLaunchKernelGGL((ce_wave_kernel<NC>), grid, block, 0, stream, logits, targets, loss_rows, (bf16_t*)dlogits, R, V, ldl, ldd, grad_scale)
        if (width <= 256 * 4) L(4); else if (width <= 256 * 9) L(9); else L(12);
#undef L
    } else {
        hipLaunchKernelGGL(ce_kernel, dim3((unsigned)R), dim3(256), 0, stream, logits, targets, loss_rows, (bf16_t*)dlogits, V, ldl,
                           ldd, grad_scale);
    }
    CSM_CHECK_LAUNCH("csm_ce_fwd_bwd");
    return 0;
}

extern "C" int csm_reduce_sum_f32(const float* x, long long n, float scale, float* out, hipStream_t stream) {
    CSM_REQUIRE(x && out && n > 0, "csm_reduce_sum_f32: bad arguments");
    hipLaunchKernelGGL(reduce_sum_kernel, dim3(1), dim3(1024), 0, stream, x, n, scale, out);
    CSM_CHECK_LAUNCH("csm_reduce_sum_f32");
    return 0;
}

#define CSM_SUMSQ_BLOCKS 8192
extern "C" int csm_sumsq_blocks(void) { return CSM_SUMSQ_BLOCKS; }

extern "C" int csm_sumsq_bf16(const void* g, long long n, float* partials, hipStream_t stream) {
    CSM_REQUIRE(g && partials && n > 0 && ((uintptr_t)g & 15) == 0, "csm_sumsq_bf16: bad arguments");
    hipLaunchKernelGGL(sumsq_kernel, dim3(CSM_SUMSQ_BLOCKS), dim3(256), 0, stream, (const bf16_t*)g, n, partials);
    CSM_CHECK_LAUNCH("csm_sumsq_bf16");
    return 0;
}

extern "C" int csm_clip_coef(const float* partials, int n_partials, float max_norm, float* norm_and_coef,
                             hipStream_t stream) {
    CSM_REQUIRE(partials && norm_and_coef && n_partials > 0, "csm_clip_coef: bad arguments");
    hipLaunchKernelGGL(clip_coef_kernel, dim3(1), dim3(1024), 0, stream, partials, n_partials, max_norm, norm_and_coef);
    CSM_CHECK_LAUNCH("csm_clip_coef");
    return 0;
}

static int g_adamw_blocks = 1 << 20;
extern "C" int csm_set_adamw_blocks(int b) { g_adamw_blocks = b; return 0; }

extern "C" int csm_adamw_step(float* master, float* m, float* v, void* param, void* grad, long long n, float lr,
                              float beta1, float beta2, float eps, float weight_decay, int step,
                              const float* norm_and_coef, float grad_mul, int zero_grad, hipStream_t stream) {
    CSM_REQUIRE(master && m && v && param && grad && n > 0 && step > 0, "csm_adamw_step: bad arguments");
    CSM_REQUIRE((n & 7) == 0, "csm_adamw_step: n must be a multiple of 8 (pad the arena)");
    const float bc1 = 1.f - powf(beta1, (float)step);
    const float bc2s = sqrtf(1.f - powf(beta2, (float)step));
    hipLaunchKernelGGL(adamw_kernel, dim3(grid_for(n >> 3, 256, g_adamw_blocks)), dim3(256), 0, stream, master, m, v, (bf16_t*)param,
                       (bf16_t*)grad, n, lr, beta1, beta2, eps, weight_decay, bc1, bc2s, norm_and_coef, grad_mul, zero_grad);
    CSM_CHECK_LAUNCH("csm_adamw_step");
    return 0;
}

extern "C" int csm_adamw_step_split(void* master_lo, float* m, float* v, void* param, void* grad, long long n, float lr, float beta1,
                                    float beta2, float eps, float weight_decay, int step, const float* norm_and_coef, float grad_mul,
                                    int zero_grad, hipStream_t stream) {
    CSM_REQUIRE(master_lo && m && v && param && grad && n > 0 && step >= 1, "csm_adamw_step_split: bad arguments");
    CSM_REQUIRE((n & 7) == 0, "csm_adamw_step_split: n must be a multiple of 8 (pad the arena)");
    const float bc1 = 1.f - powf(beta1, (float)step);
    const float bc2s = sqrtf(1.f - powf(beta2, (float)step));
    hipLaunchKernelGGL(adamw_split_kernel, dim3(grid_for(n >> 3, 256, g_adamw_blocks)), dim3(256), 0, stream, (uint16_t*)master_lo, m, v,
                       (bf16_t*)param, (bf16_t*)grad, n, lr, beta1, beta2, eps, weight_decay, bc1, bc2s, norm_and_coef, grad_mul, zero_grad);
    CSM_CHECK_LAUNCH("csm_adamw_step_split");
    return 0;
}

extern "C" int csm_adamw_step_live(float* master, float* m, float* v, void* param, void* grad, long long n, float lr,
                                   float beta1, float beta2, float eps, float weight_decay, int step,
                                   const float* norm_and_coef, float grad_mul, int zero_grad, void* block_live, hipStream_t stream) {
    CSM_REQUIRE(master && m && v && param && grad && block_live && n > 0 && step > 0, "csm_adamw_step_live: bad arguments");
    CSM_REQUIRE((n & 7) == 0, "csm_adamw_step_live: n must be a multiple of 8 (pad the arena)");
    const float bc1 = 1.f - powf(beta1, (float)step);
    const float bc2s = sqrtf(1.f - powf(beta2, (float)step));
    hipLaunchKernelGGL(adamw_live_kernel, dim3(grid_for(n >> 3, 256, g_adamw_blocks)), dim3(256), 0, stream, master, m, v, (bf16_t*)param,
                       (bf16_t*)grad, n, lr, beta1, beta2, eps, weight_decay, bc1, bc2s, norm_and_coef, grad_mul, zero_grad,
                       (uint8_t*)block_live);
    CSM_CHECK_LAUNCH("csm_adamw_step_live");
    return 0;
}
// ... 16 lines not shown
```

include/csm_hip.h:

```cpp
#ifndef CSM_HIP_H
#define CSM_HIP_H
#include <stdint.h>

#ifdef __cplusplus
extern "C" {
#endif

typedef struct ihipStream_t* csm_stream_t;

int csm_abi_version(void);
const char* csm_last_error(void);
int csm_device_check(int device);

int csm_gemm_bf16(const void* A, const void* B, void* C, const void* R, int M, int N, int K, int lda, int ldb, int ldc,
                  int ldr, int transA, int transB, int out_f32, float alpha, int batch, long long strideA,
                  long long strideB, long long strideC, long long strideR, csm_stream_t stream);

int csm_gemm_bf16_ex(const void* A, const void* B, void* C, const void* R, int M, int N, int K, int lda, int ldb, int ldc,
                     int ldr, int transA, int transB, int out_f32, float alpha, int batch, long long strideA,
                     long long strideB, long long strideC, long long strideR, int epilogue, const void* aux_in,
                     void* aux_out, int ld_aux, csm_stream_t stream);
int csm_gemm_bf16_rope(const void* A, const void* W, void* C, int M, int N, int K, int lda, int ldw, int ldc,
                       const float* rope_table, int rows_per_seq, int n_rope_cols, int head_dim, csm_stream_t stream);
int csm_gemm_bf16_kext(const void* A, const void* B, void* C, const void* R, int M, int N, int K, int lda, int ldb, int ldc, int ldr,
// ... 11 lines not shown
                              int accumulate, float alpha_w, csm_stream_t stream);
int csm_gemm_bf16_two_wgrad(const void* dY1, const void* X1, void* dW1, int N1, int K1, int ld_dy1, int ldx1, int ld_dw1,
                            const void* dY2, const void* X2, void* dW2, int N2, int K2, int ld_dy2, int ldx2, int ld_dw2,
                            int M, int accumulate, float alpha, csm_stream_t stream);
int csm_gemm_bf16_multi_wgrad(int n, const void* const* dY, const void* const* X, void* const* dW, const int* N, const int* K,
                              const int* ld_dy, const int* ldx, const int* ld_dw, int M, int accumulate, float alpha,
                              csm_stream_t stream);


int csm_set_gemm_variant(int v);
int csm_set_gemm256_persistent(int v);
int csm_get_gemm256_persistent(void);
int csm_set_gemm_tuning(int key, int value);
const char* csm_gemm_last_kernel(void);

int csm_rmsnorm_fwd(const void* x, const void* scale, void* y, float* rstd, int M, int D, float eps, csm_stream_t stream);
int csm_rmsnorm_bwd_blocks(void);
int csm_rmsnorm_bwd(const void* x, const void* scale, const float* rstd, const void* dy, const void* dres, void* dx,
                    float* dscale_partials , int M, int D, csm_stream_t stream);
int csm_colsum_bf16(const float* partials, int rows, int D, void* dst, int accumulate, csm_stream_t stream);
int csm_colsum_bf16_multi(int n, const float* const* partials, void* const* dst, int rows, int D, int accumulate, csm_stream_t stream);

int csm_dropout_bf16(const void* in, int ld_in, void* out, int ld_out, long long M, int D, float p, unsigned long long seed,
                     int accumulate, csm_stream_t stream);
int csm_bias_add_bf16(void* y, int ld, const void* bias, long long M, int D, csm_stream_t stream);
int csm_colsum_rows_bf16(const void* x, int ld, long long M, int D, float* partials , int slices,
                         csm_stream_t stream);

int csm_rope(void* qkv, const float* table, const int* pos, long long M, int S, int n_heads_qk, int head_dim, int ld,
             int inverse, csm_stream_t stream);

int csm_set_attn_variant(int v);
int csm_attn_fwd(const void* qkv, void* out, float* lse, int B, int S, int H, int KV, int HD, csm_stream_t stream);
long long csm_attn_bwd_workspace_bytes(int B, int S, int H);
int csm_attn_bwd(const void* qkv, const void* out, const void* dout, const float* lse, void* dqkv,
                 float* delta_ws , int B, int S, int H, int KV, int HD, csm_stream_t stream);
int csm_attn_bwd_rope(const void* qkv, const void* out, const void* dout, const float* lse, void* dqkv, float* delta_ws,
                      const float* rope_table, int B, int S, int H, int KV, int HD, csm_stream_t stream);
int csm_attn_last_dkv_kernel(void);
int csm_attn_fwd_seg(const void* qkv, void* out, float* lse, const int* seg_start, int B, int S, int H, int KV, int HD, csm_stream_t stream);
int csm_attn_bwd_seg(const void* qkv, const void* out, const void* dout, const float* lse, void* dqkv, float* delta_ws,
                     const int* seg_start, const int* seg_end, int B, int S, int H, int KV, int HD, csm_stream_t stream);
int csm_attn64_set_debug(void* device_buffer);

int csm_swiglu_fwd(const void* gu, void* out, long long M, int F, csm_stream_t stream);
int csm_swiglu_bwd(const void* gu, const void* dout, void* dgu, long long M, int F, csm_stream_t stream);

int csm_embed_fwd(const long long* tokens, const uint8_t* mask, const void* text_emb, const void* audio_emb, void* out,
                  long long M, int K, int D, int audio_vocab, csm_stream_t stream);

int csm_embed_bwd_sorted(const long long* sorted_rows, const long long* src_index, long long n_occ, const void* dh,
                         const void* dseq, long long M, void* g_text, void* g_audio, long long text_rows, long long n_rows,
                         int D, csm_stream_t stream);
int csm_rows_add_bf16(void* dst, const int* rows, const void* src, long long N, int src_stride_rows, int D, csm_stream_t stream);
int csm_rows_take_bf16(void* table, const int* rows, void* out, long long N, int D, csm_stream_t stream);

int csm_decoder_input_fwd(const void* hidden, const int* rows, const long long* codes, const void* audio_emb, void* out,
                          long long N, int K, int D, int audio_vocab, csm_stream_t stream);

int csm_ce_fwd_bwd(const float* logits, const long long* targets, float* loss_rows, void* dlogits, long long R, int V,
                   int ldl, int ldd, float grad_scale, csm_stream_t stream);
int csm_reduce_sum_f32(const float* x, long long n, float scale, float* out, csm_stream_t stream);

int csm_sumsq_blocks(void);
int csm_sumsq_bf16(const void* g, long long n, float* partials , csm_stream_t stream);
int csm_clip_coef(const float* partials, int n_partials, float max_norm, float* norm_and_coef , csm_stream_t stream);
int csm_adamw_step(float* master, float* m, float* v, void* param, void* grad, long long n, float lr, float beta1,
                   float beta2, float eps, float weight_decay, int step, const float* norm_and_coef ,
                   float grad_mul, int zero_grad , csm_stream_t stream);
int csm_adamw_step_split(void* master_lo, float* m, float* v, void* param, void* grad, long long n, float lr, float beta1,
                         float beta2, float eps, float weight_decay, int step, const float* norm_and_coef, float grad_mul,
                         int zero_grad, csm_stream_t stream);
int csm_adamw_step_live(float* master, float* m, float* v, void* param, void* grad, long long n, float lr, float beta1,
                        float beta2, float eps, float weight_decay, int step, const float* norm_and_coef, float grad_mul,
                        int zero_grad, void* block_live, csm_stream_t stream);
int csm_adamw_step_split_live(void* master_lo, float* m, float* v, void* param, void* grad, long long n, float lr, float beta1,
                              float beta2, float eps, float weight_decay, int step, const float* norm_and_coef, float grad_mul,
                              int zero_grad, void* block_live, csm_stream_t stream);

int csm_set_adamw_blocks(int blocks);

int csm_sample_topk(const float* logits, const float* q, int* out, int rows, int V, int ldl, int topk, float temperature,
                    csm_stream_t stream);
int csm_sample_topk_rows(const float* logits, const float* q, int* out, int rows, int V, int ldl, const int* topk,
                         const float* temperature, csm_stream_t stream);
int csm_sample_filtered_rows(const float* logits, const float* q, int* out, int rows, int V, int ldl, const int* topk,
                             const float* temperature, const float* top_p, const float* min_p, csm_stream_t stream);

int csm_set_decode_tuning(int key, int value);
int csm_gemv_bf16(const void* x, const void* W, void* y, const void* residual, int B, int N, int K, int ldw, int ldx, int ldy,
                  int out_f32, csm_stream_t stream);
int csm_gemv_bf16_ex(const void* x, const void* W, void* y, const void* residual, int B, int N, int K, int ldw, int ldx, int ldy,
                     int out_f32, const void* norm_scale, float eps, int swiglu, const int* row_index, int row_offset,
                     csm_stream_t stream);
int csm_quantize_rows_fp8(const void* W, void* W8, void* scale, int N, int K, int ldw, int ldw8, csm_stream_t stream);
int csm_gemv_fp8w(const void* x, const void* W8, const void* scale, void* y, const void* residual, int B, int N, int K, int ldw8,
                  int ldx, int ldy, int out_f32, const void* norm_scale, float eps, int swiglu, const int* row_index, int row_offset,
                  csm_stream_t stream);
int csm_lora_project_bf16(const void* x, const void* At, void* t, int B, int K, int kx, int ldx, int lda, int ldt, float scale,
                          const void* norm_scale, float eps, csm_stream_t stream);
int csm_gemv_bf16_kext(const void* x, const void* W, void* y, const void* residual, int B, int N, int K, int ldw, int ldx, int ldy,
                       int out_f32, const void* norm_scale, float eps, int swiglu, const int* row_index, int row_offset,
                       const void* ext_t, const void* ext_B, int kx, int ld_ext_t, int ld_ext_B, const void* bias,
                       csm_stream_t stream);
int csm_lora_project_rows_bf16(const void* x, const void* const* At, void* t, const int* row_adapter, const float* scale,
                               int n_adapters, int B, int K, int kx, int ldx, int lda, int ldt, const void* norm_scale, float eps,
                               csm_stream_t stream);
int csm_gemv_bf16_kext_rows(const void* x, const void* W, void* y, const void* residual, int B, int N, int K, int ldw, int ldx,
                            int ldy, int out_f32, const void* norm_scale, float eps, int swiglu, const int* row_index, int row_offset,
                            const void* ext_t, const void* const* ext_B, const void* const* bias, const int* row_adapter,
                            int n_adapters, int kx, int ld_ext_t, int ld_ext_B, csm_stream_t stream);
int csm_gemv_t_bf16(const void* x, const void* W, void* y, int B, int N, int K, int ldw, int ldx, int ldy, int out_f32,
                    csm_stream_t stream);
int csm_gemv_attn_bf16(const void* qkv, void* kcache, void* vcache, const int* pos, const float* rope_table, const void* W, void* y,
                       const void* residual, int B, int N, int H, int KV, int HD, int S_max, int ld_qkv, int ldw, int ldy,
                       csm_stream_t stream);
int csm_attn_decode_rope_at(const void* qkv, void* kcache, void* vcache, void* out, int pos, const float* rope_table, int B, int H,
                            int KV, int HD, int S_max, int ld, csm_stream_t stream);
int csm_gemv_attn_at_bf16(const void* qkv, void* kcache, void* vcache, int pos, const float* rope_table, const void* W, void* y,
// ... 67 lines not shown
```

Before: 129,600.

## Fold gradient-norm sum-of-squares into wgrad and embedding backward kernels

Registers each weight-gradient matrix with per-tile sum-of-squares slots that the GEMM and embedding-backward kernels are meant to fill as they write gradients. At clip time the optimizer reduces only those slots plus a multi-range pass over unregistered gaps, instead of re-reading the whole gradient arena. The goal is to remove a full extra memory pass over all bf16 gradients per step. The trade-off is freshness-tracking complexity (touch, invalidate and collect bookkeeping) and extra epilogue work inside the GEMMs. Any missed invalidation would produce a wrong norm.

```diff
diff --git a/csm-train-pytorch_amd/csm/engine.py b/csm-train-pytorch_amd/csm/engine.py
--- a/csm-train-pytorch_amd/csm/engine.py
+++ b/csm-train-pytorch_amd/csm/engine.py
@@ -638,11 +638,13 @@
             acc[g_] = gst[g_] == "live"
             if gst[g_] == "stale" and (not w_ or g_ == "embeddings"):
                 o_, n_ = m.group_range(g_)
+                ops.grad_norm_invalidate()
                 m.grad_arena[o_:o_ + n_].zero_()
                 gst[g_] = "zero"
             if w_:
                 gst[g_] = "live"
         if train_other and not acc["other"] and not dec_runs:
+            ops.grad_slots_touch(m.block("projection.weight", True))
             m.block("projection.weight", True).zero_()
             m.block("audio_head.padded", True).zero_()
         hidden = s["hidden"]
@@ -689,11 +691,11 @@
         dh0 = self.backbone.backward(dhid, B, S, tr["backbone"], 1.0, on_layer_done=self.grad_hook, acc=acc["backbone"], seg=s.get("seg"),
                                     sel=s.get("sel"))
         if train_embeddings:
-            self._embedding_backward(s, dh0, dseq if (dec is not None and s["aw"] != 0.0) else None)
+            self._embedding_backward(s, dh0, dseq if (dec is not None and s["aw"] != 0.0) else None, zero_tables=not acc["embeddings"])
         if self.grad_hook is not None:
             self.grad_hook("embeddings", -1)
 
-    def _embedding_backward(self, s, dh0, dseq):
+    def _embedding_backward(self, s, dh0, dseq, zero_tables=False):
         m, a = self.m, self.m.args
         dev = m.device
         K, V = a.audio_num_codebooks, a.audio_vocab_size
@@ -726,8 +728,11 @@
         else:
             order = torch.argsort(rows, stable=True)
             rows_s, src_s = rows[order].contiguous(), src[order].contiguous()
+        fold = ops.grad_fold
+        slots = (fold.embed_slots(rows_s.numel(), dev)
+                 if zero_tables and fold.owner is not None and fold.arena_ptr == m.grad_arena.data_ptr() else None)
         ops.embed_bwd_sorted(rows_s, src_s, dh0, dseq,
-                             m.block("text_embeddings.weight", True), m.block("audio_embeddings.weight", True))
+                             m.block("text_embeddings.weight", True), m.block("audio_embeddings.weight", True), sumsq_slots=slots)
 
     @torch.no_grad()
     def hidden_states(self, tokens: torch.Tensor, masks: torch.Tensor) -> torch.Tensor:
diff --git a/csm-train-pytorch_amd/csm/hip/__init__.py b/csm-train-pytorch_amd/csm/hip/__init__.py
--- a/csm-train-pytorch_amd/csm/hip/__init__.py
+++ b/csm-train-pytorch_amd/csm/hip/__init__.py
@@ -69,6 +69,19 @@
     "csm_sumsq_blocks": ([], _i),
     "csm_sumsq_bf16": ([_p, _ll, _p, _p], _i),
     "csm_clip_coef": ([_p, _i, _f, _p, _p], _i),
+    "csm_sumsq_max_ranges": ([], _i),
+    "csm_sumsq_ranges_bf16": ([_p, _p, _i, _p, _p], _i),
+    "csm_sumsq_launch_count": ([], C.c_ulonglong),
+    "csm_clip_max_lists": ([], _i),
+    "csm_clip_coef_lists": ([_p, _p, _i, _f, _p, _p], _i),
+    "csm_embed_bwd_sumsq_slots": ([_ll], _ll),
+    "csm_embed_bwd_sorted_sumsq": ([_p, _p, _ll, _p, _p, _ll, _p, _p, _ll, _ll, _i, _p, _p], _i),
+    "csm_grad_slots_count": ([_i, _i], _i),
+    "csm_grad_slots_register": ([_p, _i, _i, _i, _p], _i),
+    "csm_grad_slots_clear": ([], _i),
+    "csm_grad_slots_invalidate": ([], _i),
+    "csm_grad_slots_touch": ([_p], _i),
+    "csm_grad_slots_collect": ([_p, _i], _i),
     "csm_adamw_step": ([_p, _p, _p, _p, _p, _ll, _f, _f, _f, _f, _f, _i, _p, _f, _i, _p], _i),
     "csm_adamw_step_split": ([_p, _p, _p, _p, _p, _ll, _f, _f, _f, _f, _f, _i, _p, _f, _i, _p], _i),
     "csm_adamw_step_live": ([_p, _p, _p, _p, _p, _ll, _f, _f, _f, _f, _f, _i, _p, _f, _i, _p, _p], _i),
diff --git a/csm-train-pytorch_amd/csm/hip/ops.py b/csm-train-pytorch_amd/csm/hip/ops.py
--- a/csm-train-pytorch_amd/csm/hip/ops.py
+++ b/csm-train-pytorch_amd/csm/hip/ops.py
@@ -332,8 +332,18 @@
     return out
 
 
-def embed_bwd_sorted(sorted_rows, src_index, dh, dseq, g_text, g_audio):
+def embed_bwd_sorted(sorted_rows, src_index, dh, dseq, g_text, g_audio, sumsq_slots=None):
     assert sorted_rows.dtype == torch.int64 and src_index.dtype == torch.int64 and sorted_rows.is_contiguous() and src_index.is_contiguous()
+    if sumsq_slots is not None:
+        n = embed_bwd_sumsq_slots(sorted_rows.numel())
+        assert sumsq_slots.dtype == torch.float32 and sumsq_slots.is_contiguous() and sumsq_slots.numel() >= n
+        check(lib.csm_embed_bwd_sorted_sumsq(sorted_rows.data_ptr(), src_index.data_ptr(), sorted_rows.numel(), dh.data_ptr(), _ptr(dseq),
+                                             dh.shape[0], g_text.data_ptr(), g_audio.data_ptr(), g_text.shape[0],
+                                             g_text.shape[0] + g_audio.shape[0], dh.shape[1], sumsq_slots.data_ptr(), _stream()),
+              "csm_embed_bwd_sorted_sumsq")
+        grad_fold.embed = (g_text.data_ptr(), sumsq_slots[:n])
+        return
+    grad_fold.embed = None
     check(lib.csm_embed_bwd_sorted(sorted_rows.data_ptr(), src_index.data_ptr(), sorted_rows.numel(), dh.data_ptr(), _ptr(dseq),
                                    dh.shape[0], g_text.data_ptr(), g_audio.data_ptr(), g_text.shape[0],
                                    g_text.shape[0] + g_audio.shape[0], dh.shape[1], _stream()), "csm_embed_bwd_sorted")
@@ -381,6 +391,93 @@
 
 def clip_coef(partials, max_norm, norm_and_coef):
     check(lib.csm_clip_coef(partials.data_ptr(), partials.numel(), float(max_norm), norm_and_coef.data_ptr(), _stream()), "csm_clip_coef")
+
+
+class _GradFold:
+    owner = None
+    arena_ptr = 0
+    slots = None
+    n = 0
+    embed = None
+    _embed_buf = None
+
+    def embed_slots(self, n_occ: int, device) -> torch.Tensor:
+        n = embed_bwd_sumsq_slots(n_occ)
+        if self._embed_buf is None or self._embed_buf.numel() < n or self._embed_buf.device != device:
+            self._embed_buf = torch.zeros(n, dtype=torch.float32, device=device)
+        return self._embed_buf
+
+
+grad_fold = _GradFold()
+
+
+def embed_bwd_sumsq_slots(n_occ: int) -> int:
+    return lib.csm_embed_bwd_sumsq_slots(n_occ)
+
+
+def grad_slots_count(rows: int, cols: int) -> int:
+    return lib.csm_grad_slots_count(rows, cols)
+
+
+def grad_slots_clear():
+    lib.csm_grad_slots_clear()
+    grad_fold.owner, grad_fold.arena_ptr, grad_fold.slots, grad_fold.n, grad_fold.embed = None, 0, None, 0, None
+
+
+def grad_slots_register(ptr: int, rows: int, cols: int, ld: int, slots: torch.Tensor, slot_offset: int) -> int:
+    assert slots.dtype == torch.float32 and slots.is_contiguous() and slot_offset + grad_slots_count(rows, cols) <= slots.numel()
+    assert grad_fold.slots is None or grad_fold.slots is slots, "one slot buffer per registration table"
+    i = lib.csm_grad_slots_register(ptr, rows, cols, ld, slots.data_ptr() + 4 * slot_offset)
+    if i < 0:
+        raise CsmHipError("csm_grad_slots_register: " + lib.csm_last_error().decode("utf-8", "replace"))
+    grad_fold.slots, grad_fold.n = slots, i + 1
+    return i
+
+
+def grad_norm_invalidate():
+    lib.csm_grad_slots_invalidate()
+    grad_fold.embed = None
+
+
+def grad_slots_touch(t: torch.Tensor):
+    lib.csm_grad_slots_touch(t.data_ptr())
+
+
+def grad_slots_collect():
+    n = grad_fold.n
+    buf = (ctypes.c_ubyte * max(1, n))()
+    got = lib.csm_grad_slots_collect(buf, n)
+    if got != n:
+        raise CsmHipError(f"csm_grad_slots_collect: {got} matrices, expected {n}")
+    return [bool(buf[i]) for i in range(n)]
+
+
+def sumsq_launch_count() -> int:
+    return int(lib.csm_sumsq_launch_count())
+
+
+def sumsq_max_ranges() -> int:
+    return lib.csm_sumsq_max_ranges()
+
+
+def sumsq_ranges_bf16(ranges, partials):
+    n = len(ranges)
+    assert 1 <= n <= sumsq_max_ranges() and partials.numel() >= sumsq_blocks()
+    ptrs = (ctypes.c_void_p * n)(*[r[0] for r in ranges])
+    lens = (ctypes.c_longlong * n)(*[r[1] for r in ranges])
+    check(lib.csm_sumsq_ranges_bf16(ptrs, lens, n, partials.data_ptr(), _stream()), "csm_sumsq_ranges_bf16")
+
+
+def clip_max_lists() -> int:
+    return lib.csm_clip_max_lists()
+
+
+def clip_coef_lists(lists, max_norm, norm_and_coef):
+    n = len(lists)
+    assert 1 <= n <= clip_max_lists() and all(t.dtype == torch.float32 and t.is_contiguous() for t in lists)
+    ptrs = (ctypes.c_void_p * n)(*[t.data_ptr() for t in lists])
+    lens = (ctypes.c_int * n)(*[t.numel() for t in lists])
+    check(lib.csm_clip_coef_lists(ptrs, lens, n, float(max_norm), norm_and_coef.data_ptr(), _stream()), "csm_clip_coef_lists")
 
 
 ADAMW_BLOCK = 2048
diff --git a/csm-train-pytorch_amd/csm/training/optim.py b/csm-train-pytorch_amd/csm/training/optim.py
--- a/csm-train-pytorch_amd/csm/training/optim.py
+++ b/csm-train-pytorch_amd/csm/training/optim.py
@@ -7,6 +7,7 @@
 
 F32 = torch.float32
 SPLIT_MASTER = os.environ.get("CSM_ADAMW_SPLIT", "1") == "1"
+FOLD_GRAD_NORM_DEFAULT = "1"
 FLAGGED_GROUPS = ("embeddings",)
 
 
@@ -70,6 +71,9 @@
         self.step_count = 0
         self._coef: Optional[torch.Tensor] = None
         self.dead_blocks = os.environ.get("CSM_ADAMW_DEAD_BLOCKS", "1") == "1"
+        self.fold_norm = os.environ.get("CSM_FOLD_GRAD_NORM", FOLD_GRAD_NORM_DEFAULT) == "1"
+        self._fold_mats: List[tuple] = []
+        self.fold_stats: Optional[dict] = None
         model.ensure_grads()
         for name, lr in group_lrs.items():
             if lr is None or not model.trainable.get(name, False):
@@ -138,6 +142,7 @@
         return sum(g["numel"] for g in self.param_groups)
 
     def zero_grad(self, set_to_none: bool = False):
+        ops.grad_norm_invalidate()
         for g in self.param_groups:
             g["grad"].zero_()
             if g["name"] in self.model.grad_state:
@@ -148,20 +153,94 @@
         gs = self.model.grad_state
         for g in self.param_groups:
             if gs.get(g["name"]) == "stale":
+                ops.grad_norm_invalidate()
                 g["grad"].zero_()
                 gs[g["name"]] = "zero"
 
     def clip_grad_norm(self, max_norm: float) -> torch.Tensor:
         self._settle()
-        nb = ops.sumsq_blocks()
-        for i, g in enumerate(self.param_groups):
-            ops.sumsq_bf16(g["grad"], self._partials[i * nb:(i + 1) * nb])
-        ops.clip_coef(self._partials[:len(self.param_groups) * nb], max_norm, self._norm_coef)
+        if not (self._fold_ready() and self._clip_folded(max_norm)):
+            self.fold_stats = None
+            nb = ops.sumsq_blocks()
+            for i, g in enumerate(self.param_groups):
+                ops.sumsq_bf16(g["grad"], self._partials[i * nb:(i + 1) * nb])
+            ops.clip_coef(self._partials[:len(self.param_groups) * nb], max_norm, self._norm_coef)
         self._coef = self._norm_coef
         return self._norm_coef[0]
 
+    def _fold_ready(self) -> bool:
+        m = self.model
+        eng = getattr(m, "_engine", None)
+        ok = (self.fold_norm and m.lora is None and not any(g["name"] == "lora" for g in self.param_groups)
+              and (eng is None or getattr(eng, "grad_hook", None) is None) and m.grad_arena is not None and m.grad_arena.is_cuda)
+        if not ok and ops.grad_fold.owner == id(self):
+            ops.grad_slots_clear()
+        return ok
+
+    def _fold_register(self):
+        m = self.model
+        names = {g["name"] for g in self.param_groups}
+        mats = [s for s in m._slots.values() if len(s.shape) == 2 and s.group in names and s.group != "embeddings"]
+        mats.sort(key=lambda s: s.offset)
+        counts = [ops.grad_slots_count(*s.shape) for s in mats]
+        ops.grad_slots_clear()
+        slots = torch.zeros(max(1, sum(counts)), dtype=F32, device=m.grad_arena.device)
+        self._fold_mats, off = [], 0
+        for s, c in zip(mats, counts):
+            ops.grad_slots_register(m.grad_arena.data_ptr() + 2 * s.offset, s.shape[0], s.shape[1], s.shape[1], slots, off)
+            self._fold_mats.append((s.offset, s.numel, off, c, s.group))
+            off += c
+        ops.grad_fold.owner, ops.grad_fold.arena_ptr, ops.grad_fold.slots = id(self), m.grad_arena.data_ptr(), slots
+
+    def _clip_folded(self, max_norm: float) -> bool:
+        m, fold = self.model, ops.grad_fold
+        if fold.owner != id(self) or fold.arena_ptr != m.grad_arena.data_ptr():
+            self._fold_register()
+        fresh = ops.grad_slots_collect()
+        emb, fold.embed = fold.embed, None
+        if emb is not None and emb[0] != m.block("text_embeddings.weight", True).data_ptr():
+            emb = None
+        segs, ranges = [], []
+
+        def add(runs, start, n):
+            if runs and runs[-1][0] + runs[-1][1] == start:
+                runs[-1][1] += n
+            else:
+                runs.append([start, n])
+
+        lists_emb = None
+        for g in sorted(self.param_groups, key=lambda g: g["offset"]):
+            lo, hi = g["offset"], g["offset"] + g["numel"]
+            if g["name"] == "embeddings" and emb is not None:
+                lists_emb = emb[1]
+                continue
+            cur = lo
+            for (off, n, soff, cnt, grp), f in zip(self._fold_mats, fresh):
+                if grp == g["name"] and f:
+                    if off > cur:
+                        add(ranges, cur, off - cur)
+                    add(segs, soff, cnt)
+                    cur = off + n
+            if cur < hi:
+                add(ranges, cur, hi - cur)
+        n_lists = len(segs) + (lists_emb is not None) + bool(ranges)
+        if len(ranges) > ops.sumsq_max_ranges() or n_lists > ops.clip_max_lists() or n_lists == 0:
+            return False
+        lists = [fold.slots[a:a + n] for a, n in segs]
+        if lists_emb is not None:
+            lists.append(lists_emb)
+        if ranges:
+            base, nb = m.grad_arena.data_ptr(), ops.sumsq_blocks()
+            ops.sumsq_ranges_bf16([(base + 2 * a, n) for a, n in ranges], self._partials[:nb])
+            lists.append(self._partials[:nb])
+        ops.clip_coef_lists(lists, max_norm, self._norm_coef)
+        self.fold_stats = dict(fresh=sum(fresh), matrices=len(fresh), embeddings=lists_emb is not None, ranges=len(ranges),
+                               range_lens=[n for _, n in ranges], list_lens=[t.numel() for t in lists])
+        return True
+
     def step(self, zero_grad=False, skip: Optional[torch.Tensor] = None):
         self._settle()
+        ops.grad_norm_invalidate()
         self.step_count += 1
         self.model._fp32_source = None
         if skip is not None:
diff --git a/csm-train-pytorch_amd/csrc/common.h b/csm-train-pytorch_amd/csrc/common.h
--- a/csm-train-pytorch_amd/csrc/common.h
+++ b/csm-train-pytorch_amd/csrc/common.h
@@ -109,6 +109,13 @@
     return u;
 }
 
+__device__ __forceinline__ void ssq_add8(const U4& packed, float& ssq) {
+    float f[8];
+    unpack8(packed, f);
+#pragma unroll
+    for (int k = 0; k < 8; ++k) ssq = fmaf(f[k], f[k], ssq);
+}
+
 __device__ __forceinline__ bf16x4 lds_read_tr16(const void* lds_addr) {
     return __builtin_amdgcn_ds_read_tr16_b64_v4i16((__attribute__((address_space(3))) bf16x4*)(lds_addr));
 }
diff --git a/csm-train-pytorch_amd/csrc/gemm.hip b/csm-train-pytorch_amd/csrc/gemm.hip
--- a/csm-train-pytorch_amd/csrc/gemm.hip
+++ b/csm-train-pytorch_amd/csrc/gemm.hip
@@ -330,6 +330,8 @@
     return 0;
 }
 
+extern "C" int csm_grad_slots_touch(const void* ptr);
+
 static int gemm_dispatch(const void* A, const void* B, void* C, const void* R, int M, int N, int K, int lda,
                          int ldb, int ldc, int ldr, int transA, int transB, int out_f32, float alpha, int batch,
                          long long strideA, long long strideB, long long strideC, long long strideR, int epilogue,
@@ -337,6 +339,7 @@
                          const void* xA = nullptr, const void* xB = nullptr, int kx = 0, int pin = 0) {
     const int variant = pin ? 1 : g_gemm_variant;
     CSM_REQUIRE(A && B && C, "csm_gemm_bf16: null operand");
+    csm_grad_slots_touch(C);
     CSM_REQUIRE(M > 0 && N > 0 && K > 0 && batch > 0, "csm_gemm_bf16: bad shape M=%d N=%d K=%d batch=%d", M, N, K, batch);
     CSM_REQUIRE((lda & 7) == 0 && (ldb & 7) == 0, "csm_gemm_bf16: lda/ldb must be multiples of 8 (lda=%d ldb=%d)", lda, ldb);
     CSM_REQUIRE(((uintptr_t)A & 15) == 0 && ((uintptr_t)B & 15) == 0, "csm_gemm_bf16: A/B must be 16-byte aligned");
@@ -477,6 +480,7 @@
                     "csm_gemm_bf16_dgrad_wgrad: bad SwiGLU-backward epilogue arguments");
     else
         CSM_REQUIRE(ld_dx >= Kin, "csm_gemm_bf16_dgrad_wgrad: ld_dx too small");
+    csm_grad_slots_touch(dW);
     return csm_gemm256_pair_launch(dY, W, dX, M, Nout, Kin, ld_dy, ldw, ld_dx, dx_epilogue, aux_in, ld_aux, X, ldx, dW, ld_dw, accumulate,
                                    alpha_w, stream);
 }
@@ -498,6 +502,8 @@
                 ldx2 >= K2 && ld_dw2 >= K2, "csm_gemm_bf16_two_wgrad: bad leading dimensions");
     CSM_REQUIRE((((uintptr_t)dY1 | (uintptr_t)X1 | (uintptr_t)dW1 | (uintptr_t)dY2 | (uintptr_t)X2 | (uintptr_t)dW2) & 15) == 0,
                 "csm_gemm_bf16_two_wgrad: operands must be 16-byte aligned");
+    csm_grad_slots_touch(dW1);
+    csm_grad_slots_touch(dW2);
     if (g_gemm_w4 && g_gemm_variant != 3)
         return csm_gemm256w4_two_wgrad_launch(dY1, X1, dW1, N1, K1, ld_dy1, ldx1, ld_dw1, dY2, X2, dW2, N2, K2, ld_dy2, ldx2, ld_dw2, M,
                                               accumulate, alpha, stream);
@@ -519,6 +525,7 @@
                     ld_dw[i] >= K[i], "csm_gemm_bf16_multi_wgrad: product %d: dimensions must be multiples of 8, leading dimensions >= the row length", i);
         CSM_REQUIRE((((uintptr_t)dY[i] | (uintptr_t)X[i] | (uintptr_t)dW[i]) & 15) == 0, "csm_gemm_bf16_multi_wgrad: product %d: operands must be 16-byte aligned", i);
     }
+    for (int i = 0; i < n; ++i) csm_grad_slots_touch(dW[i]);
     if (!(g_gemm_w4 && g_gemm_variant != 3)) {
         for (int i = 0; i < n; ++i) {
             const int rc = csm_gemm_bf16(dY[i], X[i], dW[i], accumulate ? dW[i] : nullptr, N[i], K[i], M, ld_dy[i], ldx[i], ld_dw[i], ld_dw[i], 1, 1,
diff --git a/csm-train-pytorch_amd/csrc/gemm256w4.hip b/csm-train-pytorch_amd/csrc/gemm256w4.hip
--- a/csm-train-pytorch_amd/csrc/gemm256w4.hip
+++ b/csm-train-pytorch_amd/csrc/gemm256w4.hip
@@ -4,6 +4,7 @@
 extern const char* g_last_gemm_kernel;
 extern int g_persistent;
 extern int g_gemm_touch;
+float* csm_grad_slots_launch(const void* C, int rows, int cols, int ld);
 int g_w4_fast_epi = 1;
 int g_w4_n6 = 1;
 int g_w4_stagger[4] = {1, 0, 0, 0};
@@ -27,6 +28,7 @@
     const bf16_t* xA; const bf16_t* xB; int kx;
     int stagger_groups, stagger_ticks;
     int n6;
+    float* ss;
 };
 
 template <int N>
@@ -79,8 +81,8 @@
                  : "n"(NA), "n"(NA + 1), "n"(NA + 2), "n"(NA + 3), "n"(NB), "n"(NB + 1), "n"(NB + 2), "n"(NB + 3));
 }
 
-template <int JH, bool SWIGLU>
-__device__ __forceinline__ void w4_epi_plain(const Epi& e, int mb, int nb, int lane) {
+template <int JH, bool SWIGLU, bool SSQ = false>
+__device__ __forceinline__ void w4_epi_plain(const Epi& e, int mb, int nb, int lane, float* ssq = nullptr) {
     asm volatile("" : "+v"(lane));
     const int g = lane >> 4, r = lane & 15;
     const int nl = (g & 1) ? 16 + 4 * (g - 1) : 4 * g;
@@ -96,7 +98,9 @@
             w4_gather<(8 * i + 4 * JH + 2 * jp) * 4, (8 * i + 4 * JH + 2 * jp + 1) * 4>(v);
 #pragma unroll
             for (int k = 0; k < 8; ++k) v[k] *= e.alpha;
-            st16_s<64 * jp>(baseC, voffC + i * stepC, pack8_pk(v));
+            const U4 packed = pack8_pk(v);
+            st16_s<64 * jp>(baseC, voffC + i * stepC, packed);
+            if constexpr (SSQ) ssq_add8(packed, *ssq);
             if constexpr (SWIGLU) {
                 float a[4];
 #pragma unroll
@@ -190,6 +194,7 @@
 template <int TA, int TB, typename OutT, int NJ = 8>
 __device__ __forceinline__ void w4_tiles(const W4Args& g, int tile, const int stride, const int bz, char* smem) {
     constexpr int TN = 32 * NJ;
+    constexpr bool SS = TA == 1 && TB == 1 && sizeof(OutT) == 2 && NJ == 8;
     const int nwg = g.tiles_m * g.tiles_n;
     const bf16_t* Ap = g.A + (size_t)bz * g.sA;
     const bf16_t* Bp = g.B + (size_t)bz * g.sB;
@@ -281,7 +286,7 @@
                              : CSM_W4_KEXT_CLOBBERS);
             }
         }
-        const int em0 = m0, en0 = n0;
+        const int em0 = m0, en0 = n0, etile = tile;
         tile += stride;
         const bool more = tile < nwg;
         if (more) {
@@ -306,13 +311,20 @@
             else if (al && e.mode == EPI_SWIGLU_BWD && (e.ld_aux & 7) == 0 && (reinterpret_cast<uintptr_t>(e.aux_in) & 15) == 0) fastm = 3;
         }
         fastm = __builtin_amdgcn_readfirstlane(fastm);
+        float ssq = 0.f;
+        bool emit = false;
+        if constexpr (SS) emit = g.ss != nullptr;
         static_for<0, 2>([&](auto jh_) {
             constexpr int jh = decltype(jh_)::value;
             if constexpr (sizeof(OutT) == 2) {
                 if (fastm) {
                     if (CSM_ABLATE_W4EPI & 8) return;
                     const int mb = __builtin_amdgcn_readfirstlane(em0 + wr * 128), nb = __builtin_amdgcn_readfirstlane(en0 + wc * (16 * NJ) + jh * 64);
-                    if (fastm == 1) { w4_epi_plain<jh, false>(e, mb, nb, lane); pend += 16; }
+                    if (fastm == 1) {
+                        if (SS && emit) w4_epi_plain<jh, false, SS>(e, mb, nb, lane, &ssq);
+                        else w4_epi_plain<jh, false>(e, mb, nb, lane);
+                        pend += 16;
+                    }
                     else if (fastm == 2) { w4_epi_plain<jh, true>(e, mb, nb, lane); pend += 32; }
                     else if (jh == 0) { w4_epi_swiglu_bwd(e, mb, nb, lane); pend += 128; }
                     return;
@@ -335,9 +347,16 @@
                 if constexpr (sizeof(OutT) == 2) epi_swiglu_bwd_block<8, 4>(e, mb, nb, lane, acc);
                 pend += 32;
             } else {
-                pend += epi_block<OutT, 8>(e, vec_ok, mb, nb, lane, acc);
+                pend += epi_block<OutT, 8, 2, SS>(e, vec_ok, mb, nb, lane, acc, &ssq);
             }
         });
+        if constexpr (SS) {
+            if (emit) {
+                const float t = wave_sum(ssq);
+                if (lane == 0) g.ss[etile * 4 + wave] = t;
+                pend += 1;
+            }
+        }
         if (!full) pend = 0;
         if (!more) break;
     }
@@ -435,6 +454,7 @@
     }
     g.epi_mode = epi_mode; g.aux_in = (const bf16_t*)aux_in; g.aux_out = (bf16_t*)aux_out; g.ld_aux = ld_aux;
     g.epi_p0 = epi_p0; g.epi_p1 = epi_p1; g.touch = g_gemm_touch; g.fast_epi = g_w4_fast_epi;
+    g.ss = (transA && transB && !out_f32 && batch == 1 && epi_mode == EPI_NONE && kx == 0) ? csm_grad_slots_launch(C, M, N, ldc) : nullptr;
     {
         const long long tiles = (long long)g.tiles_m * g.tiles_n;
         const int ticks = g_w4_stagger[epi_mode == EPI_SWIGLU_FWD ? 1 : epi_mode == EPI_SWIGLU_BWD ? 2 : 3];
@@ -456,6 +476,7 @@
     g.epi_mode = EPI_NONE; g.aux_in = nullptr; g.aux_out = nullptr; g.ld_aux = 0; g.epi_p0 = g.epi_p1 = 0; g.touch = 0;
     g.stagger_groups = 1; g.stagger_ticks = 0; g.fast_epi = g_w4_fast_epi;
     g.xA = g.xB = nullptr; g.kx = 0; g.n6 = 0;
+    g.ss = csm_grad_slots_launch(C, M, N, ldc);
 }
 
 int csm_gemm256w4_two_wgrad_launch(const void* dY1, const void* X1, void* dW1, int N1, int K1, int ld_dy1, int ldx1, int ld_dw1,
diff --git a/csm-train-pytorch_amd/csrc/gemm_common.h b/csm-train-pytorch_amd/csrc/gemm_common.h
--- a/csm-train-pytorch_amd/csrc/gemm_common.h
+++ b/csm-train-pytorch_amd/csrc/gemm_common.h
@@ -219,8 +219,8 @@
     }
 }
 
-template <typename OutT>
-__device__ __forceinline__ void epi_store(const Epi& e, bool vec_ok, int m, int n, const f32x4& a) {
+template <typename OutT, bool SSQ = false>
+__device__ __forceinline__ void epi_store(const Epi& e, bool vec_ok, int m, int n, const f32x4& a, float* ssq = nullptr) {
     float v[4] = {a[0] * e.alpha, a[1] * e.alpha, a[2] * e.alpha, a[3] * e.alpha};
     if (e.mode == EPI_SWIGLU_BWD) {
         if constexpr (sizeof(OutT) == 2) {
@@ -247,6 +247,11 @@
         if constexpr (sizeof(OutT) == 2) {
             uint2 o; o.x = pack2bf(v[0], v[1]); o.y = pack2bf(v[2], v[3]);
             store8_asm(reinterpret_cast<bf16_t*>(e.C) + (size_t)m * e.ldc + n, o);
+            if constexpr (SSQ) {
+                const float f0 = __uint_as_float(o.x << 16), f1 = __uint_as_float(o.x & 0xffff0000u);
+                const float f2 = __uint_as_float(o.y << 16), f3 = __uint_as_float(o.y & 0xffff0000u);
+                *ssq = fmaf(f3, f3, fmaf(f2, f2, fmaf(f1, f1, fmaf(f0, f0, *ssq))));
+            }
             if (e.mode == EPI_SWIGLU_FWD) {
                 const float a0 = silu(v[0]) * v[1];
                 const float a1 = silu(v[2]) * v[3];
@@ -260,7 +265,11 @@
         for (int k = 0; k < 4 && n + k < e.N; ++k) {
             float x = v[k];
             if (e.R) x += bf2f(e.R[(size_t)m * e.ldr + n + k]);
-            if constexpr (sizeof(OutT) == 2) store2_asm(reinterpret_cast<bf16_t*>(e.C) + (size_t)m * e.ldc + n + k, f2bf(x));
+            if constexpr (sizeof(OutT) == 2) {
+                const bf16_t xb = f2bf(x);
+                store2_asm(reinterpret_cast<bf16_t*>(e.C) + (size_t)m * e.ldc + n + k, xb);
+                if constexpr (SSQ) { const float f = bf2f(xb); *ssq = fmaf(f, f, *ssq); }
+            }
             else store4_asm(reinterpret_cast<float*>(e.C) + (size_t)m * e.ldc + n + k, __float_as_uint(x));
         }
     }
@@ -308,8 +317,9 @@
     }
 }
 
-template <typename OutT>
-__device__ __forceinline__ void epi_store_pair(const Epi& e, bool vec_ok, int m, int nb, int lane, const f32x4& a, const f32x4& b) {
+template <typename OutT, bool SSQ = false>
+__device__ __forceinline__ void epi_store_pair(const Epi& e, bool vec_ok, int m, int nb, int lane, const f32x4& a, const f32x4& b,
+                                               float* ssq = nullptr) {
     const int g = lane >> 4;
     bool wide = false;
     if constexpr (sizeof(OutT) == 2)
@@ -318,8 +328,8 @@
                (!e.R || (reinterpret_cast<uintptr_t>(e.R) & 15) == 0);
     if (!wide) {
         const int n = nb + 4 * g;
-        if (m < e.M && n < e.N) epi_store<OutT>(e, vec_ok, m, n, a);
-        if (m < e.M && n + 16 < e.N) epi_store<OutT>(e, vec_ok, m, n + 16, b);
+        if (m < e.M && n < e.N) epi_store<OutT, SSQ>(e, vec_ok, m, n, a, ssq);
+        if (m < e.M && n + 16 < e.N) epi_store<OutT, SSQ>(e, vec_ok, m, n + 16, b, ssq);
         return;
     }
     float v[8];
@@ -338,7 +348,9 @@
         for (int k = 0; k < 8; ++k) v[k] += rr[k];
     }
     if (e.mode == EPI_ROPE) epi_rope<4>(e, m, n, v);
-    store16_asm(reinterpret_cast<bf16_t*>(e.C) + (size_t)m * e.ldc + n, pack8(v));
+    const U4 packed = pack8(v);
+    store16_asm(reinterpret_cast<bf16_t*>(e.C) + (size_t)m * e.ldc + n, packed);
+    if constexpr (SSQ) ssq_add8(packed, *ssq);
     if (e.mode == EPI_SWIGLU_FWD) {
         float a[4];
 #pragma unroll
@@ -348,8 +360,8 @@
     }
 }
 
-template <typename OutT, int NI, int NJP = 2>
-__device__ __forceinline__ int epi_block(const Epi& e, bool vec_ok, int mb, int nb, int lane, const f32x4 (&acc)[NI][4]) {
+template <typename OutT, int NI, int NJP = 2, bool SSQ = false>
+__device__ __forceinline__ int epi_block(const Epi& e, bool vec_ok, int mb, int nb, int lane, const f32x4 (&acc)[NI][4], float* ssq = nullptr) {
     bool fast = false;
     if constexpr (sizeof(OutT) == 2)
         fast = vec_ok && (e.mode == EPI_NONE || (e.mode == EPI_ROPE && (e.p0 & 63) == 0 && (e.p1 & 7) == 0) ||
@@ -361,7 +373,7 @@
         for (int i = 0; i < NI; ++i) {
             const int m = mb + 16 * i + (lane & 15);
 #pragma unroll
-            for (int jp = 0; jp < NJP; ++jp) epi_store_pair<OutT>(e, vec_ok, m, nb + 32 * jp, lane, acc[i][2 * jp], acc[i][2 * jp + 1]);
+            for (int jp = 0; jp < NJP; ++jp) epi_store_pair<OutT, SSQ>(e, vec_ok, m, nb + 32 * jp, lane, acc[i][2 * jp], acc[i][2 * jp + 1], ssq);
         }
         return 0;
     }
@@ -443,7 +455,9 @@
                 }
                 const int n = nl + 32 * jp;
                 if (m < e.M) {
-                    store16_asm(C + (size_t)m * e.ldc + n, pack8(v));
+                    const U4 packed = pack8(v);
+                    store16_asm(C + (size_t)m * e.ldc + n, packed);
+                    if constexpr (SSQ) ssq_add8(packed, *ssq);
                     if (e.mode == EPI_SWIGLU_FWD) {
                         float a[4];
 #pragma unroll
diff --git a/csm-train-pytorch_amd/csrc/grad_slots.cpp b/csm-train-pytorch_amd/csrc/grad_slots.cpp
--- /dev/null
+++ b/csm-train-pytorch_amd/csrc/grad_slots.cpp
@@ -0,0 +1,69 @@
+#include <stdint.h>
+
+#include <map>
+#include <vector>
+
+extern "C" void csm_set_error(const char* fmt, ...);
+
+namespace {
+struct GradMatrix { uintptr_t base, end; int rows, cols, ld; float* slots; bool fresh; };
+std::vector<GradMatrix> g_mats;
+std::map<uintptr_t, int> g_by_base;
+unsigned long long g_sumsq_launches = 0;
+
+GradMatrix* find_containing(uintptr_t p) {
+    if (g_by_base.empty()) return nullptr;
+    auto it = g_by_base.upper_bound(p);
+    if (it == g_by_base.begin()) return nullptr;
+    GradMatrix& m = g_mats[(--it)->second];
+    return p < m.end ? &m : nullptr;
+}
+}
+
+float* csm_grad_slots_launch(const void* C, int rows, int cols, int ld) {
+    GradMatrix* m = find_containing((uintptr_t)C);
+    if (!m) return nullptr;
+    if (m->base == (uintptr_t)C && m->rows == rows && m->cols == cols && m->ld == ld) { m->fresh = true; return m->slots; }
+    m->fresh = false;
+    return nullptr;
+}
+
+extern "C" int csm_grad_slots_count(int rows, int cols) {
+    if (rows <= 0 || cols <= 0) return 0;
+    return 4 * ((rows + 255) / 256) * ((cols + 255) / 256);
+}
+
+extern "C" int csm_grad_slots_register(const void* ptr, int rows, int cols, int ld, float* slots) {
+    if (!ptr || !slots || rows <= 0 || cols <= 0 || ld < cols) { csm_set_error("csm_grad_slots_register: bad arguments"); return -1; }
+    const uintptr_t base = (uintptr_t)ptr, end = base + ((size_t)(rows - 1) * ld + cols) * 2;
+    auto it = g_by_base.lower_bound(base);
+    if ((it != g_by_base.end() && it->first < end) || (it != g_by_base.begin() && g_mats[std::prev(it)->second].end > base)) {
+        csm_set_error("csm_grad_slots_register: the matrix overlaps a registered one");
+        return -1;
+    }
+    g_mats.push_back(GradMatrix{base, end, rows, cols, ld, slots, false});
+    g_by_base[base] = (int)g_mats.size() - 1;
+    return (int)g_mats.size() - 1;
+}
+
+extern "C" int csm_grad_slots_clear(void) { g_mats.clear(); g_by_base.clear(); return 0; }
+
+extern "C" int csm_grad_slots_invalidate(void) {
+    for (auto& m : g_mats) m.fresh = false;
+    return 0;
+}
+
+extern "C" int csm_grad_slots_touch(const void* ptr) {
+    if (GradMatrix* m = find_containing((uintptr_t)ptr)) m->fresh = false;
+    return 0;
+}
+
+extern "C" int csm_grad_slots_collect(unsigned char* fresh, int capacity) {
+    const int n = (int)g_mats.size();
+    if (n > capacity || (n > 0 && !fresh)) { csm_set_error("csm_grad_slots_collect: %d matrices registered, room for %d", n, capacity); return -1; }
+    for (int i = 0; i < n; ++i) { fresh[i] = g_mats[i].fresh ? 1 : 0; g_mats[i].fresh = false; }
+    return n;
+}
+
+void csm_count_sumsq_launch(void) { ++g_sumsq_launches; }
+extern "C" unsigned long long csm_sumsq_launch_count(void) { return g_sumsq_launches; }
diff --git a/csm-train-pytorch_amd/csrc/ops.hip b/csm-train-pytorch_amd/csrc/ops.hip
--- a/csm-train-pytorch_amd/csrc/ops.hip
+++ b/csm-train-pytorch_amd/csrc/ops.hip
@@ -1,5 +1,8 @@
 #include "common.h"
 #include <math.h>
+
+extern "C" int csm_grad_slots_touch(const void* ptr);
+void csm_count_sumsq_launch(void);
 
 namespace {
 
@@ -323,17 +326,14 @@
     }
 }
 
-template <int NC>
-__global__ __launch_bounds__(256) void embed_bwd_sorted_kernel(const long long* __restrict__ rows, const long long* __restrict__ src,
-                                                               long long n_occ, const bf16_t* __restrict__ dh,
-                                                               const bf16_t* __restrict__ dseq, long long M,
-                                                               bf16_t* __restrict__ g_text, bf16_t* __restrict__ g_audio,
-                                                               long long text_rows, long long n_rows, int D) {
-    const int lane = threadIdx.x & 63;
-    const long long i = (long long)blockIdx.x * (blockDim.x >> 6) + (threadIdx.x >> 6);
-    if (i >= n_occ) return;
+template <int NC, bool SSQ>
+__device__ __forceinline__ float embed_bwd_row(long long i, int lane, const long long* __restrict__ rows, const long long* __restrict__ src,
+                                               long long n_occ, const bf16_t* __restrict__ dh, const bf16_t* __restrict__ dseq, long long M,
+                                               bf16_t* __restrict__ g_text, bf16_t* __restrict__ g_audio, long long text_rows,
+                                               long long n_rows, int D) {
+    float ssq = 0.f;
     const long long r = rows[i];
-    if (r >= n_rows || (i > 0 && rows[i - 1] == r)) return;
+    if (r >= n_rows || (i > 0 && rows[i - 1] == r)) return ssq;
     float acc[NC][8];
 #pragma unroll
     for (int c = 0; c < NC; ++c)
@@ -363,8 +363,33 @@
             unpack8(*reinterpret_cast<const U4*>(dst + ch * 8), f);
 #pragma unroll
             for (int j = 0; j < 8; ++j) f[j] += acc[c][j];
-            *reinterpret_cast<U4*>(dst + ch * 8) = pack8(f);
-        }
+            const U4 packed = pack8(f);
+            *reinterpret_cast<U4*>(dst + ch * 8) = packed;
+            if constexpr (SSQ) ssq_add8(packed, ssq);
+        }
+    }
+    return ssq;
+}
+
+
+template <int NC, bool SSQ = false>
+__global__ __launch_bounds__(256) void embed_bwd_sorted_kernel(const long long* __restrict__ rows, const long long* __restrict__ src,
+                                                               long long n_occ, const bf16_t* __restrict__ dh,
+                                                               const bf16_t* __restrict__ dseq, long long M,
+                                                               bf16_t* __restrict__ g_text, bf16_t* __restrict__ g_audio,
+                                                               long long text_rows, long long n_rows, int D, float* __restrict__ slots) {
+    const int lane = threadIdx.x & 63;
+    const long long i = (long long)blockIdx.x * (blockDim.x >> 6) + (threadIdx.x >> 6);
+    float ssq = 0.f;
+    if constexpr (SSQ) {
+        if (i < n_occ) ssq = embed_bwd_row<NC, true>(i, lane, rows, src, n_occ, dh, dseq, M, g_text, g_audio, text_rows, n_rows, D);
+        __shared__ float red[4];
+        ssq = wave_sum(ssq);
+        if (lane == 0) red[threadIdx.x >> 6] = ssq;
+        __syncthreads();
+        if (threadIdx.x == 0) slots[blockIdx.x] = ((red[0] + red[1]) + red[2]) + red[3];
+    } else {
+        if (i < n_occ) embed_bwd_row<NC, false>(i, lane, rows, src, n_occ, dh, dseq, M, g_text, g_audio, text_rows, n_rows, D);
     }
 }
 
@@ -533,6 +558,46 @@
         for (long long i = (nvec << 3) + threadIdx.x; i < n; i += blockDim.x) { const float f = bf2f(g[i]); acc += f * f; }
     acc = block_sum(acc, red);
     if (threadIdx.x == 0) partials[blockIdx.x] = acc;
+}
+
+#define CSM_SUMSQ_MAX_RANGES 128
+struct SumsqRanges { const bf16_t* p[CSM_SUMSQ_MAX_RANGES]; long long n[CSM_SUMSQ_MAX_RANGES]; };
+__global__ __launch_bounds__(256) void sumsq_ranges_kernel(SumsqRanges r, int nr, float* __restrict__ partials) {
+    __shared__ float red[16];
+    float acc = 0.f;
+    const long long stride = (long long)gridDim.x * blockDim.x;
+    for (int k = 0; k < nr; ++k) {
+        const bf16_t* __restrict__ g = r.p[k];
+        const long long n = r.n[k], nvec = n >> 3;
+        long long i = (long long)blockIdx.x * blockDim.x + threadIdx.x;
+        for (; i + stride < nvec; i += 2 * stride) {
+            const U4 q0 = *reinterpret_cast<const U4*>(g + i * 8), q1 = *reinterpret_cast<const U4*>(g + (i + stride) * 8);
+            ssq_add8(q0, acc);
+            ssq_add8(q1, acc);
+        }
+        if (i < nvec) ssq_add8(*reinterpret_cast<const U4*>(g + i * 8), acc);
+        if (blockIdx.x == 0)
+            for (long long j = (nvec << 3) + threadIdx.x; j < n; j += blockDim.x) { const float f = bf2f(g[j]); acc = fmaf(f, f, acc); }
+    }
+    acc = block_sum(acc, red);
+    if (threadIdx.x == 0) partials[blockIdx.x] = acc;
+}
+
+#define CSM_CLIP_MAX_LISTS 96
+struct ClipLists { const float* p[CSM_CLIP_MAX_LISTS]; int n[CSM_CLIP_MAX_LISTS]; };
+__global__ __launch_bounds__(1024) void clip_coef_lists_kernel(ClipLists l, int nl, float max_norm, float* __restrict__ out) {
+    __shared__ float red[16];
+    float acc = 0.f;
+    for (int k = 0; k < nl; ++k) {
+        const float* __restrict__ p = l.p[k];
+        for (int i = threadIdx.x; i < l.n[k]; i += blockDim.x) acc += p[i];
+    }
+    acc = block_sum(acc, red);
+    if (threadIdx.x == 0) {
+        const float norm = sqrtf(acc);
+        out[0] = norm;
+        out[1] = (max_norm > 0.f) ? fminf(1.f, max_norm / (norm + 1e-6f)) : 1.f;
+    }
 }
 
 __global__ __launch_bounds__(1024) void clip_coef_kernel(const float* __restrict__ partials, int n, float max_norm,
@@ -796,6 +861,7 @@
 
 extern "C" int csm_colsum_bf16(const float* partials, int rows, int D, void* dst, int accumulate, hipStream_t stream) {
     CSM_REQUIRE(partials && dst && rows > 0 && D > 0, "csm_colsum_bf16: bad arguments");
+    csm_grad_slots_touch(dst);
     hipLaunchKernelGGL(colsum_kernel, dim3((D + 63) / 64), dim3(rows >= 64 ? 1024 : 256), 0, stream, partials, rows, D, (bf16_t*)dst,
                        accumulate);
     CSM_CHECK_LAUNCH("csm_colsum_bf16");
@@ -809,6 +875,7 @@
     for (int i = 0; i < 8; ++i) {
         CSM_REQUIRE(i >= n || (partials[i] && dst[i]), "csm_colsum_bf16_multi: null pointer in pair %d", i);
         p.partials[i] = partials[i < n ? i : 0]; p.dst[i] = (bf16_t*)dst[i < n ? i : 0];
+        if (i < n) csm_grad_slots_touch(dst[i]);
     }
     hipLaunchKernelGGL(colsum_multi_kernel, dim3((D + 63) / 64, n), dim3(rows >= 64 ? 1024 : 256), 0, stream, p, rows, D, accumulate);
     CSM_CHECK_LAUNCH("csm_colsum_bf16_multi");
@@ -882,19 +949,35 @@
     return 0;
 }
 
-extern "C" int csm_embed_bwd_sorted(const long long* sorted_rows, const long long* src_index, long long n_occ, const void* dh,
-                                    const void* dseq, long long M, void* g_text, void* g_audio, long long text_rows,
-                                    long long n_rows, int D, hipStream_t stream) {
+static int embed_bwd_sorted_launch(const long long* sorted_rows, const long long* src_index, long long n_occ, const void* dh,
+                                   const void* dseq, long long M, void* g_text, void* g_audio, long long text_rows,
+                                   long long n_rows, int D, float* slots, hipStream_t stream) {
     CSM_REQUIRE(sorted_rows && src_index && dh && g_text && g_audio && n_occ > 0, "csm_embed_bwd_sorted: bad arguments");
     CSM_REQUIRE((D & 7) == 0 && D <= 4096, "csm_embed_bwd_sorted: D=%d must be a multiple of 8 and <= 4096", D);
     const long long blocks = (n_occ + 3) / 4;
     CSM_REQUIRE(blocks < (1ll << 31), "csm_embed_bwd_sorted: too many occurrences");
     const int nc = (D + 511) / 512;
-#define L(NC) hipLaunchKernelGGL((embed_bwd_sorted_kernel<NC>), dim3((unsigned)blocks), dim3(256), 0, stream, sorted_rows, src_index, n_occ, (const bf16_t*)dh, (const bf16_t*)dseq, M, (bf16_t*)g_text, (bf16_t*)g_audio, text_rows, n_rows, D)
-    if (nc <= 1) L(1); else if (nc <= 2) L(2); else if (nc <= 4) L(4); else L(8);
+#define L(NC, SSQ) hipLaunchKernelGGL((embed_bwd_sorted_kernel<NC, SSQ>), dim3((unsigned)blocks), dim3(256), 0, stream, sorted_rows, src_index, n_occ, (const bf16_t*)dh, (const bf16_t*)dseq, M, (bf16_t*)g_text, (bf16_t*)g_audio, text_rows, n_rows, D, slots)
+    if (slots) { if (nc <= 1) L(1, true); else if (nc <= 2) L(2, true); else if (nc <= 4) L(4, true); else L(8, true); }
+    else { if (nc <= 1) L(1, false); else if (nc <= 2) L(2, false); else if (nc <= 4) L(4, false); else L(8, false); }
 #undef L
     CSM_CHECK_LAUNCH("csm_embed_bwd_sorted");
     return 0;
+}
+
+extern "C" int csm_embed_bwd_sorted(const long long* sorted_rows, const long long* src_index, long long n_occ, const void* dh,
+                                    const void* dseq, long long M, void* g_text, void* g_audio, long long text_rows,
+                                    long long n_rows, int D, hipStream_t stream) {
+    return embed_bwd_sorted_launch(sorted_rows, src_index, n_occ, dh, dseq, M, g_text, g_audio, text_rows, n_rows, D, nullptr, stream);
+}
+
+extern "C" long long csm_embed_bwd_sumsq_slots(long long n_occ) { return (n_occ + 3) / 4; }
+
+extern "C" int csm_embed_bwd_sorted_sumsq(const long long* sorted_rows, const long long* src_index, long long n_occ, const void* dh,
+                                          const void* dseq, long long M, void* g_text, void* g_audio, long long text_rows,
+                                          long long n_rows, int D, float* slots, hipStream_t stream) {
+    CSM_REQUIRE(slots, "csm_embed_bwd_sorted_sumsq: null slots");
+    return embed_bwd_sorted_launch(sorted_rows, src_index, n_occ, dh, dseq, M, g_text, g_audio, text_rows, n_rows, D, slots, stream);
 }
 
 extern "C" int csm_rows_add_bf16(void* dst, const int* rows, const void* src, long long N, int src_stride_rows, int D,
@@ -956,6 +1039,37 @@
     CSM_REQUIRE(g && partials && n > 0 && ((uintptr_t)g & 15) == 0, "csm_sumsq_bf16: bad arguments");
     hipLaunchKernelGGL(sumsq_kernel, dim3(CSM_SUMSQ_BLOCKS), dim3(256), 0, stream, (const bf16_t*)g, n, partials);
     CSM_CHECK_LAUNCH("csm_sumsq_bf16");
+    csm_count_sumsq_launch();
+    return 0;
+}
+
+extern "C" int csm_sumsq_max_ranges(void) { return CSM_SUMSQ_MAX_RANGES; }
+
+extern "C" int csm_sumsq_ranges_bf16(const void* const* ptr, const long long* len, int n, float* partials, hipStream_t stream) {
+    CSM_REQUIRE(ptr && len && partials && n >= 1 && n <= CSM_SUMSQ_MAX_RANGES, "csm_sumsq_ranges_bf16: 1..%d ranges", CSM_SUMSQ_MAX_RANGES);
+    SumsqRanges r;
+    for (int i = 0; i < CSM_SUMSQ_MAX_RANGES; ++i) {
+        CSM_REQUIRE(i >= n || (ptr[i] && len[i] > 0 && ((uintptr_t)ptr[i] & 15) == 0), "csm_sumsq_ranges_bf16: range %d: null, empty or not 16-byte aligned", i);
+        r.p[i] = (const bf16_t*)ptr[i < n ? i : 0]; r.n[i] = i < n ? len[i] : 0;
+    }
+    hipLaunchKernelGGL(sumsq_ranges_kernel, dim3(CSM_SUMSQ_BLOCKS), dim3(256), 0, stream, r, n, partials);
+    CSM_CHECK_LAUNCH("csm_sumsq_ranges_bf16");
+    csm_count_sumsq_launch();
+    return 0;
+}
+
+extern "C" int csm_clip_max_lists(void) { return CSM_CLIP_MAX_LISTS; }
+
+extern "C" int csm_clip_coef_lists(const float* const* list, const int* len, int n, float max_norm, float* norm_and_coef,
+                                   hipStream_t stream) {
+    CSM_REQUIRE(list && len && norm_and_coef && n >= 1 && n <= CSM_CLIP_MAX_LISTS, "csm_clip_coef_lists: 1..%d lists", CSM_CLIP_MAX_LISTS);
+    ClipLists l;
+    for (int i = 0; i < CSM_CLIP_MAX_LISTS; ++i) {
+        CSM_REQUIRE(i >= n || (list[i] && len[i] > 0), "csm_clip_coef_lists: list %d: null or empty", i);
+        l.p[i] = list[i < n ? i : 0]; l.n[i] = i < n ? len[i] : 0;
+    }
+    hipLaunchKernelGGL(clip_coef_lists_kernel, dim3(1), dim3(1024), 0, stream, l, n, max_norm, norm_and_coef);
+    CSM_CHECK_LAUNCH("csm_clip_coef_lists");
     return 0;
 }
 
diff --git a/include/csm_hip.h b/include/csm_hip.h
--- a/include/csm_hip.h
+++ b/include/csm_hip.h
@@ -87,6 +87,10 @@
 int csm_embed_bwd_sorted(const long long* sorted_rows, const long long* src_index, long long n_occ, const void* dh,
                          const void* dseq, long long M, void* g_text, void* g_audio, long long text_rows, long long n_rows,
                          int D, csm_stream_t stream);
+long long csm_embed_bwd_sumsq_slots(long long n_occ);
+int csm_embed_bwd_sorted_sumsq(const long long* sorted_rows, const long long* src_index, long long n_occ, const void* dh,
+                               const void* dseq, long long M, void* g_text, void* g_audio, long long text_rows, long long n_rows,
+                               int D, float* slots, csm_stream_t stream);
 int csm_rows_add_bf16(void* dst, const int* rows, const void* src, long long N, int src_stride_rows, int D, csm_stream_t stream);
 int csm_rows_take_bf16(void* table, const int* rows, void* out, long long N, int D, csm_stream_t stream);
 
@@ -100,6 +104,18 @@
 int csm_sumsq_blocks(void);
 int csm_sumsq_bf16(const void* g, long long n, float* partials , csm_stream_t stream);
 int csm_clip_coef(const float* partials, int n_partials, float max_norm, float* norm_and_coef , csm_stream_t stream);
+int csm_grad_slots_count(int rows, int cols);
+int csm_grad_slots_register(const void* matrix, int rows, int cols, int ld, float* slots);
+int csm_grad_slots_clear(void);
+int csm_grad_slots_invalidate(void);
+int csm_grad_slots_touch(const void* ptr);
+int csm_grad_slots_collect(unsigned char* fresh, int capacity);
+int csm_sumsq_max_ranges(void);
+int csm_sumsq_ranges_bf16(const void* const* ptr, const long long* len, int n, float* partials, csm_stream_t stream);
+unsigned long long csm_sumsq_launch_count(void);
+int csm_clip_max_lists(void);
+int csm_clip_coef_lists(const float* const* list, const int* len, int n, float max_norm, float* norm_and_coef ,
+                        csm_stream_t stream);
 int csm_adamw_step(float* master, float* m, float* v, void* param, void* grad, long long n, float lr, float beta1,
                    float beta2, float eps, float weight_decay, int step, const float* norm_and_coef ,
                    float grad_mul, int zero_grad , csm_stream_t stream);
```

After: 130,200 (median of 6 runs). No clear change (+0.4%).
